# lidq92/LBDRN-MSIC

Hardware: AMD Instinct MI355X
Metric: Mpixels/s encode+decode (and bpp/PSNR parity) on D2/K5/bc64/nl2 (higher is better)
Workload: dtype f32; 1 GPU; synthetic 8-band 2048x2048 uint16 tile per step, K=5 D=2 bc=64 nl=2 bs=8192 e=10 (BASELINE.json configs[1] by default); encode fit + 16-bit weight truncation + decode; tiles_per_gpu=50, tiles_in_flight_per_gpu=4, tiles_per_launch=2, parallelism=image-sharded x1

## Files before the change

include/lbdrn_hip.h:

```cpp
#ifndef LBDRN_HIP_H
#define LBDRN_HIP_H

#include <stddef.h>
#include <stdint.h>

#ifdef __cplusplus
extern "C" {
#endif
#if defined(__GNUC__)
#pragma GCC visibility push(default)
#endif

#define LBDRN_ABI_VERSION 2

typedef enum lbdrn_status {
    LBDRN_OK = 0,
    LBDRN_E_ARG = -1,
    LBDRN_E_DEVICE = -2,
    LBDRN_E_UNSUPPORTED = -3,
    LBDRN_E_WORKSPACE = -4
} lbdrn_status;

typedef struct lbdrn_geom {
    int32_t C, H, W;
    int32_t K;
    int32_t D;
    int32_t msb_max;
    int32_t use_colors;
    int32_t relative;
    int32_t P;
    int32_t reserved;
    const float *rowtab;
    const float *coltab;
} lbdrn_geom;

typedef struct lbdrn_net {
    int32_t F, bc, C, nl;
    int32_t act;
} lbdrn_net;
enum { LBDRN_ACT_SINE = 0, LBDRN_ACT_RELU = 1 };

const char *lbdrn_last_error(void);
int lbdrn_abi_version(void);
int lbdrn_device_check(void);
int64_t lbdrn_param_count(const lbdrn_net *net);
int32_t lbdrn_feature_dim(const lbdrn_geom *g);

int lbdrn_split_bits(const uint16_t *img, int32_t C, int32_t H, int32_t W, int32_t K,
                     uint16_t *msb, int32_t *msb_max, void *stream);

int lbdrn_labels(const uint16_t *img, int32_t C, int32_t H, int32_t W, int32_t K,
                 const int64_t *idx, int64_t n, float *labels, void *stream);

int lbdrn_features(const lbdrn_geom *g, const uint16_t *msb, const int64_t *idx, int64_t n,
                   float *features, void *stream);

size_t lbdrn_forward_workspace(const lbdrn_net *net, int64_t B);
int lbdrn_forward(const lbdrn_net *net, const float *params, const float *x, int64_t B, float *y,
                  void *workspace, size_t workspace_bytes, void *stream);

size_t lbdrn_tape_bytes(const lbdrn_net *net, int64_t B);
int lbdrn_forward_tape(const lbdrn_net *net, const float *params, const float *x, int64_t B, float *y,
                       void *tape, size_t tape_bytes, void *stream);
size_t lbdrn_backward_workspace(const lbdrn_net *net, int64_t B);
int lbdrn_backward(const lbdrn_net *net, const float *params, const float *x, int64_t B, const void *tape,
                   size_t tape_bytes, const float *y, const float *dy, float *grads, float *dx, void *workspace,
                   size_t workspace_bytes, void *stream);

#define LBDRN_PATH_AUTO 0
#define LBDRN_PATH_GENERIC 1
#define LBDRN_PATH_MFMA 2
size_t lbdrn_apply_workspace(const lbdrn_geom *g, const lbdrn_net *net);
int lbdrn_decode_fused(const lbdrn_geom *g, const lbdrn_net *net, const uint16_t *msb,
                       const float *params, uint16_t *out, float *y_out, void *workspace,
                       size_t workspace_bytes, int32_t path, void *stream);

#define LBDRN_EVAL_BACKGROUND 0x200
#define LBDRN_EVAL_FAST 0x400
#define LBDRN_EVAL_X16 0x1000
#define LBDRN_EVAL_VALID 0x4000
#define LBDRN_EVAL_DECODED 0x8000
int lbdrn_eval_sse(const lbdrn_geom *g, const lbdrn_net *net, const uint16_t *img,
                   const uint16_t *msb, const float *params, double *sse, void *workspace,
                   size_t workspace_bytes, int32_t path, void *stream);

#define LBDRN_APPLY_DECODE 0x2000
int lbdrn_apply_instance(const lbdrn_geom *g, const lbdrn_net *net, int32_t path_word, int32_t *out);

size_t lbdrn_train_workspace(const lbdrn_geom *g, const lbdrn_net *net, int32_t batch_size);
#define LBDRN_TRAIN_ALONE 0x800
int lbdrn_train_prepare(const lbdrn_geom *g, const lbdrn_net *net, const uint16_t *img,
                        const uint16_t *msb, int32_t batch_size, void *workspace,
                        size_t workspace_bytes, int32_t path, void *stream);
int lbdrn_train_epoch(const lbdrn_geom *g, const lbdrn_net *net, const uint16_t *img,
                      const uint16_t *msb, const int64_t *perm, int64_t n, int32_t batch_size,
                      float *params, float *exp_avg, float *exp_avg_sq, int64_t adam_step0,
                      double lr, float *losses, void *workspace, size_t workspace_bytes,
                      int32_t path, void *stream);

int lbdrn_train_group_max(void);
int32_t lbdrn_train_group_size(const lbdrn_geom *g, const lbdrn_net *net);
int32_t lbdrn_train_step_features(const lbdrn_geom *g, const lbdrn_net *net);
int lbdrn_train_epoch_group(int32_t count, const lbdrn_geom *const *g, const lbdrn_net *net,
                            const uint16_t *const *img, const uint16_t *const *msb, const int64_t *const *perm,
                            int64_t n, int32_t batch_size, float *const *params, float *const *exp_avg,
                            float *const *exp_avg_sq, int64_t adam_step0, double lr, float *const *losses,
                            void *const *workspace, size_t workspace_bytes, int32_t path, void *stream);

int lbdrn_train_profile_mode(int32_t mode);

size_t lbdrn_randperm_workspace(int64_t n, int32_t count);
int lbdrn_randperm(const uint64_t *seeds, int32_t count, int64_t n, int64_t *perm, void *workspace,
                   size_t workspace_bytes, void *stream);
int64_t lbdrn_mt19937_jump_poly(int32_t segment, uint32_t *poly624);

size_t lbdrn_plane_bound(int32_t C, int32_t H, int32_t W);
size_t lbdrn_plane_workspace(int32_t C, int32_t H, int32_t W);
int lbdrn_plane_encode(const uint16_t *planes, int32_t C, int32_t H, int32_t W, void *body, size_t body_capacity,
                       uint64_t *body_bytes, void *workspace, size_t workspace_bytes, void *stream);
int lbdrn_plane_decode(const void *body, size_t body_bytes, int32_t C, int32_t H, int32_t W, uint16_t *planes,
                       int32_t *status, void *workspace, size_t workspace_bytes, void *stream);

int64_t lbdrn_jp2k_block_count(int32_t C, int32_t H, int32_t W);
size_t lbdrn_jp2k_bound(int32_t C, int32_t H, int32_t W);
size_t lbdrn_jp2k_workspace(int32_t C, int32_t H, int32_t W);
int lbdrn_jp2k_encode(const uint16_t *planes, int32_t C, int32_t H, int32_t W, int32_t bits, void *out, size_t capacity,
                      size_t *nbytes, void *workspace, size_t workspace_bytes, void *stream);

size_t lbdrn_weights_bound(int64_t n);
int lbdrn_weights_encode(const float *values, int64_t n, int32_t precision, void *out, size_t capacity,
                         size_t *nbytes);
int lbdrn_weights_info(const void *stream, size_t nbytes, int64_t *n, int32_t *precision);
int lbdrn_weights_decode(const void *stream, size_t nbytes, float *values, int64_t capacity);

int lbdrn_train_step(const lbdrn_net *net, const float *x, const float *t, int32_t B,
                     float *params, float *exp_avg, float *exp_avg_sq, int64_t adam_step,
                     double lr, int32_t apply_adam, float *loss, float *grads, void *workspace,
                     size_t workspace_bytes, void *stream);

#if defined(__GNUC__)
#pragma GCC visibility pop
#endif
#ifdef __cplusplus
}
#endif
#endif
```

lbdrn-msic_amd/csrc/apply_mfma.hip:

```cpp
#include <cstdlib>

#include "common.hpp"
#include "lbdrn_math.hpp"

namespace lbdrn {

typedef float f32x16 __attribute__((ext_vector_type(16)));
typedef float f32x4 __attribute__((ext_vector_type(4)));
typedef _Float16 f16x8 __attribute__((ext_vector_type(8)));
typedef _Float16 f16x2 __attribute__((ext_vector_type(2)));

constexpr int APPLY_CHUNK = 20;
constexpr int APPLY_WAVES = 8;
constexpr int APPLY_THREADS = APPLY_WAVES * 64;
constexpr int TILE_W = 64;

__host__ __device__ inline int tile_row_to_neuron(int i)
{
    return 2 * ((i & 3) + 4 * (i >> 3)) + ((i >> 2) & 1);
}
__host__ __device__ inline int acc_row(int r, int h) { return (r & 3) + 8 * (r >> 2) + 4 * h; }

enum ApplyMode { MODE_DECODE = 0, MODE_EVAL = 1, MODE_EVAL_FAST = 2,
                 MODE_EVAL_X16 = 3 };
__host__ __device__ constexpr bool mode_fast(int mode) { return mode == MODE_EVAL_FAST || mode == MODE_EVAL_X16; }

#define APPLY_INSTANCES(X) \
    X(1, MODE_DECODE)    X(2, MODE_DECODE)    X(4, MODE_DECODE) \
    X(1, MODE_EVAL)      X(2, MODE_EVAL)      X(4, MODE_EVAL)   \
    X(1, MODE_EVAL_FAST) X(2, MODE_EVAL_FAST)                   \
    X(1, MODE_EVAL_X16)  X(2, MODE_EVAL_X16)
#define WAPPLY_INSTANCES(X) X(8, 1) X(8, 2) X(16, 1) X(16, 2)

#define X(NT, MODE) if (nt == NT && (mode < 0 || mode == MODE)) return true;
constexpr bool apply_row(int nt, int mode = -1) { APPLY_INSTANCES(X) return false; }
#undef X
#define X(NT, NL) if (nt == NT && (nl < 0 || nl == NL)) return true;
constexpr bool wapply_row(int nt, int nl = -1) { WAPPLY_INSTANCES(X) return false; }
#undef X
constexpr int serving_mode(int mode, int nt, bool x16)
{
    if (mode == MODE_EVAL_X16 && !(x16 && apply_row(nt, MODE_EVAL_X16))) mode = MODE_EVAL_FAST;
    if (mode == MODE_EVAL_FAST && !(apply_row(nt, MODE_EVAL_FAST) || wapply_row(nt))) mode = MODE_EVAL;
    return mode;
}
#define SERVES(mode, x16, nt12, nt4, wide)                                                                                          \
    static_assert(serving_mode(mode, 1, x16) == nt12 && serving_mode(mode, 2, x16) == nt12 && serving_mode(mode, 4, x16) == nt4 && \
                  serving_mode(mode, 8, x16) == wide && serving_mode(mode, 16, x16) == wide, #mode);
SERVES(MODE_DECODE, false, MODE_DECODE, MODE_DECODE, MODE_DECODE)          SERVES(MODE_DECODE, true, MODE_DECODE, MODE_DECODE, MODE_DECODE)
SERVES(MODE_EVAL, false, MODE_EVAL, MODE_EVAL, MODE_EVAL)                  SERVES(MODE_EVAL, true, MODE_EVAL, MODE_EVAL, MODE_EVAL)
SERVES(MODE_EVAL_FAST, false, MODE_EVAL_FAST, MODE_EVAL, MODE_EVAL_FAST)   SERVES(MODE_EVAL_FAST, true, MODE_EVAL_FAST, MODE_EVAL, MODE_EVAL_FAST)
SERVES(MODE_EVAL_X16, false, MODE_EVAL_FAST, MODE_EVAL, MODE_EVAL_FAST)    SERVES(MODE_EVAL_X16, true, MODE_EVAL_X16, MODE_EVAL, MODE_EVAL_FAST)
#undef SERVES

struct ApplyPlan {
    int NT;
    int S0;
    int TH;
    int SH, SW;
    int ncolor;
    int pair;
    int RS;
    int x16;
    int M16;
    int off_scale;
    int off_w0, off_wh, off_wl, off_bh, off_bl, pack_floats;
    int off_ktab, off_rowt, off_colt, off_tile, lds_floats;
    int tiles_x, tiles_y;
};

constexpr int X16_PIECES = 3;

static bool make_plan(const lbdrn_geom& g, const lbdrn_net& net, ApplyPlan* p, bool fast = false, bool x16 = false)
{
    if (net.act != LBDRN_ACT_SINE && net.act != LBDRN_ACT_RELU) return false;
    if (net.bc % 32 != 0 || !apply_row(net.bc / 32)) return false;
    if (net.C > 32 || net.nl < 1 || net.nl > 15) return false;
    ApplyPlan q;
    q.NT = net.bc / 32;
    q.ncolor = net.F - 2 * g.P;
    if (q.ncolor < 0) return false;
    q.S0 = g.P + ((q.ncolor + 1) / 2 + 3) / 4 * 4;
    const int side = 2 * g.D + 1;
    q.pair = fast && q.NT <= 2 && g.use_colors && g.D >= 1 && g.D <= 3 && (g.C % 2) == 0 && q.ncolor == g.C * side * side;
    q.RS = side * side - ((g.relative && g.D > 0) ? 1 : 0);
    if (q.pair) q.S0 = g.P + (g.C / 2) * q.RS;
    q.x16 = x16 && q.pair && g.relative && g.P == 0 && g.msb_max >= 1 && g.msb_max <= 2047 && (q.RS % 8) == 0;
    q.M16 = q.RS / 8;
    const int half = net.bc / 2;
    int o = 0;
    q.off_w0 = o; o += q.x16 ? (g.C / 2) * q.M16 * X16_PIECES * 64 * q.NT * 4 : q.S0 * 64 * q.NT;
    q.off_wh = o; o += (net.nl - 1) * half * 64 * q.NT;
    q.off_wl = o; o += half * 64;
    q.off_bh = o; o += net.nl * q.NT * 32;
    q.off_bl = o; o += 32;
    q.off_scale = o; o += 4;
    q.pack_floats = o;
    q.off_ktab = o; o += 2 * 2 * (q.S0 - g.P) + 2;
    q.SW = TILE_W + 2 * g.D;
    const int fixed = o;
    int th = 16;
    for (;; th >>= 1) {
        if (th == 0) return false;
        q.TH = th;
        q.SH = th + 2 * g.D;
        o = fixed;
        q.off_rowt = o; o += th * g.P;
        q.off_colt = o; o += TILE_W * g.P;
        q.off_tile = o; o += (g.use_colors ? g.C * q.SH * q.SW : 0);
        q.lds_floats = std::max(o, q.off_rowt + 2 * APPLY_THREADS + 4);
        if ((size_t)q.lds_floats * 4 <= 160 * 1024) break;
    }
    q.tiles_x = (g.W + TILE_W - 1) / TILE_W;
    q.tiles_y = (g.H + q.TH - 1) / q.TH;
    *p = q;
    return true;
}

constexpr int MFMA_PARTIALS = 1024;


__global__ void __launch_bounds__(256) k_w0_absmax(const float* __restrict__ params, int n, float* __restrict__ out)
{
    __shared__ float red[256];
    float m = 0.0f;
    for (int e = threadIdx.x; e < n; e += 256) m = fmaxf(m, fabsf(params[e]));
    red[threadIdx.x] = m;
    __syncthreads();
    for (int o = 128; o > 0; o >>= 1) {
        if ((int)threadIdx.x < o) red[threadIdx.x] = fmaxf(red[threadIdx.x], red[threadIdx.x + o]);
        __syncthreads();
    }
    if (threadIdx.x == 0) *out = red[0];
}

__device__ __forceinline__ int x16_shift(float amax)
{
    if (!(amax > 0.0f) || !(amax < 3.0e38f)) return 0;
    int ex;
    (void)frexpf(amax, &ex);
    return 15 - ex;
}

__global__ void __launch_bounds__(256)
    k_pack_apply(const float* __restrict__ params, lbdrn_net net, ApplyPlan p, int P, int C, int msb_max, const float* __restrict__ amax,
                 float* __restrict__ out)
{
    int e = blockIdx.x * blockDim.x + threadIdx.x;
    if (e >= p.pack_floats) return;
    const int NT = p.NT, half = net.bc / 2;
    float v = 0.0f;
    if (p.x16 && e < p.off_wh) {
        const int j = e & 3, q4 = e >> 2;
        const int t = q4 % NT, lane = (q4 / NT) % 64, rest = q4 / (NT * 64);
        const int piece = rest % X16_PIECES, m = (rest / X16_PIECES) % p.M16, cp = rest / (X16_PIECES * p.M16);
        const int s2 = p.ncolor / C, cen = s2 / 2, sh = x16_shift(*amax);
        const int neuron = tile_row_to_neuron(lane & 31) + 32 * t, ch = cp + (lane >> 5) * (C / 2);
        _Float16 hv[2];
        for (int u = 0; u < 2; ++u) {
            const int pos = 8 * m + 2 * j + u, r = pos + (pos >= cen ? 1 : 0);
            const float w = ldexpf(params[(int64_t)neuron * net.F + ch * s2 + r], sh);
            const _Float16 hi = (_Float16)w;
            const float r1 = w - (float)hi;
            const _Float16 mid = (_Float16)r1;
            const float r2 = r1 - (float)mid;
            hv[u] = piece == 0 ? hi : piece == 1 ? mid : (_Float16)r2;
        }
        f16x2 pk = {hv[0], hv[1]};
        out[e] = __builtin_bit_cast(float, pk);
        return;
    }
    if (e >= p.off_scale) {
        out[e] = (p.x16 && e == p.off_scale) ? ldexpf(1.0f, -x16_shift(*amax)) / (float)msb_max : 0.0f;
        return;
    }
    if (e < p.off_wh) {
        int t = e % NT, lane = (e / NT) % 64, s = e / (NT * 64);
        int k = 2 * s + (lane >> 5);
        if (p.pair && s >= P) {
            const int s2 = (p.ncolor / C), sp = s - P, c = sp / p.RS, rr = sp - c * p.RS;
            const int r = rr + ((p.RS < s2 && rr >= s2 / 2) ? 1 : 0);
            k = 2 * P + (c + (lane >> 5) * (C / 2)) * s2 + r;
        }
        int neuron = tile_row_to_neuron(lane & 31) + 32 * t;
        if (k < net.F) v = params[(int64_t)neuron * net.F + k];
    } else if (e < p.off_wl) {
        int q = e - p.off_wh;
        int t = q % NT, lane = (q / NT) % 64, s = (q / (NT * 64)) % half, l = 1 + q / (NT * 64 * half);
        int k = 2 * s + (lane >> 5);
        int neuron = tile_row_to_neuron(lane & 31) + 32 * t;
        int64_t base = (int64_t)net.bc * net.F + net.bc + (int64_t)(l - 1) * ((int64_t)net.bc * net.bc + net.bc);
        v = params[base + (int64_t)neuron * net.bc + k];
    } else if (e < p.off_bh) {
        int q = e - p.off_wl;
        int lane = q % 64, s = q / 64;
        int k = 2 * s + (lane >> 5), ch = lane & 31;
        int64_t base = (int64_t)net.bc * net.F + net.bc + (int64_t)(net.nl - 1) * ((int64_t)net.bc * net.bc + net.bc);
        if (ch < net.C) v = params[base + (int64_t)ch * net.bc + k];
    } else if (e < p.off_bl) {
        int q = e - p.off_bh;
        int r = q % 16, h = (q / 16) % 2, t = (q / 32) % NT, l = q / (32 * NT);
        int neuron = 2 * r + h + 32 * t;
        int64_t wbase = l == 0 ? 0 : (int64_t)net.bc * net.F + net.bc + (int64_t)(l - 1) * ((int64_t)net.bc * net.bc + net.bc);
        int64_t nin = l == 0 ? net.F : net.bc;
        v = params[wbase + (int64_t)net.bc * nin + neuron];
    } else {
        int q = e - p.off_bl;
        int r = q % 16, h = q / 16;
        int ch = acc_row(r, h);
        int64_t base = (int64_t)net.bc * net.F + net.bc + (int64_t)(net.nl - 1) * ((int64_t)net.bc * net.bc + net.bc);
        if (ch < net.C) v = params[base + (int64_t)net.C * net.bc + ch];
    }
    out[e] = v;
}


struct ApplyArgs {
    lbdrn_geom g;
    lbdrn_net net;
    ApplyPlan p;
    const float* packed;
    const uint16_t* msb;
    const uint16_t* img;
    uint16_t* out;
    float* y_out;
    double* partial;
    int nvirt;
    int nodata;
    int decoded;
    unsigned long long* stamps;
};

#ifdef LBDRN_APPLY_STAMPS
#define ASTAMP(k)                                                                    \
    do {                                                                              \
        unsigned long long t_;                                                        \
        __builtin_amdgcn_sched_barrier(0);                                            \
        asm volatile("s_memtime %0\n\ts_waitcnt lgkmcnt(0)" : "=s"(t_)::"memory");   \
        __builtin_amdgcn_sched_barrier(0);                                            \
        acc_t[k] += t_ - last_t;                                                      \
        last_t = t_;                                                                  \
    } while (0)
#else
#define ASTAMP(k)
#endif

template <int NT>
__device__ __forceinline__ void load_a(const float* w, int idx, float (&a)[NT])
{
    if constexpr (NT == 1) {
        a[0] = w[idx];
    } else if constexpr (NT == 2) {
        float2 v = *reinterpret_cast<const float2*>(w + (size_t)idx * 2);
        a[0] = v.x; a[1] = v.y;
    } else {
        float4 v = *reinterpret_cast<const float4*>(w + (size_t)idx * 4);
        a[0] = v.x; a[1] = v.y; a[2] = v.z; a[3] = v.w;
    }
}

template <int NT, int D, bool REL>
__device__ __forceinline__ void layer0_pair(f32x16 (&acc)[NT], const float* wc, const float* tp)
{
    constexpr int side = 2 * D + 1, S2 = side * side, CEN = D * side + D, SW = TILE_W + 2 * D, RS = S2 - (REL ? 1 : 0);
    const float cen = tp[D * SW + D];
    float bq[RS];
#pragma unroll
    for (int r = 0; r < S2; ++r) {
        if (REL && r == CEN) continue;
        const float nb = tp[(r / side) * SW + (r % side)];
        bq[r - ((REL && r > CEN) ? 1 : 0)] = REL ? nb - cen : nb;
    }
    __builtin_amdgcn_sched_barrier(0);
#pragma unroll
    for (int k = 0; k < RS; ++k) {
        float a[NT];
        load_a<NT>(wc, k * 64, a);
#pragma unroll
        for (int tt = 0; tt < NT; ++tt) acc[tt] = __builtin_amdgcn_mfma_f32_32x32x2f32(a[tt], bq[k], acc[tt], 0, 0, 0);
    }
    __builtin_amdgcn_sched_barrier(0);
}

template <int NT, int D>
__device__ __forceinline__ void layer0_pair_x16(f32x16 (&acc)[NT], const float* wc, const float* tp)
{
    constexpr int side = 2 * D + 1, S2 = side * side, CEN = D * side + D, SW = TILE_W + 2 * D, RS = S2 - 1, M = RS / 8;
    static_assert(RS % 8 == 0, "(2D+1)^2 - 1 = 4 D (D+1)");
    const float cen = tp[D * SW + D];
    float bq[RS];
#pragma unroll
    for (int r = 0; r < S2; ++r) {
        if (r == CEN) continue;
        bq[r - (r > CEN ? 1 : 0)] = tp[(r / side) * SW + (r % side)] - cen;
    }
    f16x8 b[M];
#pragma unroll
    for (int m = 0; m < M; ++m)
#pragma unroll
        for (int j = 0; j < 4; ++j) {
            const f16x2 pk = __builtin_bit_cast(f16x2, __builtin_amdgcn_cvt_pkrtz(bq[8 * m + 2 * j], bq[8 * m + 2 * j + 1]));
            b[m][2 * j] = pk[0];
            b[m][2 * j + 1] = pk[1];
        }
    __builtin_amdgcn_sched_barrier(0);
#pragma unroll
    for (int m = 0; m < M; ++m)
#pragma unroll
        for (int pc = 0; pc < X16_PIECES; ++pc) {
            const float4* ap = reinterpret_cast<const float4*>(wc + (size_t)((m * X16_PIECES + pc) * 64) * NT * 4);
#pragma unroll
            for (int tt = 0; tt < NT; ++tt)
                acc[tt] = __builtin_amdgcn_mfma_f32_32x32x16_f16(__builtin_bit_cast(f16x8, ap[tt]), b[m], acc[tt], 0, 0, 0);
        }
    __builtin_amdgcn_sched_barrier(0);
}

template <int MODE, bool RELU>
__device__ __forceinline__ float apply_hidden_act(float z)
{
    if constexpr (RELU) return z > 0.0f ? z : 0.0f;
    else return mode_fast(MODE) ? fast_sin(30.0f * z) : siren_act(z);
}

template <int NT, int NG>
__device__ __forceinline__ void last_layer_4x4(f32x16& o, const f32x16 (&hid)[NT], const float* wl, const float* bl, int lane)
{
    const bool lo = lane < 32;
    f32x4 part[NG];
#pragma unroll
    for (int gq = 0; gq < NG; ++gq) {
        const float4 b4 = *reinterpret_cast<const float4*>(bl + gq * 16);
        part[gq][0] = lo ? b4.x : 0.0f; part[gq][1] = lo ? b4.y : 0.0f;
        part[gq][2] = lo ? b4.z : 0.0f; part[gq][3] = lo ? b4.w : 0.0f;
    }
    const float* wq = wl + (lane & 32) + (lane & 3);
    float a[NT * 16][NG];
#pragma unroll
    for (int s = 0; s < NT * 16; ++s)
#pragma unroll
        for (int gq = 0; gq < NG; ++gq) a[s][gq] = wq[s * 64 + 4 * gq];
    __builtin_amdgcn_sched_barrier(0);
#pragma unroll
    for (int s = 0; s < NT * 16; ++s) {
        const float b = hid[s / 16][s % 16];
#pragma unroll
        for (int gq = 0; gq < NG; ++gq) part[gq] = __builtin_amdgcn_mfma_f32_4x4x1f32(a[s][gq], b, part[gq], 0, 0, 0);
    }
#pragma unroll
    for (int i = 0; i < 4; ++i) {
        const float x = part[0][i], y = part[NG - 1][i];
        const auto sw = __builtin_amdgcn_permlane32_swap(__float_as_uint(x), __float_as_uint(y), false, false);
        const unsigned even = sw[0], odd = sw[1];
        o[i] = __uint_as_float(even) + __uint_as_float(odd);
    }
}

template <int NT, int MODE, bool RELU>
__global__ void __launch_bounds__(APPLY_THREADS) k_apply_mfma(ApplyArgs A)
{
    extern __shared__ __attribute__((aligned(16))) float lds[];
    const lbdrn_geom& g = A.g;
    const ApplyPlan& p = A.p;
    const int tid = threadIdx.x;
    const int lane = tid & 63, wave = tid >> 6;
    const int j = lane & 31, h = lane >> 5;
    const int half = A.net.bc / 2;
    const int P = g.P, D = g.D, C = g.C;

    for (int e = tid * 4; e < p.pack_floats; e += APPLY_THREADS * 4) {
        if (e + 3 < p.pack_floats) {
            *reinterpret_cast<float4*>(lds + e) = *reinterpret_cast<const float4*>(A.packed + e);
        } else {
            for (int q = e; q < p.pack_floats; ++q) lds[q] = A.packed[q];
        }
    }
    int* ktab = reinterpret_cast<int*>(lds + p.off_ktab);
    {
        const int side = 2 * D + 1, plane = p.SH * p.SW;
        for (int k = tid; k < 2 * (p.S0 - P) + 1; k += APPLY_THREADS) {
            int kk = min(k, p.ncolor - 1);
            kk = max(kk, 0);
            int c = kk / (side * side), r = kk - c * side * side;
            int dy = r / side, dx = r - dy * side;
            ktab[2 * k] = c * plane + (dy - D) * p.SW + (dx - D);
            ktab[2 * k + 1] = c * plane;
        }
    }
    const float* w0 = lds + p.off_w0;
    const float* wh = lds + p.off_wh;
    const float* wl = lds + p.off_wl;
    const float* bh = lds + p.off_bh;
    const float* bl = lds + p.off_bl;
    float* rowt = lds + p.off_rowt;
    float* colt = lds + p.off_colt;
    float* tile = lds + p.off_tile;
    const bool rel = g.relative && D > 0;
    const float maxf = (float)g.msb_max;
    const int64_t HW = (int64_t)g.H * g.W;
    const float scale = (float)((1 << g.K) - 1);
    const int lmask = (1 << g.K) - 1;
#ifdef LBDRN_APPLY_STAMPS
    unsigned long long acc_t[8] = {}, last_t;
    asm volatile("s_memtime %0\n\ts_waitcnt lgkmcnt(0)" : "=s"(last_t)::"memory");
#endif
    const int ntiles = p.tiles_x * p.tiles_y;
    for (int v = blockIdx.x; v < A.nvirt; v += gridDim.x) {
    double sse = 0.0;
    for (int t = v; t < ntiles; t += A.nvirt) {
        const int ty = t / p.tiles_x, tx = t - ty * p.tiles_x;
        const int y0 = ty * p.TH, x0 = tx * TILE_W;
        __syncthreads();
        if (g.use_colors) {
            const int plane = p.SH * p.SW, total = C * plane;
            const unsigned msw = 0xFFFFFFFFu / (unsigned)p.SW + 1u, msh = 0xFFFFFFFFu / (unsigned)p.SH + 1u;
            const bool simple = D < g.H && D < g.W && total < 65536 && p.SH > 1;
            constexpr int UB = 8;
            for (int base = 0; base < total; base += APPLY_THREADS * UB) {
                unsigned short raw[UB];
#pragma unroll
                for (int u = 0; u < UB; ++u) {
                    const int e = min(base + u * APPLY_THREADS + tid, total - 1);
                    int row, sx, c, sy, yy, xx;
                    if (simple) {
                        row = (int)__umulhi((unsigned)e, msw); sx = e - row * p.SW;
                        c = (int)__umulhi((unsigned)row, msh); sy = row - c * p.SH;
                        yy = y0 + sy - D; xx = x0 + sx - D;
                        yy = yy < 0 ? -yy : yy; yy = yy >= g.H ? 2 * (g.H - 1) - yy : yy;
                        xx = xx < 0 ? -xx : xx; xx = xx >= g.W ? 2 * (g.W - 1) - xx : xx;
                        yy = max(0, min(yy, g.H - 1));
                        xx = max(0, min(xx, g.W - 1));
                    } else {
                        row = e / p.SW; sx = e - row * p.SW; c = row / p.SH; sy = row - c * p.SH;
                        yy = reflect_idx(y0 + sy - D, g.H); xx = reflect_idx(x0 + sx - D, g.W);
                    }
                    raw[u] = mode_fast(MODE) ? (unsigned short)(A.img[(int64_t)c * HW + (int64_t)yy * g.W + xx] >> g.K)
                                             : A.msb[(int64_t)c * HW + (int64_t)yy * g.W + xx];
                }
#pragma unroll
                for (int u = 0; u < UB; ++u) {
                    const int e = base + u * APPLY_THREADS + tid;
                    if (e < total) tile[e] = MODE == MODE_EVAL_X16 ? (float)raw[u] : (float)raw[u] / maxf;
                }
            }
        }
        for (int e = tid; e < p.TH * P; e += APPLY_THREADS) {
            int yy = min(y0 + e / P, g.H - 1);
            rowt[e] = g.rowtab[(int64_t)yy * P + e % P];
        }
        for (int e = tid; e < TILE_W * P; e += APPLY_THREADS) {
            int xx = min(x0 + e / P, g.W - 1);
            colt[e] = g.coltab[(int64_t)xx * P + e % P];
        }
        __syncthreads();

        ASTAMP(0);
        const int nseg = p.TH * (TILE_W / 32);
        for (int seg = wave; seg < nseg; seg += APPLY_WAVES) {
            const int ly = seg / (TILE_W / 32), lx = (seg % (TILE_W / 32)) * 32;
            const int pixbase = (ly + D) * p.SW + (lx + j + D);
            const int yy = y0 + ly, xx = x0 + lx + j;
            const bool inside = yy < g.H && xx < g.W;
            const int64_t pix = (int64_t)min(yy, g.H - 1) * g.W + min(xx, g.W - 1);
            const int nreg = 4 * ((C + 7) / 8);
            unsigned short pre[16];
            {
                const uint16_t* src = (MODE == MODE_DECODE) ? A.msb : A.img;
#pragma unroll
                for (int r = 0; r < 16; ++r) {
                    pre[r] = 0;
                    if (r < nreg) pre[r] = src[(int64_t)min(acc_row(r, h), C - 1) * HW + pix];
                }
            }
            f32x16 acc[NT];
            f32x16 hid[NT];
#pragma unroll
            for (int tt = 0; tt < NT; ++tt)
#pragma unroll
                for (int q4 = 0; q4 < 4; ++q4) {
                    float4 b4 = *reinterpret_cast<const float4*>(bh + (tt * 2 + h) * 16 + q4 * 4);
                    acc[tt][q4 * 4 + 0] = b4.x; acc[tt][q4 * 4 + 1] = b4.y;
                    acc[tt][q4 * 4 + 2] = b4.z; acc[tt][q4 * 4 + 3] = b4.w;
                }
            if constexpr (MODE == MODE_EVAL_X16) {
                f32x16 bias0[NT];
#pragma unroll
                for (int tt = 0; tt < NT; ++tt) {
                    bias0[tt] = acc[tt];
#pragma unroll
                    for (int r = 0; r < 16; ++r) acc[tt][r] = 0.0f;
                }
                const int plane = p.SH * p.SW;
                const float* tp = tile + h * (C / 2) * plane + ly * p.SW + lx + j;
                const float* wc = w0 + (size_t)lane * NT * 4;
                const size_t wstep = (size_t)p.M16 * X16_PIECES * 64 * NT * 4;
                for (int c = 0; c < C / 2; ++c, tp += plane, wc += wstep) {
                    if (D == 1) layer0_pair_x16<NT, 1>(acc, wc, tp);
                    else if (D == 2) layer0_pair_x16<NT, 2>(acc, wc, tp);
                    else layer0_pair_x16<NT, 3>(acc, wc, tp);
                }
                const float cs = lds[p.off_scale];
#pragma unroll
                for (int tt = 0; tt < NT; ++tt)
#pragma unroll
                    for (int r = 0; r < 16; ++r) acc[tt][r] = fmaf(acc[tt][r], cs, bias0[tt][r]);
            }
            for (int s = 0; s < (MODE == MODE_EVAL_X16 ? 0 : P); ++s) {
                int k = 2 * s + h;
                float b = (k < P) ? rowt[ly * P + k] : colt[(lx + j) * P + (k - P)];
                float a[NT];
                load_a<NT>(w0, s * 64 + lane, a);
#pragma unroll
                for (int tt = 0; tt < NT; ++tt)
                    acc[tt] = __builtin_amdgcn_mfma_f32_32x32x2f32(a[tt], b, acc[tt], 0, 0, 0);
            }
            bool paired = MODE == MODE_EVAL_X16;
            if constexpr (MODE == MODE_EVAL_FAST) {
                if (p.pair) {
                    paired = true;
                    const int plane = p.SH * p.SW;
                    const float* tp = tile + h * (C / 2) * plane + ly * p.SW + lx + j;
                    const float* wc = w0 + ((size_t)P * 64 + lane) * NT;
                    for (int c = 0; c < C / 2; ++c, tp += plane, wc += (size_t)p.RS * 64 * NT) {
                        if (rel) {
                            if (D == 1) layer0_pair<NT, 1, true>(acc, wc, tp);
                            else if (D == 2) layer0_pair<NT, 2, true>(acc, wc, tp);
                            else layer0_pair<NT, 3, true>(acc, wc, tp);
                        } else {
                            if (D == 1) layer0_pair<NT, 1, false>(acc, wc, tp);
                            else if (D == 2) layer0_pair<NT, 2, false>(acc, wc, tp);
                            else layer0_pair<NT, 3, false>(acc, wc, tp);
                        }
                    }
                }
            }
            if (!paired) {
                constexpr int CH = APPLY_CHUNK;
                static_assert(CH % 4 == 0, "the steps left behind the chunks are taken four at a time");
                int s4 = P;
                for (; s4 + CH <= p.S0; s4 += CH) {
                    float bq[CH];
#pragma unroll
                    for (int u = 0; u < CH; ++u) {
                        const int kk = 2 * (s4 + u - P) + h;
                        const int2 e = *reinterpret_cast<const int2*>(ktab + 2 * kk);
                        const float nb = tile[pixbase + e.x];
                        const float ct = tile[pixbase + e.y];
                        bq[u] = rel ? nb - ct : nb;
                    }
                    __builtin_amdgcn_sched_barrier(0);
#pragma unroll
                    for (int u = 0; u < CH; ++u) {
                        float a[NT];
                        load_a<NT>(w0, (s4 + u) * 64 + lane, a);
#pragma unroll
                        for (int tt = 0; tt < NT; ++tt)
                            acc[tt] = __builtin_amdgcn_mfma_f32_32x32x2f32(a[tt], bq[u], acc[tt], 0, 0, 0);
                    }
                    __builtin_amdgcn_sched_barrier(0);
                }
                for (; s4 < p.S0; s4 += 4) {
                    float bq[4];
                    float aq[4][NT];
#pragma unroll
                    for (int u = 0; u < 4; ++u) {
                        int kk = 2 * (s4 + u - P) + h;
                        int2 e = *reinterpret_cast<const int2*>(ktab + 2 * kk);
                        float nb = tile[pixbase + e.x];
                        float ct = tile[pixbase + e.y];
                        bq[u] = rel ? nb - ct : nb;
                        load_a<NT>(w0, (s4 + u) * 64 + lane, aq[u]);
                    }
#pragma unroll
                    for (int u = 0; u < 4; ++u)
#pragma unroll
                        for (int tt = 0; tt < NT; ++tt)
                            acc[tt] = __builtin_amdgcn_mfma_f32_32x32x2f32(aq[u][tt], bq[u], acc[tt], 0, 0, 0);
                }
            }
            ASTAMP(1);
#pragma unroll
            for (int tt = 0; tt < NT; ++tt)
#pragma unroll
                for (int r = 0; r < 16; ++r) hid[tt][r] = apply_hidden_act<MODE, RELU>(acc[tt][r]);
            ASTAMP(2);
            for (int l = 1; l < A.net.nl; ++l) {
                const float* wlayer = wh + (size_t)(l - 1) * half * 64 * NT;
#pragma unroll
                for (int tt = 0; tt < NT; ++tt)
#pragma unroll
                    for (int q4 = 0; q4 < 4; ++q4) {
                        float4 b4 = *reinterpret_cast<const float4*>(bh + ((l * NT + tt) * 2 + h) * 16 + q4 * 4);
                        acc[tt][q4 * 4 + 0] = b4.x; acc[tt][q4 * 4 + 1] = b4.y;
                        acc[tt][q4 * 4 + 2] = b4.z; acc[tt][q4 * 4 + 3] = b4.w;
                    }
#pragma unroll
                for (int s = 0; s < NT * 16; ++s) {
                    float b = hid[s / 16][s % 16];
                    float a[NT];
                    load_a<NT>(wlayer, s * 64 + lane, a);
#pragma unroll
                    for (int tt = 0; tt < NT; ++tt)
                        acc[tt] = __builtin_amdgcn_mfma_f32_32x32x2f32(a[tt], b, acc[tt], 0, 0, 0);
                }
#pragma unroll
                for (int tt = 0; tt < NT; ++tt)
#pragma unroll
                    for (int r = 0; r < 16; ++r) hid[tt][r] = apply_hidden_act<MODE, RELU>(acc[tt][r]);
            }
            ASTAMP(3);
            f32x16 o;
            if (mode_fast(MODE)) {
                if (C > 4) last_layer_4x4<NT, 2>(o, hid, wl, bl, lane);
                else last_layer_4x4<NT, 1>(o, hid, wl, bl, lane);
            } else {
#pragma unroll
                for (int q4 = 0; q4 < 4; ++q4) {
                    float4 b4 = *reinterpret_cast<const float4*>(bl + h * 16 + q4 * 4);
                    o[q4 * 4 + 0] = b4.x; o[q4 * 4 + 1] = b4.y; o[q4 * 4 + 2] = b4.z; o[q4 * 4 + 3] = b4.w;
                }
#pragma unroll
                for (int s = 0; s < NT * 16; ++s) {
                    float b = hid[s / 16][s % 16];
                    float a = wl[s * 64 + lane];
                    o = __builtin_amdgcn_mfma_f32_32x32x2f32(a, b, o, 0, 0, 0);
                }
            }
            ASTAMP(4);
#pragma unroll
            for (int r = 0; r < 16; ++r) {
                const int ch = acc_row(r, h);
                if (r < nreg && ch < C && inside) {
                    float yv = mode_fast(MODE) ? fast_sigmoid(o[r]) : canon_sigmoid(o[r]);
                    if (MODE == MODE_DECODE) {
                        float rr = __builtin_rintf(yv * scale);
                        int base = (int)pre[r] << g.K;
                        A.out[(int64_t)ch * HW + pix] = (uint16_t)(base + (int)rr);
                        if (A.y_out) A.y_out[pix * C + ch] = yv;
                    } else if ((int)pre[r] != A.nodata) {
                        if (MODE == MODE_EVAL && A.decoded) {
                            int band = ch;
                            asm volatile("" : "+v"(band));
                            sse += decoded_term((int)pre[r], (int)A.msb[(int64_t)band * HW + pix], yv, scale, g.K);
                            continue;
                        }
                        float lab = (float)((int)pre[r] & lmask) / scale;
                        float d = yv - lab;
                        sse += (double)(d * d);
                    }
                }
            }
            ASTAMP(5);
        }
    }
    if (MODE != MODE_DECODE) {
        __syncthreads();
        double* red = reinterpret_cast<double*>(lds + ((p.off_rowt + 3) & ~3));
        red[tid] = sse;
        __syncthreads();
        for (int o2 = APPLY_THREADS / 2; o2 > 0; o2 >>= 1) {
            if (tid < o2) red[tid] += red[tid + o2];
            __syncthreads();
        }
        if (tid == 0) A.partial[v] = red[0];
    }
    }
#ifdef LBDRN_APPLY_STAMPS
    if (tid == 0 && A.stamps)
        for (int k = 0; k < 8; ++k) A.stamps[(size_t)blockIdx.x * 8 + k] = acc_t[k];
#endif
}

__global__ void k_sum_partials_mfma(const double* __restrict__ partial, int n, double* dst)
{
    const int lane = threadIdx.x;
    double s = 0.0;
    for (int i = lane; i < n; i += 64) s += partial[i];
    for (int o = 32; o > 0; o >>= 1) s += __shfl_down(s, o);
    if (lane == 0) *dst = s;
}

#include "apply_wide.inc"

static size_t wapply_workspace(const lbdrn_geom& g, const lbdrn_net& net)
{
    WApplyPlan p;
    if (!make_wapply_plan(g, net, &p)) return 0;
    return align_up((size_t)p.pack_floats * 4, 256) + align_up(MFMA_PARTIALS * sizeof(double), 256);
}

bool mfma_apply_supported(const lbdrn_geom& g, const lbdrn_net& net)
{
    ApplyPlan p;
    WApplyPlan w;
    return make_plan(g, net, &p) || make_wapply_plan(g, net, &w);
}

static size_t apply_pack_bytes(const lbdrn_geom& g, const lbdrn_net& net)
{
    ApplyPlan p{}, q{};
    if (!make_plan(g, net, &p)) return 0;
    lbdrn_geom gx = g;
    gx.msb_max = 1;
    const bool x = make_plan(gx, net, &q, true, true) && q.x16;
    return align_up((size_t)std::max(p.pack_floats, x ? q.pack_floats : 0) * 4, 256);
}

size_t mfma_apply_workspace(const lbdrn_geom& g, const lbdrn_net& net)
{
    ApplyPlan p;
    if (!make_plan(g, net, &p)) return wapply_workspace(g, net);
    return apply_pack_bytes(g, net) + align_up(MFMA_PARTIALS * sizeof(double), 256) + 256;
}

template <auto KERN, int THREADS, bool ALWAYS_160K, class Args>
static int launch_pass(const Args& A, int grid, hipStream_t s, bool whole_lds)
{
    const size_t lds_bytes = std::max((size_t)A.p.lds_floats * 4, whole_lds ? (size_t)125 * 1280 : (size_t)0);
    static std::atomic<unsigned long long> configured{0};
    if (ALWAYS_160K || whole_lds)
        if (int rc = configure_lds_once(KERN, 160 * 1024, configured)) return rc;
    KERN<<<grid, THREADS, lds_bytes, s>>>(A);
    LBDRN_LAUNCH_CHECK();
    return 0;
}

static int dispatch_apply(const ApplyArgs& A, int mode, int grid, hipStream_t s, bool whole_lds)
{
    const bool relu = A.net.act == LBDRN_ACT_RELU;
    if (mode_fast(mode) && A.net.C > 8) {
        set_error("the fast instances of the fused apply pass take at most 8 bands, not %d", A.net.C);
        return LBDRN_E_UNSUPPORTED;
    }
#define X(nt, m)                                                                                                       \
    if (A.p.NT == nt && mode == m)                                                                                     \
        return relu ? launch_pass<k_apply_mfma<nt, m, true>, APPLY_THREADS, true>(A, grid, s, whole_lds)               \
                    : launch_pass<k_apply_mfma<nt, m, false>, APPLY_THREADS, true>(A, grid, s, whole_lds);
    APPLY_INSTANCES(X)
#undef X
    set_error("no fused apply pass is built for NT = %d, mode %d", A.p.NT, mode);
    return LBDRN_E_UNSUPPORTED;
}

static int dispatch_wapply(const WApplyArgs& A, int mode, int grid, hipStream_t s, bool whole_lds)
{
#define LAUNCH(nt, n, m) if (mode == m) return launch_pass<k_apply_wide<nt, n, m>, WA_THREADS, false>(A, grid, s, whole_lds);
#define X(nt, n) if (A.p.NT == nt && A.net.nl == n) { LAUNCH(nt, n, MODE_DECODE) LAUNCH(nt, n, MODE_EVAL) LAUNCH(nt, n, MODE_EVAL_FAST) }
    WAPPLY_INSTANCES(X)
#undef X
#undef LAUNCH
    set_error("no streamed apply pass is built for NT = %d, nl = %d, mode %d", A.p.NT, A.net.nl, mode);
    return LBDRN_E_UNSUPPORTED;
}

struct ApplyCall {
    const lbdrn_geom& g;
    const lbdrn_net& net;
    const uint16_t *img, *msb;
    const float* params;
    uint16_t* out;
    float* y_out;
    double* sse;
    int nodata;
    bool decoded;
    void* ws;
    size_t ws_bytes;
    bool background;
    hipStream_t s;
};

static int workspace_holds(const ApplyCall& c, size_t need)
{
    if (c.ws && c.ws_bytes >= need) return 0;
    set_error("apply workspace too small: %zu < %zu", c.ws_bytes, need);
    return LBDRN_E_WORKSPACE;
}

template <class Args>
static int report_stamps(const Args& A, int grid, hipStream_t s)
{
#ifdef LBDRN_APPLY_STAMPS
    LBDRN_HIP_TRY(hipStreamSynchronize(s));
    unsigned long long h[1024 * 8];
    LBDRN_HIP_TRY(hipMemcpy(h, A.stamps, (size_t)grid * 8 * sizeof(unsigned long long), hipMemcpyDeviceToHost));
    double sum[8] = {};
    for (int b = 0; b < grid; ++b) for (int k = 0; k < 8; ++k) sum[k] += (double)h[b * 8 + k];
    if constexpr (std::is_same<Args, WApplyArgs>::value) {
        const double segs = (double)A.p.tiles_x * A.p.tiles_y * A.p.TH * (TILE_W / 16) / 4 / grid;
        double rtmin = 1e30, rtmax = 0;
        for (int b = 0; b < grid; ++b) { rtmin = std::min(rtmin, (double)h[b * 8 + 6]); rtmax = std::max(rtmax, (double)h[b * 8 + 6]); }
        fprintf(stderr, "[lbdrn wide apply stamps] wave lifetime %.2f .. %.2f ms (mean %.2f); per wave: tiles-staging %.0f total; per 16-px segment: L0 %.0f sin %.0f L1 %.0f last %.0f epilogue %.0f\n",
                rtmin / 1e5, rtmax / 1e5, sum[6] / grid / 1e5, sum[0] / grid, sum[1] / grid / segs, sum[2] / grid / segs, sum[3] / grid / segs, sum[4] / grid / segs, sum[5] / grid / segs);
    } else {
        const double blocks = (double)A.p.tiles_x * A.p.tiles_y * A.p.TH * (TILE_W / 32) / APPLY_WAVES / grid;
        fprintf(stderr, "[lbdrn apply stamps] per wave: tiles-staging %.0f total; per 32-px block: L0 %.0f sin %.0f hidden %.0f last %.0f epilogue %.0f\n",
                sum[0] / grid, sum[1] / grid / blocks, sum[2] / grid / blocks, sum[3] / grid / blocks, sum[4] / grid / blocks, sum[5] / grid / blocks);
    }
#endif
    return 0;
}

template <class Args>
static int run_pass(Args& A, const ApplyCall& c, int mode, const float* packed, double* partial,
                    int (*dispatch)(const Args&, int, int, hipStream_t, bool))
{
    A.g = c.g; A.net = c.net; A.packed = packed; A.msb = c.msb; A.img = c.img; A.out = c.out; A.y_out = c.y_out; A.partial = partial; A.nodata = c.nodata; A.decoded = c.decoded;
    int dev = 0, cus = 256;
    if (hipGetDevice(&dev) == hipSuccess)
        (void)hipDeviceGetAttribute(&cus, hipDeviceAttributeMultiprocessorCount, dev);
    A.nvirt = std::min(std::min(A.p.tiles_x * A.p.tiles_y, cus), MFMA_PARTIALS);
    const int grid = c.background ? std::max(1, A.nvirt / 2) : A.nvirt;
    A.stamps = nullptr;
#ifdef LBDRN_APPLY_STAMPS
    static unsigned long long* stamp_buf = nullptr;
    if (!stamp_buf) LBDRN_HIP_TRY(hipMalloc(&stamp_buf, 1024 * 8 * sizeof(unsigned long long)));
    A.stamps = stamp_buf;
#endif
    if (int rc = dispatch(A, mode, grid, c.s, c.background && mode != MODE_DECODE)) return rc;
    if (mode != MODE_DECODE) {
        k_sum_partials_mfma<<<1, 64, 0, c.s>>>(partial, A.nvirt, c.sse);
        LBDRN_LAUNCH_CHECK();
    }
    return report_stamps(A, grid, c.s);
}

static bool resolve_wapply(const lbdrn_geom& g, const lbdrn_net& net, int mode, WApplyPlan* plan, int* serving)
{
    if (!make_wapply_plan(g, net, plan, mode_fast(mode))) return false;
    *serving = serving_mode(mode, plan->NT, false);
    return true;
}

static int run_wapply(const ApplyCall& c, int mode)
{
    WApplyArgs A;
    int serving = mode;
    if (!resolve_wapply(c.g, c.net, mode, &A.p, &serving)) {
        set_error("shape not supported by the MFMA apply kernels");
        return LBDRN_E_UNSUPPORTED;
    }
    if (int rc = workspace_holds(c, wapply_workspace(c.g, c.net))) return rc;
    float* packed = (float*)c.ws;
    double* partial = (double*)((char*)c.ws + align_up((size_t)A.p.pack_floats * 4, 256));
    k_pack_apply_wide<<<(A.p.pack_floats + 255) / 256, 256, 0, c.s>>>(c.params, c.net, A.p, 2 * c.g.P, packed);
    LBDRN_LAUNCH_CHECK();
    return run_pass(A, c, serving, packed, partial, dispatch_wapply);
}

static int resolve_apply(const lbdrn_geom& g, const lbdrn_net& net, int mode, ApplyPlan* plan, int* wide_mode)
{
    if (mode == MODE_EVAL_X16) {
        ApplyPlan fp, xp;
        if (make_plan(g, net, &fp, true, false) && (!make_plan(g, net, &xp, true, true) || xp.TH < fp.TH)) mode = MODE_EVAL_FAST;
    }
    const int requested = mode;
    if (mode_fast(mode) && net.C > 8) mode = MODE_EVAL;
    *wide_mode = -1;
    if (!make_plan(g, net, plan, mode_fast(mode), mode == MODE_EVAL_X16)) {
        *wide_mode = requested;
        return requested;
    }
    return serving_mode(mode, plan->NT, plan->x16);
}

bool mfma_eval_reads_msb(const lbdrn_geom& g, const lbdrn_net& net, bool fast, bool x16)
{
    ApplyPlan plan;
    int wide_mode = -1;
    int mode = resolve_apply(g, net, fast ? (x16 ? MODE_EVAL_X16 : MODE_EVAL_FAST) : MODE_EVAL, &plan, &wide_mode);
    if (wide_mode >= 0) {
        WApplyPlan wp;
        if (!resolve_wapply(g, net, wide_mode, &wp, &mode)) return true;
    }
    return !mode_fast(mode);
}

bool mfma_apply_instance(const lbdrn_geom& g, const lbdrn_net& net, int request, int32_t out[8])
{
    ApplyPlan p;
    int wide_mode = -1;
    const int serving = resolve_apply(g, net, request, &p, &wide_mode);
    if (wide_mode < 0) {
        const int32_t v[8] = {1, p.NT, net.act == LBDRN_ACT_RELU, serving, p.TH, p.pair, p.x16, p.tiles_x * p.tiles_y};
        std::copy(v, v + 8, out);
        return true;
    }
    WApplyPlan w;
    int wserving = wide_mode;
    if (!resolve_wapply(g, net, wide_mode, &w, &wserving)) return false;
    const int32_t v[8] = {2, w.NT, net.nl, wserving, w.TH, w.skip, 0, w.tiles_x * w.tiles_y};
    std::copy(v, v + 8, out);
    return true;
}

static int run_apply(const ApplyCall& c, int mode)
{
    const lbdrn_geom& g = c.g;
    const lbdrn_net& net = c.net;
    ApplyArgs A;
    int wide_mode = -1;
    mode = resolve_apply(g, net, mode, &A.p, &wide_mode);
    if (wide_mode >= 0) return run_wapply(c, wide_mode);
    if (int rc = workspace_holds(c, mfma_apply_workspace(g, net))) return rc;
    float* packed = (float*)c.ws;
    const size_t pack_bytes = apply_pack_bytes(g, net);
    double* partial = (double*)((char*)c.ws + pack_bytes);
    float* amax = (float*)((char*)c.ws + pack_bytes + align_up(MFMA_PARTIALS * sizeof(double), 256));
    if (A.p.x16) {
        k_w0_absmax<<<1, 256, 0, c.s>>>(c.params, net.bc * net.F, amax);
        LBDRN_LAUNCH_CHECK();
    }
    k_pack_apply<<<(A.p.pack_floats + 255) / 256, 256, 0, c.s>>>(c.params, net, A.p, g.P, g.C, g.msb_max, amax, packed);
    LBDRN_LAUNCH_CHECK();
    return run_pass(A, c, mode, packed, partial, dispatch_apply);
}

int mfma_decode(const lbdrn_geom& g, const lbdrn_net& net, const uint16_t* msb, const float* params,
                uint16_t* out, float* y_out, void* ws, size_t ws_bytes, hipStream_t s)
{
    return run_apply({g, net, nullptr, msb, params, out, y_out, nullptr, -1, false, ws, ws_bytes, false, s}, MODE_DECODE);
}

int mfma_eval_sse(const lbdrn_geom& g, const lbdrn_net& net, const uint16_t* img,
                  const uint16_t* msb, const float* params, double* sse, void* ws, size_t ws_bytes,
                  bool background, bool fast, bool x16, int nodata, bool decoded, hipStream_t s)
{
    return run_apply({g, net, img, msb, params, nullptr, nullptr, sse, nodata, decoded, ws, ws_bytes, background, s},
                     fast ? (x16 ? MODE_EVAL_X16 : MODE_EVAL_FAST) : MODE_EVAL);
}

}
```

lbdrn-msic_amd/csrc/cabi.hip:

```cpp
#include <string>

#include "common.hpp"

namespace lbdrn {
bool mfma_train_supported(const lbdrn_geom& g, const lbdrn_net& net, int bs = 0);
int mfma_train_step_features(const lbdrn_geom& g, const lbdrn_net& net);
bool mfma_train_takes_groups(const lbdrn_geom& g, const lbdrn_net& net);
size_t mfma_train_workspace(const lbdrn_geom& g, const lbdrn_net& net, int bs);
int mfma_train_prepare(const lbdrn_geom& g, const lbdrn_net& net, const uint16_t* img,
                       const uint16_t* msb, int bs, void* ws, size_t ws_bytes, hipStream_t s);
int mfma_train_epoch(const lbdrn_geom& g, const lbdrn_net& net, const uint16_t* img,
                     const uint16_t* msb, const int64_t* perm, int64_t n, int bs, float* params,
                     float* m, float* v, int64_t step0, double lr, float* losses, void* ws,
                     size_t ws_bytes, hipStream_t s, bool alone);
int train_profile_mode(int mode);
size_t randperm_workspace(int64_t n, int count);
size_t plane_bound(int C, int H, int W);
size_t plane_workspace(int C, int H, int W);
int plane_encode(const uint16_t* planes, int C, int H, int W, void* body, size_t body_cap, uint64_t* body_bytes,
                 void* ws, size_t ws_bytes, hipStream_t s);
int plane_decode(const void* body, size_t body_bytes, int C, int H, int W, uint16_t* planes, int* status, void* ws,
                 size_t ws_bytes, hipStream_t s);
int plane_body_aligned(const void* body);
int64_t mt19937_jump_poly(int segment, uint32_t* out);
int randperm_batch(const uint64_t* seeds, int count, int64_t n, int64_t* out, void* ws, size_t ws_bytes,
                   hipStream_t s);
int64_t jp2k_block_count(int C, int H, int W);
size_t jp2k_bound(int C, int H, int W);
size_t jp2k_workspace(int C, int H, int W);
int jp2k_encode(const uint16_t* planes, int C, int H, int W, int bits, uint8_t* out, size_t cap, size_t* nbytes, void* ws,
                size_t ws_bytes, hipStream_t s);
size_t weights_bound(int64_t n);
int weights_encode(const float* values, int64_t n, int precision, uint8_t* out, size_t cap, size_t* nbytes);
int weights_info(const uint8_t* in, size_t nbytes, int64_t* n, int* precision);
int weights_decode(const uint8_t* in, size_t nbytes, float* values, int64_t cap);
}

using namespace lbdrn;

static int device_ok()
{
    static thread_local int cached = 1;
    static thread_local char why[384] = "";
    if (cached < 0) set_error("%s", why);
    if (cached != 1) return cached;
    int n = 0;
    hipError_t e = hipGetDeviceCount(&n);
    if (e != hipSuccess || n < 1) {
        snprintf(why, sizeof(why), "no HIP device available (%s); liblbdrn_hip has no CPU path",
                 e == hipSuccess ? "device count 0" : hipGetErrorString(e));
        set_error("%s", why);
        return cached = LBDRN_E_DEVICE;
    }
    int dev = 0;
    hipDeviceProp_t prop;
    if (hipGetDevice(&dev) != hipSuccess || hipGetDeviceProperties(&prop, dev) != hipSuccess) {
        snprintf(why, sizeof(why), "cannot query the current HIP device");
        set_error("%s", why);
        return cached = LBDRN_E_DEVICE;
    }
    if (std::string(prop.gcnArchName).rfind("gfx950", 0) != 0) {
        snprintf(why, sizeof(why), "device %d is %s; this library is built for gfx950 (MI355X) only", dev, prop.gcnArchName);
        set_error("%s", why);
        return cached = LBDRN_E_DEVICE;
    }
    return cached = 0;
}

#define NEED_DEVICE()                  \
    do {                               \
        if (int rc_ = device_ok()) return rc_; \
    } while (0)

static bool aligned_to(const void* p, size_t a) { return ((uintptr_t)p & (a - 1)) == 0; }
#define LBDRN_ALIGNED(ptr, a) LBDRN_REQUIRE(aligned_to(ptr, a), #ptr " must be %d-byte aligned (lbdrn_hip.h: Alignment)", (int)(a))
#define LBDRN_ALIGNED_FIT(arr, f, a) \
    LBDRN_REQUIRE(aligned_to((arr)[f], a), #arr " of fit %c must be %d-byte aligned (lbdrn_hip.h: Alignment)", (char)('A' + (f)), (int)(a))
enum { ALIGN_WORKSPACE = 256, ALIGN_TRAIN_PARAMS = 16 };

static int geom_tables_aligned(const lbdrn_geom* g)
{
    LBDRN_ALIGNED(g->rowtab, 4);
    LBDRN_ALIGNED(g->coltab, 4);
    return 0;
}

static int check_geom_call(const lbdrn_geom* g)
{
    if (int rc = check_geom(g)) return rc;
    return geom_tables_aligned(g);
}

static int net_matches(const lbdrn_geom* g, const lbdrn_net* net)
{
    LBDRN_REQUIRE(net->F == feature_dim(*g), "net.F=%d but the geometry yields %d features", net->F,
                  feature_dim(*g));
    LBDRN_REQUIRE(net->C == g->C, "net.C=%d but the image has %d bands", net->C, g->C);
    LBDRN_REQUIRE(g->msb_max >= 0 && g->msb_max <= 65535, "msb_max=%d out of range", g->msb_max);
    return 0;
}

static int workspace_fits(const char* what, const void* ws, size_t have, size_t need)
{
    if (!ws || have < need) {
        set_error("%s workspace too small: %zu < %zu", what, have, need);
        return LBDRN_E_WORKSPACE;
    }
    return 0;
}

extern "C" {

const char* lbdrn_last_error(void) { return last_error(); }
int lbdrn_abi_version(void) { return LBDRN_ABI_VERSION; }
int lbdrn_device_check(void) { return device_ok(); }

int64_t lbdrn_param_count(const lbdrn_net* net)
{
    if (check_net(net)) return LBDRN_E_ARG;
    return param_count(*net);
}

int32_t lbdrn_feature_dim(const lbdrn_geom* g)
{
    if (!g) return LBDRN_E_ARG;
    return feature_dim(*g);
}

int lbdrn_split_bits(const uint16_t* img, int32_t C, int32_t H, int32_t W, int32_t K, uint16_t* msb,
                     int32_t* msb_max, void* stream)
{
    LBDRN_REQUIRE(img && msb_max, "img and msb_max must not be null");
    LBDRN_REQUIRE(C >= 1 && H >= 1 && W >= 1 && K >= 1 && K <= 15, "bad arguments C=%d H=%d W=%d K=%d", C, H, W, K);
    LBDRN_ALIGNED(img, 2);
    LBDRN_ALIGNED(msb, 2);
    LBDRN_ALIGNED(msb_max, 4);
    NEED_DEVICE();
    return generic_split_bits(img, C, H, W, K, msb, msb_max, (hipStream_t)stream);
}

int lbdrn_labels(const uint16_t* img, int32_t C, int32_t H, int32_t W, int32_t K, const int64_t* idx,
                 int64_t n, float* labels, void* stream)
{
    LBDRN_REQUIRE(img && labels, "img and labels must not be null");
    LBDRN_REQUIRE(C >= 1 && H >= 1 && W >= 1 && K >= 1 && K <= 15 && n >= 0, "bad arguments");
    LBDRN_REQUIRE(idx || n <= (int64_t)H * W, "n exceeds the pixel count");
    LBDRN_ALIGNED(img, 2);
    LBDRN_ALIGNED(idx, 8);
    LBDRN_ALIGNED(labels, 4);
    NEED_DEVICE();
    return generic_labels(img, C, H, W, K, idx, n, labels, (hipStream_t)stream);
}

int lbdrn_features(const lbdrn_geom* g, const uint16_t* msb, const int64_t* idx, int64_t n,
                   float* features, void* stream)
{
    if (int rc = check_geom_call(g)) return rc;
    LBDRN_REQUIRE(msb && features && n >= 0, "msb/features null or n negative");
    LBDRN_REQUIRE(idx || n <= (int64_t)g->H * g->W, "n exceeds the pixel count");
    LBDRN_ALIGNED(msb, 2);
    LBDRN_ALIGNED(idx, 8);
    LBDRN_ALIGNED(features, 4);
    NEED_DEVICE();
    return generic_features(launch_geom(*g), msb, idx, n, 0, features, (hipStream_t)stream);
}

size_t lbdrn_forward_workspace(const lbdrn_net* net, int64_t B)
{
    if (check_net(net) || B < 0) return 0;
    return generic_forward_workspace(*net, B);
}

int lbdrn_forward(const lbdrn_net* net, const float* params, const float* x, int64_t B, float* y,
                  void* workspace, size_t workspace_bytes, void* stream)
{
    if (int rc = check_net(net)) return rc;
    LBDRN_REQUIRE(params && x && y && B >= 0, "null pointer or negative batch");
    LBDRN_ALIGNED(params, 4);
    LBDRN_ALIGNED(x, 4);
    LBDRN_ALIGNED(y, 4);
    LBDRN_ALIGNED(workspace, ALIGN_WORKSPACE);
    NEED_DEVICE();
    return generic_forward(*net, params, x, B, y, workspace, workspace_bytes, (hipStream_t)stream);
}

size_t lbdrn_tape_bytes(const lbdrn_net* net, int64_t B)
{
    if (check_net(net) || B < 0) return 0;
    return generic_tape_bytes(*net, B);
}

int lbdrn_forward_tape(const lbdrn_net* net, const float* params, const float* x, int64_t B, float* y, void* tape,
                       size_t tape_bytes, void* stream)
{
    if (int rc = check_net(net)) return rc;
    LBDRN_REQUIRE(params && x && y && B >= 0, "null pointer or negative batch");
    LBDRN_ALIGNED(params, 4);
    LBDRN_ALIGNED(x, 4);
    LBDRN_ALIGNED(y, 4);
    LBDRN_ALIGNED(tape, ALIGN_WORKSPACE);
    NEED_DEVICE();
    return generic_forward_tape(*net, params, x, B, y, tape, tape_bytes, (hipStream_t)stream);
}

size_t lbdrn_backward_workspace(const lbdrn_net* net, int64_t B)
{
    if (check_net(net) || B < 0) return 0;
    return generic_backward_workspace(*net, B);
}

int lbdrn_backward(const lbdrn_net* net, const float* params, const float* x, int64_t B, const void* tape,
                   size_t tape_bytes, const float* y, const float* dy, float* grads, float* dx, void* workspace,
                   size_t workspace_bytes, void* stream)
{
    if (int rc = check_net(net)) return rc;
    LBDRN_REQUIRE(params && x && y && dy && grads && B >= 0, "null pointer or negative batch");
    LBDRN_ALIGNED(params, 4);
    LBDRN_ALIGNED(x, 4);
    LBDRN_ALIGNED(y, 4);
    LBDRN_ALIGNED(dy, 4);
    LBDRN_ALIGNED(grads, 4);
    LBDRN_ALIGNED(dx, 4);
    LBDRN_ALIGNED(tape, ALIGN_WORKSPACE);
    LBDRN_ALIGNED(workspace, ALIGN_WORKSPACE);
    NEED_DEVICE();
    return generic_backward(*net, params, x, B, tape, tape_bytes, y, dy, grads, dx, workspace, workspace_bytes,
                            (hipStream_t)stream);
}

size_t lbdrn_apply_workspace(const lbdrn_geom* g, const lbdrn_net* net)
{
    if (check_geom(g) || check_net(net)) return 0;
    size_t a = generic_apply_workspace(*g, *net);
    size_t b = mfma_apply_supported(*g, *net) ? mfma_apply_workspace(*g, *net) : 0;
    return a > b ? a : b;
}

static int pick_apply(const lbdrn_geom* g, const lbdrn_net* net, int32_t path, bool* use_mfma)
{
    const bool ok = mfma_apply_supported(*g, *net);
    if (path == LBDRN_PATH_MFMA && !ok) {
        set_error("fused MFMA apply kernel does not support bc=%d nl=%d C=%d D=%d", net->bc, net->nl,
                  net->C, g->D);
        return LBDRN_E_UNSUPPORTED;
    }
    LBDRN_REQUIRE(path >= LBDRN_PATH_AUTO && path <= LBDRN_PATH_MFMA, "unknown path %d", path);
    *use_mfma = ok && path != LBDRN_PATH_GENERIC;
    return 0;
}

int lbdrn_decode_fused(const lbdrn_geom* g, const lbdrn_net* net, const uint16_t* msb,
                       const float* params, uint16_t* out, float* y_out, void* workspace,
                       size_t workspace_bytes, int32_t path, void* stream)
{
    if (int rc = check_geom_call(g)) return rc;
    if (int rc = check_net(net)) return rc;
    if (int rc = net_matches(g, net)) return rc;
    LBDRN_REQUIRE(msb && params && out, "msb, params and out must not be null");
    LBDRN_ALIGNED(msb, 2);
    LBDRN_ALIGNED(params, 4);
    LBDRN_ALIGNED(out, 2);
    LBDRN_ALIGNED(y_out, 4);
    LBDRN_ALIGNED(workspace, ALIGN_WORKSPACE);
    NEED_DEVICE();
    bool use_mfma = false;
    if (int rc = pick_apply(g, net, path, &use_mfma)) return rc;
    if (int rc = workspace_fits("apply", workspace, workspace_bytes, lbdrn_apply_workspace(g, net))) return rc;
    const lbdrn_geom gl = launch_geom(*g);
    if (use_mfma)
        return mfma_decode(gl, *net, msb, params, out, y_out, workspace, workspace_bytes, (hipStream_t)stream);
    return generic_decode(gl, *net, msb, params, out, y_out, workspace, workspace_bytes, (hipStream_t)stream);
}

int lbdrn_eval_sse(const lbdrn_geom* g, const lbdrn_net* net, const uint16_t* img, const uint16_t* msb,
                   const float* params, double* sse, void* workspace, size_t workspace_bytes,
                   int32_t path, void* stream)
{
    if (int rc = check_geom_call(g)) return rc;
    if (int rc = check_net(net)) return rc;
    if (int rc = net_matches(g, net)) return rc;
    LBDRN_REQUIRE(img && params && sse, "img, params and sse must not be null");
    LBDRN_ALIGNED(img, 2);
    LBDRN_ALIGNED(msb, 2);
    LBDRN_ALIGNED(params, 4);
    LBDRN_ALIGNED(sse, 8);
    LBDRN_ALIGNED(workspace, ALIGN_WORKSPACE);
    const bool background = (path & LBDRN_EVAL_BACKGROUND) != 0, fast = (path & LBDRN_EVAL_FAST) != 0;
    const bool x16 = fast && (path & LBDRN_EVAL_X16) != 0;
    const bool valid = (path & LBDRN_EVAL_VALID) != 0;
    LBDRN_REQUIRE(!valid || (g->reserved >= 0 && g->reserved <= 65535),
                  "LBDRN_EVAL_VALID: g->reserved holds the nodata value, 0..65535, not %d", g->reserved);
    const int nodata = valid ? g->reserved : -1;
    const bool decoded = (path & LBDRN_EVAL_DECODED) != 0;
    LBDRN_REQUIRE(!decoded || !(path & (LBDRN_EVAL_FAST | LBDRN_EVAL_X16)),
                  "LBDRN_EVAL_DECODED takes neither LBDRN_EVAL_FAST nor LBDRN_EVAL_X16: decode arithmetic is canonical");
    LBDRN_REQUIRE(!decoded || msb, "LBDRN_EVAL_DECODED: msb must not be null, it is the plane the reconstruction is built on");
    path &= ~(LBDRN_EVAL_BACKGROUND | LBDRN_EVAL_FAST | LBDRN_EVAL_X16 | LBDRN_EVAL_VALID | LBDRN_EVAL_DECODED);
    bool use_mfma = false;
    if (int rc = pick_apply(g, net, path, &use_mfma)) return rc;
    const lbdrn_geom gl = launch_geom(*g);
    LBDRN_REQUIRE(msb || (use_mfma && !mfma_eval_reads_msb(gl, *net, fast, x16)),
                  "msb must not be null: %s", !fast ? "only LBDRN_EVAL_FAST leaves it unread"
                  : !use_mfma ? "the generic path ignores LBDRN_EVAL_FAST and reads it"
                  : "a canonical instance serves this shape's LBDRN_EVAL_FAST request and reads it");
    NEED_DEVICE();
    if (int rc = workspace_fits("apply", workspace, workspace_bytes, lbdrn_apply_workspace(g, net))) return rc;
    if (use_mfma)
        return mfma_eval_sse(gl, *net, img, msb, params, sse, workspace, workspace_bytes, background, fast, x16,
                             nodata, decoded, (hipStream_t)stream);
    return generic_eval_sse(gl, *net, img, msb, params, sse, workspace, workspace_bytes, nodata, decoded, (hipStream_t)stream);
}

int lbdrn_apply_instance(const lbdrn_geom* g, const lbdrn_net* net, int32_t path_word, int32_t* out)
{
    if (int rc = check_geom(g)) return rc;
    if (int rc = check_net(net)) return rc;
    if (int rc = net_matches(g, net)) return rc;
    LBDRN_REQUIRE(out, "out must not be null");
    const bool decode = (path_word & LBDRN_APPLY_DECODE) != 0, fast = (path_word & LBDRN_EVAL_FAST) != 0;
    const bool x16 = fast && (path_word & LBDRN_EVAL_X16) != 0;
    LBDRN_REQUIRE(!(decode && fast), "LBDRN_APPLY_DECODE takes no evaluation flag");
    const int32_t path = path_word & ~(LBDRN_APPLY_DECODE | LBDRN_EVAL_BACKGROUND | LBDRN_EVAL_FAST | LBDRN_EVAL_X16 | LBDRN_EVAL_VALID | LBDRN_EVAL_DECODED);
    LBDRN_REQUIRE(path >= LBDRN_PATH_AUTO && path <= LBDRN_PATH_MFMA, "unknown path %d", path);
    if (!mfma_apply_supported(*g, *net) || !mfma_apply_instance(launch_geom(*g), *net, decode ? 0 : fast ? (x16 ? 3 : 2) : 1, out)) {
        set_error("fused MFMA apply kernel does not support bc=%d nl=%d C=%d D=%d", net->bc, net->nl, net->C, g->D);
        return LBDRN_E_UNSUPPORTED;
    }
    return 0;
}

size_t lbdrn_train_workspace(const lbdrn_geom* g, const lbdrn_net* net, int32_t batch_size)
{
    if (check_geom(g) || check_net(net) || batch_size < 1) return 0;
    size_t a = generic_train_workspace(*net, batch_size);
    size_t b = mfma_train_supported(*g, *net, batch_size) ? mfma_train_workspace(*g, *net, batch_size) : 0;
    return a > b ? a : b;
}

int lbdrn_train_prepare(const lbdrn_geom* g, const lbdrn_net* net, const uint16_t* img,
                        const uint16_t* msb, int32_t batch_size, void* workspace, size_t workspace_bytes,
                        int32_t path, void* stream)
{
    if (int rc = check_geom_call(g)) return rc;
    if (int rc = check_net(net)) return rc;
    if (int rc = net_matches(g, net)) return rc;
    LBDRN_REQUIRE(img && msb && batch_size >= 1, "null pointer or bad batch size");
    LBDRN_REQUIRE(path >= LBDRN_PATH_AUTO && path <= LBDRN_PATH_MFMA, "unknown path %d", path);
    LBDRN_ALIGNED(img, 2);
    LBDRN_ALIGNED(msb, 2);
    LBDRN_ALIGNED(workspace, ALIGN_WORKSPACE);
    NEED_DEVICE();
    const bool ok = mfma_train_supported(*g, *net, batch_size);
    if (path == LBDRN_PATH_MFMA && !ok) {
        set_error("fused MFMA train kernel does not support this shape or minibatch size");
        return LBDRN_E_UNSUPPORTED;
    }
    if (int rc = workspace_fits("train", workspace, workspace_bytes, lbdrn_train_workspace(g, net, batch_size))) return rc;
    if (ok && path != LBDRN_PATH_GENERIC)
        return mfma_train_prepare(launch_geom(*g), *net, img, msb, batch_size, workspace, workspace_bytes, (hipStream_t)stream);
    return 0;
}

int lbdrn_train_epoch(const lbdrn_geom* g, const lbdrn_net* net, const uint16_t* img,
                      const uint16_t* msb, const int64_t* perm, int64_t n, int32_t batch_size,
                      float* params, float* exp_avg, float* exp_avg_sq, int64_t adam_step0, double lr,
                      float* losses, void* workspace, size_t workspace_bytes, int32_t path,
                      void* stream)
{
    if (int rc = check_geom_call(g)) return rc;
    if (int rc = check_net(net)) return rc;
    if (int rc = net_matches(g, net)) return rc;
    LBDRN_REQUIRE(img && msb && perm && params && exp_avg && exp_avg_sq, "null pointer");
    LBDRN_REQUIRE(n >= 0 && batch_size >= 1 && adam_step0 >= 0, "bad n/batch_size/adam_step0");
    LBDRN_ALIGNED(img, 2);
    LBDRN_ALIGNED(msb, 2);
    LBDRN_ALIGNED(perm, 8);
    LBDRN_ALIGNED(params, ALIGN_TRAIN_PARAMS);
    LBDRN_ALIGNED(exp_avg, 4);
    LBDRN_ALIGNED(exp_avg_sq, 4);
    LBDRN_ALIGNED(losses, 4);
    LBDRN_ALIGNED(workspace, ALIGN_WORKSPACE);
    NEED_DEVICE();
    const bool alone = (path & LBDRN_TRAIN_ALONE) != 0;
    path &= ~LBDRN_TRAIN_ALONE;
    const bool ok = mfma_train_supported(*g, *net, batch_size);
    if (path == LBDRN_PATH_MFMA && !ok) {
        set_error("fused MFMA train kernel does not support this shape or minibatch size");
        return LBDRN_E_UNSUPPORTED;
    }
    LBDRN_REQUIRE(path >= LBDRN_PATH_AUTO && path <= LBDRN_PATH_MFMA, "unknown path %d", path);
    if (int rc = workspace_fits("train", workspace, workspace_bytes, lbdrn_train_workspace(g, net, batch_size))) return rc;
    const lbdrn_geom gl = launch_geom(*g);
    if (ok && path != LBDRN_PATH_GENERIC)
        return mfma_train_epoch(gl, *net, img, msb, perm, n, batch_size, params, exp_avg, exp_avg_sq,
                                adam_step0, lr, losses, workspace, workspace_bytes, (hipStream_t)stream, alone);
    return generic_train_epoch(gl, *net, img, msb, perm, n, batch_size, params, exp_avg, exp_avg_sq,
                               adam_step0, lr, losses, workspace, workspace_bytes, (hipStream_t)stream);
}

int lbdrn_train_group_max(void) { return 4; }

int32_t lbdrn_train_group_size(const lbdrn_geom* g, const lbdrn_net* net)
{
    if (!g || !net) return 1;
    return mfma_train_takes_groups(*g, *net) ? lbdrn_train_group_max() : 1;
}

int32_t lbdrn_train_step_features(const lbdrn_geom* g, const lbdrn_net* net)
{
    if (!g || !net) return 0;
    return mfma_train_step_features(*g, *net);
}

int lbdrn_train_epoch_group(int32_t count, const lbdrn_geom* const* g, const lbdrn_net* net, const uint16_t* const* img,
                            const uint16_t* const* msb, const int64_t* const* perm, int64_t n, int32_t batch_size,
                            float* const* params, float* const* exp_avg, float* const* exp_avg_sq, int64_t adam_step0,
                            double lr, float* const* losses, void* const* workspace, size_t workspace_bytes, int32_t path,
                            void* stream)
{
    LBDRN_REQUIRE(count >= 1 && count <= lbdrn_train_group_max(), "group of %d fits (1..%d)", count, lbdrn_train_group_max());
    LBDRN_REQUIRE(g && img && msb && perm && params && exp_avg && exp_avg_sq && workspace, "null pointer array");
    if (int rc = check_net(net)) return rc;
    for (int f = 0; f < count; ++f) {
        LBDRN_REQUIRE(g[f] && img[f] && msb[f] && perm[f] && params[f] && exp_avg[f] && exp_avg_sq[f], "null pointer (fit %d)", f);
        if (int rc = check_geom_call(g[f])) return rc;
        if (int rc = net_matches(g[f], net)) return rc;
        LBDRN_ALIGNED_FIT(img, f, 2);
        LBDRN_ALIGNED_FIT(msb, f, 2);
        LBDRN_ALIGNED_FIT(perm, f, 8);
        LBDRN_ALIGNED_FIT(params, f, ALIGN_TRAIN_PARAMS);
        LBDRN_ALIGNED_FIT(exp_avg, f, 4);
        LBDRN_ALIGNED_FIT(exp_avg_sq, f, 4);
        if (losses) LBDRN_ALIGNED_FIT(losses, f, 4);
        LBDRN_ALIGNED_FIT(workspace, f, ALIGN_WORKSPACE);
        LBDRN_REQUIRE(g[f]->C == g[0]->C && g[f]->H == g[0]->H && g[f]->W == g[0]->W &&
                      g[f]->D == g[0]->D && g[f]->P == g[0]->P && g[f]->use_colors == g[0]->use_colors &&
                      g[f]->relative == g[0]->relative, "the fits of a group must have one shape (fit %d differs)", f);
    }
    LBDRN_REQUIRE(n >= 0 && batch_size >= 1 && adam_step0 >= 0, "bad n/batch_size/adam_step0");
    const int32_t hint = count == 1 ? (path & LBDRN_TRAIN_ALONE) : 0;
    path &= ~LBDRN_TRAIN_ALONE;
    LBDRN_REQUIRE(path >= LBDRN_PATH_AUTO && path <= LBDRN_PATH_MFMA, "unknown path %d", path);
    NEED_DEVICE();
    for (int f = 0; f < count; ++f)
        if (int rc = workspace_fits("train", workspace[f], workspace_bytes, lbdrn_train_workspace(g[f], net, batch_size))) return rc;
    if (count > 1 && path != LBDRN_PATH_GENERIC && mfma_train_supported(*g[0], *net, batch_size)) {
        const int rc = mfma_train_epoch_group(count, launch_geom(*g[0]), *net, perm, n, batch_size, params, exp_avg, exp_avg_sq,
                                              adam_step0, lr, losses, workspace, workspace_bytes, (hipStream_t)stream, false);
        if (rc != LBDRN_E_UNSUPPORTED) return rc;
    }
    for (int f = 0; f < count; ++f)
        if (int rc = lbdrn_train_epoch(g[f], net, img[f], msb[f], perm[f], n, batch_size, params[f], exp_avg[f],
                                       exp_avg_sq[f], adam_step0, lr, losses ? losses[f] : nullptr, workspace[f],
                                       workspace_bytes, path | hint, stream))
            return rc;
    return 0;
}

int lbdrn_train_profile_mode(int32_t mode)
{
    LBDRN_REQUIRE(mode >= 0 && mode <= 5, "mode must be 0 .. 5");
    return train_profile_mode(mode);
}

size_t lbdrn_randperm_workspace(int64_t n, int32_t count)
{
    if (n < 0 || count < 1 || count > 32) return 0;
    return randperm_workspace(n, count);
}

int lbdrn_randperm(const uint64_t* seeds, int32_t count, int64_t n, int64_t* perm, void* workspace,
                   size_t workspace_bytes, void* stream)
{
    LBDRN_REQUIRE(n >= 0 && (perm || n == 0), "bad n or null output");
    LBDRN_ALIGNED(perm, 8);
    LBDRN_ALIGNED(workspace, ALIGN_WORKSPACE);
    NEED_DEVICE();
    return randperm_batch(seeds, count, n, perm, workspace, workspace_bytes, (hipStream_t)stream);
}

int64_t lbdrn_mt19937_jump_poly(int32_t segment, uint32_t* poly624)
{
    LBDRN_REQUIRE(poly624, "null output");
    return mt19937_jump_poly(segment, poly624);
}

size_t lbdrn_plane_bound(int32_t C, int32_t H, int32_t W) { return plane_bound(C, H, W); }
size_t lbdrn_plane_workspace(int32_t C, int32_t H, int32_t W) { return plane_workspace(C, H, W); }

int lbdrn_plane_encode(const uint16_t* planes, int32_t C, int32_t H, int32_t W, void* body, size_t body_capacity,
                       uint64_t* body_bytes, void* workspace, size_t workspace_bytes, void* stream)
{
    LBDRN_REQUIRE(C >= 1 && H >= 1 && W >= 1 && C <= 65535, "bad raster geometry");
    LBDRN_ALIGNED(planes, 2);
    if (int rc = plane_body_aligned(body)) return rc;
    LBDRN_ALIGNED(body_bytes, 8);
    LBDRN_ALIGNED(workspace, ALIGN_WORKSPACE);
    NEED_DEVICE();
    return plane_encode(planes, C, H, W, body, body_capacity, body_bytes, workspace, workspace_bytes,
                        (hipStream_t)stream);
}

int lbdrn_plane_decode(const void* body, size_t body_bytes, int32_t C, int32_t H, int32_t W, uint16_t* planes,
                       int32_t* status, void* workspace, size_t workspace_bytes, void* stream)
{
    LBDRN_REQUIRE(C >= 1 && H >= 1 && W >= 1 && C <= 65535, "bad raster geometry");
    if (int rc = plane_body_aligned(body)) return rc;
    LBDRN_ALIGNED(planes, 2);
    LBDRN_ALIGNED(status, 4);
    LBDRN_ALIGNED(workspace, ALIGN_WORKSPACE);
    NEED_DEVICE();
    return plane_decode(body, body_bytes, C, H, W, planes, status, workspace, workspace_bytes, (hipStream_t)stream);
}

int64_t lbdrn_jp2k_block_count(int32_t C, int32_t H, int32_t W) { return jp2k_block_count(C, H, W); }
size_t lbdrn_jp2k_bound(int32_t C, int32_t H, int32_t W) { return jp2k_bound(C, H, W); }
size_t lbdrn_jp2k_workspace(int32_t C, int32_t H, int32_t W) { return jp2k_workspace(C, H, W); }

int lbdrn_jp2k_encode(const uint16_t* planes, int32_t C, int32_t H, int32_t W, int32_t bits, void* out, size_t capacity,
                      size_t* nbytes, void* workspace, size_t workspace_bytes, void* stream)
{
    LBDRN_ALIGNED(planes, 2);
    LBDRN_ALIGNED(workspace, ALIGN_WORKSPACE);
    if (int rc = device_ok()) return rc;
    return jp2k_encode(planes, C, H, W, bits, (uint8_t*)out, capacity, nbytes, workspace, workspace_bytes, (hipStream_t)stream);
}

size_t lbdrn_weights_bound(int64_t n) { return n < 0 ? 0 : weights_bound(n); }

int lbdrn_weights_encode(const float* values, int64_t n, int32_t precision, void* out, size_t capacity, size_t* nbytes)
{
    LBDRN_REQUIRE((values || n == 0) && out && nbytes && n >= 0 && n < ((int64_t)1 << 32), "null pointer or bad count");
    LBDRN_REQUIRE(precision == 0 || (precision >= 2 && precision <= 32), "precision %d is not 0 or 2..32", precision);
    LBDRN_ALIGNED(values, 4);
    return weights_encode(values, n, precision, (uint8_t*)out, capacity, nbytes);
}

int lbdrn_weights_info(const void* stream, size_t nbytes, int64_t* n, int32_t* precision)
{
    LBDRN_REQUIRE(stream && n && precision, "null pointer");
    int prec = 0;
    const int rc = weights_info((const uint8_t*)stream, nbytes, n, &prec);
    *precision = prec;
    return rc;
}

int lbdrn_weights_decode(const void* stream, size_t nbytes, float* values, int64_t capacity)
{
    LBDRN_REQUIRE(stream && (values || capacity == 0) && capacity >= 0, "null pointer or bad capacity");
    LBDRN_ALIGNED(values, 4);
    return weights_decode((const uint8_t*)stream, nbytes, values, capacity);
}

int lbdrn_train_step(const lbdrn_net* net, const float* x, const float* t, int32_t B, float* params,
                     float* exp_avg, float* exp_avg_sq, int64_t adam_step, double lr,
                     int32_t apply_adam, float* loss, float* grads, void* workspace,
                     size_t workspace_bytes, void* stream)
{
    if (int rc = check_net(net)) return rc;
    LBDRN_REQUIRE(x && t && params, "x, t and params must not be null");
    LBDRN_REQUIRE(!apply_adam || (exp_avg && exp_avg_sq && adam_step >= 1), "Adam state missing or adam_step < 1");
    LBDRN_ALIGNED(x, 4);
    LBDRN_ALIGNED(t, 4);
    LBDRN_ALIGNED(params, 4);
    LBDRN_ALIGNED(exp_avg, 4);
    LBDRN_ALIGNED(exp_avg_sq, 4);
    LBDRN_ALIGNED(loss, 4);
    LBDRN_ALIGNED(grads, 4);
    LBDRN_ALIGNED(workspace, ALIGN_WORKSPACE);
    NEED_DEVICE();
    return generic_train_step(*net, x, t, B, params, exp_avg, exp_avg_sq, adam_step, lr, apply_adam,
                              loss, grads, workspace, workspace_bytes, (hipStream_t)stream);
}

}
```

lbdrn-msic_amd/csrc/common.hpp:

```cpp
#pragma once
#include <hip/hip_runtime.h>
#include <stdint.h>
#include <stdio.h>

#include <atomic>

#include "../../include/lbdrn_hip.h"

namespace lbdrn {

void set_error(const char* fmt, ...);
const char* last_error();

#define LBDRN_HIP_TRY(expr)                                                                  \
    do {                                                                                     \
        hipError_t e_ = (expr);                                                              \
        if (e_ != hipSuccess) {                                                              \
            ::lbdrn::set_error("%s failed: %s (%s:%d)", #expr, hipGetErrorString(e_), __FILE__, \
                               __LINE__);                                                    \
            return LBDRN_E_DEVICE;                                                           \
        }                                                                                    \
    } while (0)

#define LBDRN_REQUIRE(cond, ...)            \
    do {                                    \
        if (!(cond)) {                      \
            ::lbdrn::set_error(__VA_ARGS__); \
            return LBDRN_E_ARG;             \
        }                                   \
    } while (0)

#define LBDRN_LAUNCH_CHECK() LBDRN_HIP_TRY(hipGetLastError())

inline int64_t param_count(const lbdrn_net& n)
{
    int64_t c = 0;
    for (int l = 0; l < n.nl; ++l) c += (int64_t)n.bc * (l ? n.bc : n.F) + n.bc;
    return c + (int64_t)n.C * n.bc + n.C;
}
inline int64_t layer_offset(const lbdrn_net& n, int l)
{
    int64_t c = 0;
    for (int i = 0; i < l; ++i) c += (int64_t)n.bc * (i ? n.bc : n.F) + n.bc;
    return c;
}
inline int feature_dim(const lbdrn_geom& g)
{
    const int side = 2 * g.D + 1;
    return 2 * g.P + (g.use_colors ? g.C * side * side : 0);
}
inline size_t align_up(size_t x, size_t a) { return (x + a - 1) / a * a; }
inline lbdrn_geom launch_geom(const lbdrn_geom& g)
{
    lbdrn_geom r = g;
    if (r.msb_max < 1) r.msb_max = 1;
    return r;
}

template <class K>
static int configure_lds_once(K kern, int bytes, std::atomic<unsigned long long>& configured)
{
    int dev = 0;
    (void)hipGetDevice(&dev);
    const unsigned long long bit = 1ull << (dev & 63);
    if (!(configured.load(std::memory_order_relaxed) & bit)) {
        LBDRN_HIP_TRY(hipFuncSetAttribute(reinterpret_cast<const void*>(kern), hipFuncAttributeMaxDynamicSharedMemorySize, bytes));
        configured.fetch_or(bit, std::memory_order_relaxed);
    }
    return 0;
}

int check_geom(const lbdrn_geom* g);
int check_net(const lbdrn_net* n);

int generic_split_bits(const uint16_t* img, int C, int H, int W, int K, uint16_t* msb, int32_t* mx,
                       hipStream_t s);
int generic_labels(const uint16_t* img, int C, int H, int W, int K, const int64_t* idx, int64_t n,
                   float* labels, hipStream_t s);
int generic_features(const lbdrn_geom& g, const uint16_t* msb, const int64_t* idx, int64_t n,
                     int64_t first, float* out, hipStream_t s);
size_t generic_forward_workspace(const lbdrn_net& net, int64_t B);
int generic_forward(const lbdrn_net& net, const float* params, const float* x, int64_t B, float* y,
                    void* ws, size_t ws_bytes, hipStream_t s);
size_t generic_apply_workspace(const lbdrn_geom& g, const lbdrn_net& net);
int generic_decode(const lbdrn_geom& g, const lbdrn_net& net, const uint16_t* msb,
                   const float* params, uint16_t* out, float* y_out, void* ws, size_t ws_bytes,
                   hipStream_t s);
int generic_eval_sse(const lbdrn_geom& g, const lbdrn_net& net, const uint16_t* img,
                     const uint16_t* msb, const float* params, double* sse, void* ws,
                     size_t ws_bytes, int nodata, bool decoded, hipStream_t s);
size_t generic_train_workspace(const lbdrn_net& net, int B);
int generic_train_step(const lbdrn_net& net, const float* x, const float* t, int B, float* params,
                       float* m, float* v, int64_t adam_step, double lr, int apply_adam,
                       float* loss, float* grads, void* ws, size_t ws_bytes, hipStream_t s);
size_t generic_tape_bytes(const lbdrn_net& net, int64_t B);
size_t generic_backward_workspace(const lbdrn_net& net, int64_t B);
int generic_forward_tape(const lbdrn_net& net, const float* params, const float* x, int64_t B, float* y, void* tape,
                         size_t tape_bytes, hipStream_t s);
int generic_backward(const lbdrn_net& net, const float* params, const float* x, int64_t B, const void* tape,
                     size_t tape_bytes, const float* y, const float* dy, float* grads, float* dx, void* ws,
                     size_t ws_bytes, hipStream_t s);
int generic_train_epoch(const lbdrn_geom& g, const lbdrn_net& net, const uint16_t* img,
                        const uint16_t* msb, const int64_t* perm, int64_t n, int bs, float* params,
                        float* m, float* v, int64_t step0, double lr, float* losses, void* ws,
                        size_t ws_bytes, hipStream_t s);

bool mfma_apply_supported(const lbdrn_geom& g, const lbdrn_net& net);
size_t mfma_apply_workspace(const lbdrn_geom& g, const lbdrn_net& net);
int mfma_decode(const lbdrn_geom& g, const lbdrn_net& net, const uint16_t* msb, const float* params,
                uint16_t* out, float* y_out, void* ws, size_t ws_bytes, hipStream_t s);
int mfma_eval_sse(const lbdrn_geom& g, const lbdrn_net& net, const uint16_t* img,
                  const uint16_t* msb, const float* params, double* sse, void* ws, size_t ws_bytes,
                  bool background, bool fast, bool x16, int nodata, bool decoded, hipStream_t s);
bool mfma_eval_reads_msb(const lbdrn_geom& g, const lbdrn_net& net, bool fast, bool x16);
bool mfma_apply_instance(const lbdrn_geom& g, const lbdrn_net& net, int request, int32_t out[8]);

int mfma_train_epoch_group(int count, const lbdrn_geom& g, const lbdrn_net& net, const int64_t* const* perm, int64_t n,
                           int bs, float* const* params, float* const* m, float* const* v, int64_t step0, double lr,
                           float* const* losses, void* const* ws, size_t ws_bytes, hipStream_t s, bool alone);

}
```

lbdrn-msic_amd/lbdrn_hip/_lib.py:

```python
import ctypes

from ._native import E_ARG, E_DEVICE, E_UNSUPPORTED, E_WORKSPACE, Library

ABI_VERSION = 2
PATH_AUTO, PATH_GENERIC, PATH_MFMA = 0, 1, 2
EVAL_BACKGROUND = 0x200
EVAL_FAST = 0x400
EVAL_X16 = 0x1000
EVAL_VALID = 0x4000
EVAL_DECODED = 0x8000
APPLY_DECODE = 0x2000
TRAIN_ALONE = 0x800


class LbdrnError(RuntimeError):
    code = None


class Geom(ctypes.Structure):
    _fields_ = [("C", ctypes.c_int32), ("H", ctypes.c_int32), ("W", ctypes.c_int32),
                ("K", ctypes.c_int32), ("D", ctypes.c_int32), ("msb_max", ctypes.c_int32),
                ("use_colors", ctypes.c_int32), ("relative", ctypes.c_int32),
                ("P", ctypes.c_int32), ("reserved", ctypes.c_int32),
                ("rowtab", ctypes.c_void_p), ("coltab", ctypes.c_void_p)]


class Net(ctypes.Structure):
    _fields_ = [("F", ctypes.c_int32), ("bc", ctypes.c_int32), ("C", ctypes.c_int32),
                ("nl", ctypes.c_int32), ("act", ctypes.c_int32)]


_vp, _i32, _i64, _sz, _dbl = (ctypes.c_void_p, ctypes.c_int32, ctypes.c_int64, ctypes.c_size_t,
                              ctypes.c_double)
_GP, _NP = ctypes.POINTER(Geom), ctypes.POINTER(Net)
SIGNATURES = {
    "lbdrn_last_error": (ctypes.c_char_p, []),
    "lbdrn_abi_version": (ctypes.c_int, []),
    "lbdrn_device_check": (ctypes.c_int, []),
    "lbdrn_param_count": (_i64, [_NP]),
    "lbdrn_feature_dim": (_i32, [_GP]),
    "lbdrn_split_bits": (ctypes.c_int, [_vp, _i32, _i32, _i32, _i32, _vp, _vp, _vp]),
    "lbdrn_labels": (ctypes.c_int, [_vp, _i32, _i32, _i32, _i32, _vp, _i64, _vp, _vp]),
    "lbdrn_features": (ctypes.c_int, [_GP, _vp, _vp, _i64, _vp, _vp]),
    "lbdrn_forward_workspace": (_sz, [_NP, _i64]),
    "lbdrn_forward": (ctypes.c_int, [_NP, _vp, _vp, _i64, _vp, _vp, _sz, _vp]),
    "lbdrn_tape_bytes": (_sz, [_NP, _i64]),
    "lbdrn_forward_tape": (ctypes.c_int, [_NP, _vp, _vp, _i64, _vp, _vp, _sz, _vp]),
    "lbdrn_backward_workspace": (_sz, [_NP, _i64]),
    "lbdrn_backward": (ctypes.c_int, [_NP, _vp, _vp, _i64, _vp, _sz, _vp, _vp, _vp, _vp, _vp, _sz, _vp]),
    "lbdrn_apply_workspace": (_sz, [_GP, _NP]),
    "lbdrn_decode_fused": (ctypes.c_int, [_GP, _NP, _vp, _vp, _vp, _vp, _vp, _sz, _i32, _vp]),
    "lbdrn_eval_sse": (ctypes.c_int, [_GP, _NP, _vp, _vp, _vp, _vp, _vp, _sz, _i32, _vp]),
    "lbdrn_apply_instance": (ctypes.c_int, [_GP, _NP, _i32, ctypes.POINTER(_i32)]),
    "lbdrn_train_workspace": (_sz, [_GP, _NP, _i32]),
    "lbdrn_train_prepare": (ctypes.c_int, [_GP, _NP, _vp, _vp, _i32, _vp, _sz, _i32, _vp]),
    "lbdrn_train_epoch": (ctypes.c_int, [_GP, _NP, _vp, _vp, _vp, _i64, _i32, _vp, _vp, _vp, _i64,
                                         _dbl, _vp, _vp, _sz, _i32, _vp]),
    "lbdrn_train_group_max": (ctypes.c_int, []),
    "lbdrn_train_step_features": (_i32, [_GP, _NP]),
    "lbdrn_train_group_size": (_i32, [_GP, _NP]),
    "lbdrn_train_epoch_group": (ctypes.c_int, [_i32, _vp, _NP, _vp, _vp, _vp, _i64, _i32, _vp, _vp, _vp, _i64, _dbl, _vp,
                                               _vp, _sz, _i32, _vp]),
    "lbdrn_train_profile_mode": (ctypes.c_int, [_i32]),
    "lbdrn_randperm_workspace": (_sz, [_i64, _i32]),
    "lbdrn_randperm": (ctypes.c_int, [ctypes.POINTER(ctypes.c_uint64), _i32, _i64, _vp, _vp, _sz, _vp]),
    "lbdrn_mt19937_jump_poly": (_i64, [_i32, _vp]),
    "lbdrn_plane_bound": (_sz, [_i32, _i32, _i32]),
    "lbdrn_plane_workspace": (_sz, [_i32, _i32, _i32]),
    "lbdrn_plane_encode": (ctypes.c_int, [_vp, _i32, _i32, _i32, _vp, _sz, _vp, _vp, _sz, _vp]),
    "lbdrn_plane_decode": (ctypes.c_int, [_vp, _sz, _i32, _i32, _i32, _vp, _vp, _vp, _sz, _vp]),
    "lbdrn_jp2k_block_count": (_i64, [_i32, _i32, _i32]),
    "lbdrn_jp2k_bound": (_sz, [_i32, _i32, _i32]),
    "lbdrn_jp2k_workspace": (_sz, [_i32, _i32, _i32]),
    "lbdrn_jp2k_encode": (ctypes.c_int, [_vp, _i32, _i32, _i32, _i32, _vp, _sz, ctypes.POINTER(ctypes.c_size_t), _vp, _sz, _vp]),
    "lbdrn_weights_bound": (_sz, [_i64]),
    "lbdrn_weights_encode": (ctypes.c_int, [_vp, _i64, _i32, _vp, _sz, ctypes.POINTER(ctypes.c_size_t)]),
    "lbdrn_weights_info": (ctypes.c_int, [_vp, _sz, ctypes.POINTER(_i64), ctypes.POINTER(_i32)]),
    "lbdrn_weights_decode": (ctypes.c_int, [_vp, _sz, _vp, _i64]),
    "lbdrn_train_step": (ctypes.c_int, [_NP, _vp, _vp, _i32, _vp, _vp, _vp, _i64, _dbl, _i32, _vp,
                                        _vp, _vp, _sz, _vp]),
}

_NATIVE = Library("liblbdrn_hip.so", "LBDRN_HIP_LIB", "lbdrn_", ABI_VERSION, SIGNATURES, LbdrnError,
                  missing="{path} is missing: build it with `python lbdrn-msic_amd/csrc/build.py` "
                          "(hipcc, gfx950).  This package has no CPU fallback.",
                  mismatch="liblbdrn_hip ABI {got} != {want}")


def lib_path():
    return _NATIVE.path


def lib():
    if _NATIVE.loaded is None:
        import torch
        _NATIVE.lib()
    return _NATIVE.loaded


def check(rc):
    if rc != 0:
        err = LbdrnError(f"liblbdrn_hip error {rc}: {_NATIVE.last_error()}")
        err.code = rc
        raise err
```

lbdrn-msic_amd/lbdrn_hip/codec.py:

```python
import collections
import copy
import os
import threading
import time
from concurrent.futures import ThreadPoolExecutor

import numpy as np
import torch

from . import ops
from .features import FeatCfg
from .model import LBDRNModel
from .sampler import DevicePermutationStream, GPU_RANDPERM_MAX, as_valid_pixels, draw_pass_seeds, epoch_plan, steps_per_epoch as steps_of


def lr_schedule(lr, epochs):
    step = max(1, int(epochs / 3))
    out, cur = [], float(lr)
    for e in range(1, epochs + 1):
        out.append(cur)
        if e % step == 0:
            cur *= 0.1
    return out


def skip_fit_rng(n_feature, base_channel, channels, num_layers, epochs, val_duration=1):
    draw_fit(n_feature, base_channel, channels, num_layers, epochs, val_duration)


class FitDraws:

    def __init__(self, params, train_seeds):
        self.params, self.train_seeds = params, train_seeds


def draw_fit(n_feature, base_channel, channels, num_layers, epochs, val_duration=1):
    model = LBDRNModel(dim_in=n_feature, dim_hidden=base_channel, dim_out=channels, num_layers=num_layers)
    return FitDraws(model.flat_parameters(), draw_pass_seeds(epoch_plan(epochs, val_duration)))


class FitResult:
    def __init__(self):
        self.params = None
        self.best_epoch = -1
        self.best_mse = None
        self.epoch_mse = []
        self.losses = None
        self.msb = None
        self.msb_device = None
        self.msb_max = None
        self.n_feature = None
        self.channels = None
        self.n_subpixels = None
        self.n_valid = None
        self.seconds = {}


class DeviceFit:

    def __init__(self):
        self.best_params = None
        self.msb = None
        self.msb_max = None
        self.geom = None
        self.net = None
        self.mse_log = None
        self.evaluated = []
        self.losses = None
        self.epochs = 0
        self.n_valid = None


_RNG_LOCK = threading.Lock()
_POOL_LOCK = threading.Lock()
_FIT_STREAMS = {}


def _fit_stream_pool(dev, n):
    with _POOL_LOCK:
        pool_ = _FIT_STREAMS.setdefault(dev, [])
        while len(pool_) < n:
            pool_.append(torch.cuda.Stream(device=dev))
        return pool_


def fast_evaluation():
    return os.environ.get("LBDRN_EVAL_CANONICAL") != "1"


def exact16_evaluation():
    return os.environ.get("LBDRN_EVAL_X16") == "1"


def alone_streams_fit_queues():
    return 3 <= int(os.environ.get("GPU_MAX_HW_QUEUES", "4"))


def overlap_evaluation(dev, alone):
    env = os.environ.get("LBDRN_OVERLAP_EVAL")
    if env in ("0", "1"):
        return env == "1"
    if not alone or device_shared():
        return False
    return alone_streams_fit_queues()


def device_shared():
    return os.environ.get("LBDRN_DEVICE_SHARED", "0") not in ("", "0")


def k_per_fit(K, count):
    if isinstance(K, (int, np.integer)):
        return [int(K)] * count
    Ks = [int(k) for k in K]
    if len(Ks) != count:
        raise ValueError(f"{len(Ks)} values of K for {count} images: one K, or one per image")
    return Ks


def image_bytes(C, H, W):
    return C * H * W * 2


def fit_bytes(C, H, W, K, D, base_channel, num_layers, batch_size, epochs, cfg=None):
    if not isinstance(K, (int, np.integer)):
        return max(fit_bytes(C, H, W, int(k), D, base_channel, num_layers, batch_size, epochs, cfg) for k in K)
    cfg = cfg or FeatCfg.from_constants()
    N = H * W
    g = ops._lib.Geom(C, H, W, int(K), D, 1, int(cfg.use_colors), int(cfg.relative), int(cfg.P), 0, None, None)
    net = ops.make_net(cfg.feature_dim(C, D), base_channel, C, num_layers, cfg.act)
    L = ops.lib()
    import ctypes
    train = int(L.lbdrn_train_workspace(ctypes.byref(g), ctypes.byref(net), batch_size))
    apply_ws = int(L.lbdrn_apply_workspace(ctypes.byref(g), ctypes.byref(net)))
    perms = epochs * N * 8 + int(L.lbdrn_randperm_workspace(N, min(32, max(epochs - 1, 1))))
    planes = 3 * C * N * 2
    return train + apply_ws + perms + planes + (epochs + 4) * int(ops.param_count(net)) * 4 + (64 << 20)


def default_in_flight(C, H, W, K, D, base_channel, num_layers, cfg=None, path=None):
    cfg = cfg or FeatCfg.from_constants()
    if path == ops._lib.PATH_GENERIC:
        return 4
    if base_channel >= 128:
        return 3
    return 4


def memory_limited_in_flight(images, wanted, K, D, base_channel, num_layers, batch_size, epochs, cfg=None):
    if not images:
        return wanted
    dev = images[0].device
    Ks = k_per_fit(K, len(images))
    need = max(fit_bytes(*tuple(t.shape), k, D, base_channel, num_layers, batch_size, epochs, cfg) for t, k in zip(images, Ks))
    shared = max(image_bytes(*tuple(t.shape)) for t in images)
    free, total = torch.cuda.mem_get_info(dev)
    free += torch.cuda.memory_reserved(dev) - torch.cuda.memory_allocated(dev)
    if device_shared():
        free //= 2
    keys = [t.data_ptr() if hasattr(t, "data_ptr") else ("entry", k) for k, t in enumerate(images)]
    fits = in_flight_that_fit(keys, need, shared, 0.85 * free, wanted)
    if fits < 1:
        raise ops._lib.LbdrnError(f"one fit of this shape holds {need / 2**30:.1f} GiB on the device, {free / 2**30:.1f} GiB are free "
                                  f"(of {total / 2**30:.0f}): split the image (-sr)")
    return max(1, min(wanted, fits))


def in_flight_that_fit(image_keys, need, shared, budget, wanted):
    for m in range(max(int(wanted), 1), 0, -1):
        run = min(m, len(image_keys))
        distinct = max(len(set(image_keys[k:k + run])) for k in range(len(image_keys) - run + 1)) + m - run
        if m * (need - shared) + distinct * shared <= budget:
            return m
    return 0


EVAL_PASS_FRAC_OF_PEAK, HALF_CHIP_STEP_FRAC_OF_PEAK, HALF_CHIP_STEP_OVERHEAD_S, PEAK_FLOPS = 0.65, 0.26, 5.0e-6, 157.3e12
_HEAD_LOCK = threading.Lock()
_HEAD_MEASURED = {}
_HEAD_PENDING = {}


def _head_key(dev, net, n_pixels, batch_size):
    return (dev.index, int(net.F), int(net.bc), int(net.C), int(net.nl), int(net.act), int(n_pixels), int(batch_size))


def _calibrated_head(key, guess, steps_per_epoch):
    with _HEAD_LOCK:
        pend = _HEAD_PENDING.get(key)
        if pend is not None and pend[0][1].query() and pend[0][3].query():
            (p0, p1, h0, h1), head = pend
            del _HEAD_PENDING[key]
            t_pass, t_head = p0.elapsed_time(p1), h0.elapsed_time(h1)
            if t_pass > 0 and t_head > 0 and head > 0:
                _HEAD_MEASURED[key] = int(round(min(max(head * t_pass / t_head, 0.5 * guess), 2.0 * guess)))
        return max(0, min(steps_per_epoch, _HEAD_MEASURED.get(key, guess)))


def head_calibration():
    with _HEAD_LOCK:
        return dict(_HEAD_MEASURED)


def background_steps(steps_per_epoch, net=None, n_pixels=None, batch_size=None):
    env = os.environ.get("LBDRN_LONE_HEAD_FRAC")
    if env is not None:
        return int(round(float(env) * steps_per_epoch))
    if net is None:
        return int(round(0.27 * steps_per_epoch))
    F, bc, C, nl = int(net.F), int(net.bc), int(net.C), int(net.nl)
    fwd = 2 * (F * bc + (nl - 1) * bc * bc + bc * C)
    step = 2 * fwd + 2 * ((nl - 1) * bc * bc + bc * C)
    t_pass = 2.0 * n_pixels * fwd / (EVAL_PASS_FRAC_OF_PEAK * PEAK_FLOPS)
    t_step = min(batch_size, n_pixels) * step / (HALF_CHIP_STEP_FRAC_OF_PEAK * PEAK_FLOPS) + HALF_CHIP_STEP_OVERHEAD_S
    return max(0, min(steps_per_epoch, int(round(t_pass / t_step))))


def _eval_stream(dev, main):
    for s in _fit_stream_pool(dev, 2):
        if s.cuda_stream != main.cuda_stream:
            return s


def fit_device(img_d, K, D, base_channel, num_layers, lr, batch_size, epochs, val_duration=1,
               cfg=None, path=ops.PATH_AUTO, keep_losses=False, seed=None, draws=None, alone=True, nodata=None):
    cfg = cfg or FeatCfg.from_constants()
    out = DeviceFit()
    dev = img_d.device
    C, H, W = img_d.shape
    N = H * W
    alone = alone and not device_shared()
    msb_d, msb_max = ops.split_bits(img_d, K)
    geom = ops.FeatureGeometry(C, H, W, K, D, msb_max, cfg, dev)
    if N >= GPU_RANDPERM_MAX:
        raise ops._lib.LbdrnError(
            f"{N} pixels in one fit: torch.randperm switches algorithm at 2^32/20 elements and lbdrn_randperm "
            "implements the Fisher-Yates branch only; split the image (-sr) -- there is no host fallback")
    if draws is None:
        with _RNG_LOCK:
            if seed is not None:
                torch.manual_seed(seed)
            draws = draw_fit(geom.F, base_channel, C, num_layers, epochs, val_duration)
    vp = as_valid_pixels(img_d, nodata)
    n_fit = N if vp is None else vp.n
    out.n_valid = None if vp is None else vp.n
    net = ops.make_net(geom.F, base_channel, C, num_layers, cfg.act)
    params = draws.params.to(dev, copy=True).contiguous()
    if params.numel() != ops.param_count(net):
        raise ValueError("draws were made for another network shape")
    steps_per_epoch = steps_of(n_fit, batch_size)
    if n_fit == 0:
        out.best_params, out.msb, out.msb_max, out.geom, out.net = params, msb_d, msb_max, geom, net
        out.mse_log, out.epochs = torch.zeros((epochs, 2), dtype=torch.float32, device=dev), epochs
        out.losses = torch.zeros((epochs, 0), dtype=torch.float32, device=dev) if keep_losses else None
        return out
    stream = DevicePermutationStream(n_fit, epochs, val_duration, dev, train_seeds=draws.train_seeds)
    draws_params0 = params.clone()
    exp_avg = torch.zeros_like(params)
    exp_avg_sq = torch.zeros_like(params)
    lrs = lr_schedule(lr, epochs)
    mean_over = float(N * C) if vp is None else vp.samples.to(torch.float64)
    losses = torch.zeros((epochs, steps_per_epoch), dtype=torch.float32, device=dev) if keep_losses else None
    train_ws = ops.TrainWorkspace(geom, net, batch_size, dev).prepare(img_d, msb_d, path)
    apply_ws = ops.ApplyWorkspace(geom, net, dev)
    mse_log = torch.zeros((epochs, 2), dtype=torch.float32, device=dev)
    eval_epochs = [] if epochs == 1 else [e for e in range(1, epochs + 1) if e % min(val_duration, epochs) == 0]
    main = torch.cuda.current_stream(dev)
    side = _eval_stream(dev, main) if len(eval_epochs) > 1 and overlap_evaluation(dev, alone) else None
    snaps = torch.empty((max(len(eval_epochs), 1), params.numel()), dtype=torch.float32, device=dev)
    mses = torch.zeros((max(len(eval_epochs), 1),), dtype=torch.float32, device=dev)
    if side is not None:
        side.wait_stream(main)
    adam_steps = 0
    hkey = _head_key(dev, net, n_fit, batch_size)
    cal_epoch = eval_epochs[0] if eval_epochs else 0
    cal_events = [torch.cuda.Event(enable_timing=True) for _ in range(4)] if (side is not None and alone and cal_epoch + 1 <= epochs) else None
    try:
        for e in range(1, epochs + 1):
            perm = stream.get(e).to(dev, non_blocking=True)
            if vp is not None:
                perm = vp.gather(perm)
            head = 0
            if side is not None and alone and e - 1 in eval_epochs:
                head = background_steps(steps_per_epoch, net, n_fit, batch_size)
                if "LBDRN_LONE_HEAD_FRAC" not in os.environ:
                    head = _calibrated_head(hkey, head, steps_per_epoch)
            for lo, hi, hint in ((0, head, False), (head, steps_per_epoch, alone)):
                if hi > lo:
                    timed = cal_events is not None and lo == 0 and head > 0 and e == cal_epoch + 1
                    if timed:
                        cal_events[2].record(main)
                    ops.train_epoch(geom, net, img_d, msb_d, perm[lo * batch_size:hi * batch_size], batch_size, params, exp_avg,
                                    exp_avg_sq, adam_steps + lo, lrs[e - 1], losses[e - 1][lo:hi] if keep_losses else None, path,
                                    train_ws, alone=hint)
                    if timed:
                        cal_events[3].record(main)
                        with _HEAD_LOCK:
                            _HEAD_PENDING[hkey] = (cal_events, head)
            adam_steps += steps_per_epoch
            if e in eval_epochs:
                k = eval_epochs.index(e)
                snaps[k].copy_(params)
                if side is not None:
                    side.wait_stream(main)
                with torch.cuda.stream(side if side is not None else main):
                    background = side is not None and e != epochs
                    if cal_events is not None and e == cal_epoch:
                        cal_events[0].record()
                    sse = ops.eval_sse(geom, net, img_d, msb_d, snaps[k], path, apply_ws, background=background,
                                       fast=fast_evaluation(), x16=exact16_evaluation(),
                                       nodata=None if vp is None else vp.value)
                    if cal_events is not None and e == cal_epoch:
                        cal_events[1].record()
                    mses[k:k + 1].copy_((sse / mean_over).float())
                out.evaluated.append(e)
    finally:
        if side is not None:
            main.wait_stream(side)
    best_params = params.clone() if epochs == 1 else draws_params0
    best_mse = torch.full((1,), 1e6, dtype=torch.float32, device=dev)
    for k, e in enumerate(eval_epochs):
        mse = mses[k:k + 1]
        improved = mse < best_mse
        best_params = torch.where(improved, snaps[k], best_params)
        best_mse = torch.where(improved, mse, best_mse)
        mse_log[e - 1, 0] = mse[0]
        mse_log[e - 1, 1] = improved[0].float()
    stream.close()
    out.best_params, out.msb, out.msb_max, out.geom, out.net = best_params, msb_d, msb_max, geom, net
    out.mse_log, out.losses, out.epochs = mse_log, losses, epochs
    return out


def fit_group(imgs_d, K, D, base_channel, num_layers, lr, batch_size, epochs, val_duration=1, cfg=None,
              path=ops.PATH_AUTO, keep_losses=False, seed=None, draws=None, nodata=None):
    cfg = cfg or FeatCfg.from_constants()
    G = len(imgs_d)
    Ks = k_per_fit(K, G)
    vps = valid_pixels_per_fit(imgs_d, nodata)
    dev = imgs_d[0].device
    C, H, W = imgs_d[0].shape
    if any(tuple(t.shape) != (C, H, W) for t in imgs_d):
        raise ValueError("the fits of a group must have one raster shape")
    N = H * W
    if N >= GPU_RANDPERM_MAX:
        raise ops._lib.LbdrnError(f"{N} pixels in one fit: split the image (-sr)")
    if len({None if vp is None else vp.n for vp in vps}) > 1:
        raise ValueError("the fits of a group must have one n_valid: " + ", ".join(str(None if vp is None else vp.n) for vp in vps))
    n_fit = N if vps[0] is None else vps[0].n
    if n_fit == 0:
        return [fit_device(img_d, K_, D, base_channel, num_layers, lr, batch_size, epochs, val_duration, cfg, path, keep_losses,
                           seed, draws[k] if draws is not None else None, alone=False, nodata=vp)
                for k, (img_d, K_, vp) in enumerate(zip(imgs_d, Ks, vps))]
    outs = [DeviceFit() for _ in range(G)]
    st = []
    net = None
    streams = {}
    for k, (img_d, K) in enumerate(zip(imgs_d, Ks)):
        msb_d, msb_max = ops.split_bits(img_d, K)
        geom = ops.FeatureGeometry(C, H, W, K, D, msb_max, cfg, dev)
        dr = draws[k] if draws is not None else None
        if dr is None:
            with _RNG_LOCK:
                if seed is not None:
                    torch.manual_seed(seed)
                dr = draw_fit(geom.F, base_channel, C, num_layers, epochs, val_duration)
        net = ops.make_net(geom.F, base_channel, C, num_layers, cfg.act)
        params = dr.params.to(dev, copy=True).contiguous()
        if params.numel() != ops.param_count(net):
            raise ValueError("draws were made for another network shape")
        steps = steps_of(n_fit, batch_size)
        seeds = tuple(int(s_) for s_ in dr.train_seeds)
        if seeds not in streams:
            streams[seeds] = DevicePermutationStream(n_fit, epochs, val_duration, dev, train_seeds=seeds)
        vp = vps[k]
        st.append(dict(
            vp=vp, mean_over=float(N * C) if vp is None else vp.samples.to(torch.float64),
            img=img_d, msb=msb_d, msb_max=msb_max, geom=geom, params=params, params0=params.clone(),
            m=torch.zeros_like(params), v=torch.zeros_like(params),
            perms=streams[seeds],
            losses=torch.zeros((epochs, steps), dtype=torch.float32, device=dev) if keep_losses else None,
            tws=ops.TrainWorkspace(geom, net, batch_size, dev).prepare(img_d, msb_d, path),
            aws=ops.ApplyWorkspace(geom, net, dev)))
    lrs = lr_schedule(lr, epochs)
    steps_per_epoch = steps_of(n_fit, batch_size)
    eval_epochs = [] if epochs == 1 else [e for e in range(1, epochs + 1) if e % min(val_duration, epochs) == 0]
    for f in st:
        f["snaps"] = torch.empty((max(len(eval_epochs), 1), f["params"].numel()), dtype=torch.float32, device=dev)
        f["mses"] = torch.zeros((max(len(eval_epochs), 1),), dtype=torch.float32, device=dev)
    adam_steps = 0
    for e in range(1, epochs + 1):
        of_stream = {id(ps): ps.get(e).to(dev, non_blocking=True) for ps in streams.values()}
        gathered = {}
        perms = []
        for f in st:
            key = (id(f["perms"]), id(f["vp"]))
            if key not in gathered:
                perm = of_stream[id(f["perms"])]
                gathered[key] = perm if f["vp"] is None else f["vp"].gather(perm)
            perms.append(gathered[key])
        ops.train_epoch_group([f["geom"] for f in st], net, [f["img"] for f in st], [f["msb"] for f in st], perms,
                              batch_size, [f["params"] for f in st], [f["m"] for f in st], [f["v"] for f in st],
                              adam_steps, lrs[e - 1], [f["losses"][e - 1] for f in st] if keep_losses else None,
                              path, [f["tws"] for f in st])
        adam_steps += steps_per_epoch
        if e in eval_epochs:
            k = eval_epochs.index(e)
            for f, out in zip(st, outs):
                f["snaps"][k].copy_(f["params"])
                sse = ops.eval_sse(f["geom"], net, f["img"], f["msb"], f["snaps"][k], path, f["aws"], fast=fast_evaluation(), x16=exact16_evaluation(),
                                   nodata=None if f["vp"] is None else f["vp"].value)
                f["mses"][k:k + 1].copy_((sse / f["mean_over"]).float())
                out.evaluated.append(e)
    for f, out in zip(st, outs):
        best_params = f["params"].clone() if epochs == 1 else f["params0"]
        best_mse = torch.full((1,), 1e6, dtype=torch.float32, device=dev)
        mse_log = torch.zeros((epochs, 2), dtype=torch.float32, device=dev)
        for k, e in enumerate(eval_epochs):
            mse = f["mses"][k:k + 1]
            improved = mse < best_mse
            best_params = torch.where(improved, f["snaps"][k], best_params)
            best_mse = torch.where(improved, mse, best_mse)
            mse_log[e - 1, 0] = mse[0]
            mse_log[e - 1, 1] = improved[0].float()
        out.best_params, out.msb, out.msb_max, out.geom, out.net = best_params, f["msb"], f["msb_max"], f["geom"], net
        out.mse_log, out.losses, out.epochs = mse_log, f["losses"], epochs
        out.n_valid = None if f["vp"] is None else f["vp"].n
    for ps in streams.values():
        ps.close()
    return outs


def fit_many(images, K, D, base_channel, num_layers, lr, batch_size, epochs, val_duration=1, cfg=None,
             path=ops.PATH_AUTO, seed=19920517, in_flight=None, then=None, draws=None, group=None, nodata=None):
    Ks = k_per_fit(K, len(images))
    vps = valid_pixels_per_fit(images, nodata)
    K = Ks[0] if Ks else K
    if in_flight is None:
        in_flight = default_in_flight(*tuple(images[0].shape), K, D, base_channel, num_layers, cfg, path) if images else 4
    in_flight = memory_limited_in_flight(images, in_flight, Ks, D, base_channel, num_layers, batch_size, epochs, cfg)
    if group is None:
        group = int(os.environ.get("LBDRN_FIT_GROUP", "0"))
        if group == 0:
            group = 1
            if in_flight >= 4 and images:
                C, H, W = images[0].shape
                fcfg = cfg or FeatCfg.from_constants()
                if ops.train_group_size(C, H, W, K, D, fcfg, base_channel, num_layers) >= 2 and path != ops._lib.PATH_GENERIC:
                    group = 2
    group = max(1, min(group, in_flight, ops.train_group_max()))
    if draws is not None:
        seed = None
        if len(draws) != len(images):
            raise ValueError("one FitDraws per image expected")
    elif seed is None and in_flight > 1 and len(images) > 1:
        raise ValueError("fits in flight together must seed themselves (seed=...) or bring their draws: "
                         "they share one generator")
    caller = torch.cuda.current_stream(images[0].device) if images else None
    local = threading.local()
    taken = []

    def work(job):
        idx, imgs, drs, ks = job
        if not hasattr(local, "stream"):
            with _POOL_LOCK:
                k = len(taken)
                taken.append(None)
            local.stream = _fit_stream_pool(imgs[0].device, k + 1)[k]
            local.stream.wait_stream(caller)
        with torch.cuda.stream(local.stream):
            if len(imgs) == 1:
                fits = [fit_device(imgs[0], ks[0], D, base_channel, num_layers, lr, batch_size, epochs, val_duration, cfg,
                                   path, seed=seed, draws=drs[0], alone=False, nodata=vps[idx[0]])]
            else:
                fits = fit_group(imgs, ks, D, base_channel, num_layers, lr, batch_size, epochs, val_duration, cfg, path,
                                 seed=seed, draws=drs if draws is not None else None, nodata=[vps[i] for i in idx])
            outs = [then(fit) if then is not None else fit for fit in fits]
            done = torch.cuda.Event()
            done.record(local.stream)
        return idx, outs, done

    drs_all = draws if draws is not None else [None] * len(images)
    if in_flight <= 1 or len(images) <= 1:
        results = []
        for img_d, dr, k_, vp in zip(images, drs_all, Ks, vps):
            fit = fit_device(img_d, k_, D, base_channel, num_layers, lr, batch_size, epochs, val_duration, cfg, path,
                             seed=seed, draws=dr, nodata=vp)
            results.append(then(fit) if then is not None else fit)
        return results
    n_valid = [None if vp is None else vp.n for vp in vps]
    jobs = form_jobs(images, drs_all, Ks, group, n_valid)
    if group > 1 and 2 * sum(len(j[0]) for j in jobs if len(j[0]) > 1) < len(images):
        group = 1
        jobs = form_jobs(images, drs_all, Ks, 1, n_valid)
    with ThreadPoolExecutor(max_workers=max(1, in_flight // group)) as pool:
        done_jobs = list(pool.map(work, jobs))
    results = [None] * len(images)
    for idx, outs, done in done_jobs:
        caller.wait_event(done)
        for i, o in zip(idx, outs):
            results[i] = o
    return results


def valid_pixels_per_fit(images, nodata):
    if not isinstance(nodata, (list, tuple)):
        nodata = [nodata] * len(images)
    if len(nodata) != len(images):
        raise ValueError(f"{len(nodata)} nodata entries for {len(images)} images: one, or one per image")
    formed, out = {}, []
    for img, nd in zip(images, nodata):
        if nd is not None and not hasattr(nd, "idx"):
            key = (id(img), int(nd))
            if key not in formed:
                formed[key] = as_valid_pixels(img, int(nd))
            nd = formed[key]
        out.append(nd)
    return out


def form_jobs(images, draws, Ks, group, n_valid=None):
    if n_valid is None:
        n_valid = [None] * len(images)
    jobs, k = [], 0
    while k < len(images):
        n = 1
        while (n < group and k + n < len(images) and tuple(images[k + n].shape) == tuple(images[k].shape)
               and n_valid[k + n] == n_valid[k]):
            n += 1
        jobs.append((list(range(k, k + n)), list(images[k:k + n]), list(draws[k:k + n]), list(Ks[k:k + n])))
        k += n
    return jobs


def truncate_device(params, precision):
    if precision in (0, 32):
        return params.clone()
    mask = -(1 << (32 - precision))
    return (params.view(torch.int32) & mask).view(torch.float32)


def apply_device(geom, net, msb_d, params_d, path=ops.PATH_AUTO, ws=None, want_y=False):
    return ops.decode_fused(geom, net, msb_d, params_d, want_y=want_y, path=path, ws=ws)


def _host_result(fit, epochs, seconds, host_msb):
    res = FitResult()
    res.seconds = dict(seconds)
    mse_host = fit.mse_log.cpu().numpy()
    if epochs == 1:
        res.best_epoch = 1
    for e in fit.evaluated:
        res.epoch_mse.append((e, float(mse_host[e - 1, 0]), bool(mse_host[e - 1, 1] > 0)))
        if mse_host[e - 1, 1] > 0:
            res.best_epoch, res.best_mse = e, float(mse_host[e - 1, 0])
    if epochs > 1 and fit.evaluated and res.best_epoch < 0:
        worst = [m for _, m, _ in res.epoch_mse]
        raise ops._lib.LbdrnError(
            f"no evaluation pass improved on the initial best MSE of 1e6 (per-epoch MSE {worst}): the fit diverged or "
            "the input is degenerate (e.g. an all-zero MSB plane gives 0/0 features); no bitstream is written")
    res.params = fit.best_params.cpu().numpy()
    res.msb_device = fit.msb
    if host_msb:
        msb = ops.from_device_u16(fit.msb)
        res.msb = msb.astype(np.uint16) if fit.msb_max > 255 else msb.astype(np.uint8)
    res.msb_max = fit.msb_max
    C, H, W = fit.msb.shape
    res.n_feature, res.channels, res.n_subpixels = fit.geom.F, C, H * W * C
    res.losses = fit.losses
    res.n_valid = fit.n_valid
    return res


def _as_planes(img):
    img = np.ascontiguousarray(img, dtype=np.uint16)
    return img[None] if img.ndim == 2 else img


def fit_image(img, K, D, base_channel, num_layers, lr, batch_size, epochs, val_duration=1, cfg=None,
              device="cuda:0", path=ops.PATH_AUTO, keep_losses=False, host_msb=True, draws=None, nodata=None):
    t0 = time.time()
    img_d = ops.to_device_u16(_as_planes(img), torch.device(device))
    t1 = time.time()
    fit = fit_device(img_d, K, D, base_channel, num_layers, lr, batch_size, epochs, val_duration, cfg,
                     path, keep_losses, draws=draws, nodata=nodata)
    res = _host_result(fit, epochs, {"upload": t1 - t0}, host_msb)
    res.seconds["fit"] = time.time() - t1
    return res


def fit_images(imgs, K, D, base_channel, num_layers, lr, batch_size, epochs, val_duration=1, cfg=None,
               device="cuda:0", path=ops.PATH_AUTO, host_msb=True, draws=None, seed=None, in_flight=None, errors="raise",
               nodata=None):
    t0 = time.time()
    dev = torch.device(device)
    uploaded = {}
    for img in imgs:
        if id(img) not in uploaded:
            uploaded[id(img)] = ops.to_device_u16(_as_planes(img), dev)
    tiles = [uploaded[id(img)] for img in imgs]
    t1 = time.time()
    fits = fit_many(tiles, K, D, base_channel, num_layers, lr, batch_size, epochs, val_duration, cfg, path,
                    seed=seed, in_flight=in_flight, draws=draws, nodata=nodata)
    results = []
    for fit in fits:
        try:
            results.append(_host_result(fit, epochs, {"upload": (t1 - t0) / max(len(imgs), 1)}, host_msb))
        except Exception as e:
            if errors != "return":
                raise
            results.append(e)
    per_tile = (time.time() - t1) / max(len(imgs), 1)
    for res in results:
        if not isinstance(res, Exception):
            res.seconds["fit"] = per_tile
    return results


def apply_image(base, params, K, D, base_channel, num_layers, cfg=None, device="cuda:0",
                path=ops.PATH_AUTO, want_y=False, keep_on_device=False):
    cfg = cfg or FeatCfg.from_constants()
    dev = torch.device(device)
    if isinstance(base, torch.Tensor):
        msb_d = base if base.dim() == 3 else base[None]
        msb_max = int((msb_d.to(torch.int32) & 0xFFFF).max().item())
    else:
        base = np.ascontiguousarray(base).astype(np.uint16)
        if base.ndim == 2:
            base = base[None]
        msb_d = ops.to_device_u16(base, dev)
        msb_max = int(base.max())
    C, H, W = msb_d.shape
    geom = ops.FeatureGeometry(C, H, W, K, D, msb_max, cfg, dev)
    net = ops.make_net(geom.F, base_channel, C, num_layers, cfg.act)
    p = torch.from_numpy(np.ascontiguousarray(params, dtype=np.float32)).to(dev)
    if p.numel() != ops.param_count(net):
        raise ValueError(f"weight payload has {p.numel()} values, the network needs {ops.param_count(net)}")
    out = ops.decode_fused(geom, net, msb_d, p, want_y=want_y, path=path)
    if keep_on_device:
        return out
    if want_y:
        return ops.from_device_u16(out[0]), out[1].cpu().numpy()
    return ops.from_device_u16(out)



def _closed_loop_recon(fit_result, img, nn_payload, K, D, base_channel, num_layers, cfg, device, path):
    from . import container
    cfg = cfg or FeatCfg.from_constants()
    dev = torch.device(device)
    msb_d = fit_result.msb_device
    C, H, W = msb_d.shape
    orig_d = ops.to_device_u16(_as_planes(img), dev)
    if tuple(orig_d.shape) != (C, H, W):
        raise ValueError(f"the original is {tuple(orig_d.shape)}, the fit's planes are {(C, H, W)}")
    geom = ops.FeatureGeometry(C, H, W, K, D, fit_result.msb_max, cfg, dev)
    net = ops.make_net(geom.F, base_channel, C, num_layers, cfg.act)
    params = container.decode_weights(nn_payload, expected=ops.param_count(net))
    p = torch.from_numpy(np.ascontiguousarray(params, dtype=np.float32)).to(dev)
    return orig_d, ops.decode_fused(geom, net, msb_d, p, path=path).contiguous()


def closed_loop_sse(fit_result, img, nn_payload, K, D, base_channel, num_layers, cfg=None, device="cuda:0",
                    path=ops.PATH_AUTO):
    from . import container
    cfg = cfg or FeatCfg.from_constants()
    dev = torch.device(device)
    msb_d = fit_result.msb_device
    C, H, W = msb_d.shape
    orig_d = ops.to_device_u16(_as_planes(img), dev)
    if tuple(orig_d.shape) != (C, H, W):
        raise ValueError(f"the original is {tuple(orig_d.shape)}, the fit's planes are {(C, H, W)}")
    geom = ops.FeatureGeometry(C, H, W, K, D, fit_result.msb_max, cfg, dev)
    net = ops.make_net(geom.F, base_channel, C, num_layers, cfg.act)
    params = container.decode_weights(nn_payload, expected=ops.param_count(net))
    p = torch.from_numpy(np.ascontiguousarray(params, dtype=np.float32)).to(dev)
    sse = float(ops.eval_sse(geom, net, orig_d, msb_d, p, path=path, decoded=True).item())
    if not (sse < 2.0 ** 53 and sse == int(sse)):
        raise ops._lib.LbdrnError(f"closed-loop SSE {sse!r} is not an exact integer below 2^53")
    return int(sse)


def residual_encode(fit_result, tau, img, nn_payload, K, D, base_channel, num_layers, cfg=None, device="cuda:0",
                    path=ops.PATH_AUTO, nodata=None):
    from . import resid
    orig_d, recon = _closed_loop_recon(fit_result, img, nn_payload, K, D, base_channel, num_layers, cfg, device, path)
    if nodata is not None:
        from . import nodata as nd
        V, kind, mask_body = nodata
        body = resid.encode(nd.merge_original(orig_d, recon, V), recon, nd.tau_for(tau, V))
        check = nd.apply(resid.apply(body, recon.clone()), kind, mask_body, V)
        try:
            return body, nd.check(orig_d, check, V, tau)
        except ValueError as e:
            raise ops._lib.LbdrnError(str(e)) from None
    body = resid.encode(orig_d, recon, tau)
    check = resid.apply(body, recon.clone())
    err = int((orig_d.to(torch.int32) & 0xFFFF).sub_(check.to(torch.int32) & 0xFFFF).abs_().max().item())
    if err > tau:
        raise ops._lib.LbdrnError(f"residual layer: max error {err} after decoding the body, {tau} was asked for; no bitstream is written")
    return body, err


def nodata_verify(fit_result, nodata, img, nn_payload, K, D, base_channel, num_layers, cfg=None, device="cuda:0", path=ops.PATH_AUTO):
    from . import nodata as nd
    orig_d, recon = _closed_loop_recon(fit_result, img, nn_payload, K, D, base_channel, num_layers, cfg, device, path)
    V, kind, mask_body = nodata
    try:
        return nd.check(orig_d, nd.apply(recon, kind, mask_body, V), V)
    except ValueError as e:
        raise ops._lib.LbdrnError(str(e)) from None


def residual_apply(body, recon_d, rect=None):
    from . import resid
    return resid.apply(body, recon_d, rect)



WindowPiece = collections.namedtuple(
    "WindowPiece", "tile tx ty tw th xa xb ya yb left right top bottom ox oy")
WindowPiece.__doc__ = """The part of a window that lies in one tile.  tile: index in tile_windows order; (tx, ty, tw, th): the
tile in scene pixels; [xa,xb) x [ya,yb): the window clipped to the tile, in TILE pixels; left / right / top / bottom: the
margin of MSB samples taken around it (D, clipped to the tile's own edges); (ox, oy): where the piece goes in the window."""


def check_window(window, width, height):
    try:
        x0, y0, w, h = (int(v) for v in window)
    except (TypeError, ValueError):
        raise ValueError(f"window {window!r}: four integers (x0, y0, w, h) expected") from None
    if w < 1 or h < 1:
        raise ValueError(f"window x0={x0} y0={y0} w={w} h={h} is empty (the scene is {width} x {height})")
    if x0 < 0 or y0 < 0 or x0 + w > width or y0 + h > height:
        raise ValueError(f"window x0={x0} y0={y0} w={w} h={h} is not inside the {width} x {height} scene")
    return x0, y0, w, h


def window_pieces(width, height, split_ratio, window, D):
    from LBDRNdataset import tile_windows
    x0, y0, w, h = check_window(window, width, height)
    pieces = []
    for t, (_, _, tx, ty, tw, th) in enumerate(tile_windows(width, height, split_ratio)):
        xa, xb = max(x0, tx) - tx, min(x0 + w, tx + tw) - tx
        ya, yb = max(y0, ty) - ty, min(y0 + h, ty + th) - ty
        if xa >= xb or ya >= yb:
            continue
        pieces.append(WindowPiece(t, tx, ty, tw, th, xa, xb, ya, yb, min(D, xa), min(D, tw - xb), min(D, ya),
                                  min(D, th - yb), tx + xa - x0, ty + ya - y0))
    return pieces


def decode_window_pieces(bitstream, window, device="cuda:0", path=ops.PATH_AUTO, cfg=None, take=None, enhance=True, mask=True):
    from . import container
    from .features import window_tables
    bitstream = bytes(bitstream) if not isinstance(bitstream, (bytes, memoryview)) else bitstream
    n_hdr, split_ratio, width, height, K, bc, nl, D, nn_list, base_list = container.unpack_header(bitstream)
    pieces = window_pieces(width, height, split_ratio, window, D)
    cfg = copy.copy(cfg) if cfg is not None else FeatCfg.from_constants()
    activation = container.header_activation(bitstream)
    if activation is not None:
        cfg.activation = activation
    dev = torch.device(device)
    layer = container.unpack_residual_trailer(bitstream) if enhance else None
    nodata = container.unpack_nodata_trailer(bitstream) if mask else None
    offsets = [n_hdr]
    for t in range(split_ratio * split_ratio):
        offsets.append(offsets[-1] + nn_list[t] + base_list[t])
    out = []
    for k, pc in enumerate(pieces):
        if take is not None and not take(k, pc):
            continue
        off = offsets[pc.tile]
        nn_payload = bitstream[off:off + nn_list[pc.tile]]
        base_payload = bitstream[off + nn_list[pc.tile]:offsets[pc.tile + 1]]
        base = container.decode_base(bytes(base_payload), device=device, keep_on_device=True)
        if not isinstance(base, torch.Tensor):
            base = np.ascontiguousarray(base).astype(np.uint16)
            base = ops.to_device_u16(base[None] if base.ndim == 2 else base, dev)
        msb_d = base if base.dim() == 3 else base[None]
        C, H, W = msb_d.shape
        if (H, W) != (pc.th, pc.tw):
            raise ValueError(f"tile {pc.tile}: the MSB payload is {W} x {H}, the header's tile is {pc.tw} x {pc.th}")
        msb_max = int((msb_d.to(torch.int32) & 0xFFFF).max().item())
        need = ops.param_count(ops.make_net(cfg.feature_dim(C, D), bc, C, nl))
        params = container.decode_weights(bytes(nn_payload), expected=need)
        rows, cols = (pc.ya - pc.top, pc.yb + pc.bottom), (pc.xa - pc.left, pc.xb + pc.right)
        crop = msb_d[:, rows[0]:rows[1], cols[0]:cols[1]].contiguous()
        geom = ops.FeatureGeometry(C, rows[1] - rows[0], cols[1] - cols[0], K, D, msb_max, cfg, dev,
                                   tables=window_tables(H, W, cfg, rows, cols))
        net = ops.make_net(geom.F, bc, C, nl, cfg.act)
        p = torch.from_numpy(np.ascontiguousarray(params, dtype=np.float32)).to(dev)
        rec = ops.decode_fused(geom, net, crop, p, path=path)
        rec = rec[:, pc.top:pc.top + pc.yb - pc.ya, pc.left:pc.left + pc.xb - pc.xa]
        if layer is not None:
            rec = residual_apply(layer[1][pc.tile], rec.contiguous(), (pc.xa, pc.ya, pc.xb - pc.xa, pc.yb - pc.ya))
        if nodata is not None:
            from . import nodata as nd
            rec = nd.apply(rec.contiguous(), *nodata[1][pc.tile], nodata[0], (pc.xa, pc.ya, pc.xb - pc.xa, pc.yb - pc.ya))
        out.append((pc, rec))
    return (width, height), out


def decode_window(bitstream, window, device="cuda:0", path=ops.PATH_AUTO, cfg=None, keep_on_device=True, enhance=True, mask=True):
    _, parts = decode_window_pieces(bitstream, window, device, path, cfg, enhance=enhance, mask=mask)
    x0, y0, w, h = (int(v) for v in window)
    out = None
    for pc, rec in parts:
        if out is None:
            out = torch.empty((rec.shape[0], h, w), dtype=rec.dtype, device=rec.device)
        out[:, pc.oy:pc.oy + rec.shape[1], pc.ox:pc.ox + rec.shape[2]] = rec
    return out if keep_on_device else ops.from_device_u16(out)
```

lbdrn-msic_amd/lbdrn_hip/ops.py:

```python
import ctypes

import numpy as np
import torch

from . import _lib
from ._lib import EVAL_BACKGROUND, EVAL_DECODED, EVAL_FAST, EVAL_VALID, EVAL_X16, TRAIN_ALONE, Geom, Net, PATH_AUTO, check, lib


def _call(fn, ref, *args):
    dev = ref.device if isinstance(ref, torch.Tensor) else torch.device(ref)
    if dev.type != "cuda":
        raise _lib.LbdrnError("liblbdrn_hip works on device (HBM) tensors only; there is no CPU path in this package")
    with torch.cuda.device(dev):
        check(fn(*args, ctypes.c_void_p(torch.cuda.current_stream(dev).cuda_stream)))


def _ptr(t):
    return ctypes.c_void_p(t.data_ptr()) if t is not None else None


def _need_cuda(*ts):
    for t in ts:
        if t is not None and not t.is_cuda:
            raise _lib.LbdrnError("liblbdrn_hip works on device (HBM) tensors only; there is no "
                                  "CPU path in this package")


def _u16(t):
    if t.dtype == torch.uint16:
        return t.view(torch.int16)
    assert t.dtype == torch.int16, t.dtype
    return t


class FeatureGeometry:

    def __init__(self, C, H, W, K, D, msb_max, cfg, device, tables=None):
        from .features import pos_tables
        self.C, self.H, self.W, self.K, self.D, self.msb_max = C, H, W, K, D, int(msb_max)
        self.cfg = cfg
        rowtab, coltab = tables if tables is not None else pos_tables(H, W, cfg)
        if rowtab.shape != (H, cfg.P) or coltab.shape != (W, cfg.P):
            raise ValueError(f"positional tables {rowtab.shape}, {coltab.shape} for a {H} x {W} raster with P = {cfg.P}")
        self.P = rowtab.shape[1]
        self.rowtab = torch.from_numpy(rowtab).to(device) if self.P else None
        self.coltab = torch.from_numpy(coltab).to(device) if self.P else None
        self.F = cfg.feature_dim(C, D)
        self.c = Geom(C, H, W, K, D, int(msb_max), int(cfg.use_colors), int(cfg.relative), self.P,
                      0, self.rowtab.data_ptr() if self.P else None,
                      self.coltab.data_ptr() if self.P else None)

    def with_max(self, msb_max):
        self.msb_max = int(msb_max)
        self.c.msb_max = int(msb_max)
        return self


ACT_SINE, ACT_RELU = 0, 1


def make_net(F, bc, C, nl, act=ACT_SINE):
    return Net(F, bc, C, nl, act)


def param_count(net):
    return int(lib().lbdrn_param_count(ctypes.byref(net)))


def split_bits(img, K):
    _need_cuda(img)
    img = _u16(img.contiguous())
    C, H, W = img.shape
    msb = torch.empty_like(img)
    mx = torch.zeros(1, dtype=torch.int32, device=img.device)
    _call(lib().lbdrn_split_bits, img, _ptr(img), C, H, W, K, _ptr(msb), _ptr(mx))
    return msb, int(mx.item())


def labels(img, K, idx=None):
    _need_cuda(img, idx)
    img = _u16(img.contiguous())
    C, H, W = img.shape
    n = H * W if idx is None else idx.numel()
    out = torch.empty((n, C), dtype=torch.float32, device=img.device)
    if idx is not None:
        idx = idx.to(torch.int64).contiguous()
    _call(lib().lbdrn_labels, img, _ptr(img), C, H, W, K, _ptr(idx), n, _ptr(out))
    return out


def features(geom, msb, idx=None):
    _need_cuda(msb, idx)
    msb = _u16(msb.contiguous())
    n = geom.H * geom.W if idx is None else idx.numel()
    out = torch.empty((n, geom.F), dtype=torch.float32, device=msb.device)
    if idx is not None:
        idx = idx.to(torch.int64).contiguous()
    _call(lib().lbdrn_features, msb, ctypes.byref(geom.c), _ptr(msb), _ptr(idx), n, _ptr(out))
    return out


def forward(net, params, x):
    _need_cuda(params, x)
    x = x.contiguous().float()
    params = params.contiguous().float()
    B = x.shape[0]
    assert x.shape[1] == net.F and params.numel() == param_count(net)
    y = torch.empty((B, net.C), dtype=torch.float32, device=x.device)
    nbytes = lib().lbdrn_forward_workspace(ctypes.byref(net), B)
    ws = torch.empty(max(nbytes, 1), dtype=torch.uint8, device=x.device)
    _call(lib().lbdrn_forward, x, ctypes.byref(net), _ptr(params), _ptr(x), B, _ptr(y), _ptr(ws), nbytes)
    return y


def forward_tape(net, params, x):
    _need_cuda(params, x)
    x = x.contiguous().float()
    params = params.contiguous().float()
    B = x.shape[0]
    assert x.shape[1] == net.F and params.numel() == param_count(net)
    y = torch.empty((B, net.C), dtype=torch.float32, device=x.device)
    nbytes = lib().lbdrn_tape_bytes(ctypes.byref(net), B)
    tape = torch.empty(max(nbytes, 1), dtype=torch.uint8, device=x.device)
    _call(lib().lbdrn_forward_tape, x, ctypes.byref(net), _ptr(params), _ptr(x), B, _ptr(y), _ptr(tape), nbytes)
    return y, tape


def backward(net, params, x, tape, y, dy, want_dx=False):
    _need_cuda(params, x, tape, y, dy)
    x = x.contiguous().float()
    params = params.contiguous().float()
    dy = dy.contiguous().float()
    B = x.shape[0]
    assert x.shape[1] == net.F and params.numel() == param_count(net)
    assert y.shape == (B, net.C) and dy.shape == (B, net.C) and y.is_contiguous()
    grads = torch.empty(param_count(net), dtype=torch.float32, device=x.device)
    dx = torch.empty((B, net.F), dtype=torch.float32, device=x.device) if want_dx else None
    nbytes = lib().lbdrn_backward_workspace(ctypes.byref(net), B)
    ws = torch.empty(max(nbytes, 1), dtype=torch.uint8, device=x.device)
    _call(lib().lbdrn_backward, x, ctypes.byref(net), _ptr(params), _ptr(x), B, _ptr(tape), tape.numel(), _ptr(y),
          _ptr(dy), _ptr(grads), _ptr(dx), _ptr(ws), nbytes)
    return grads, dx


class ApplyWorkspace:
    def __init__(self, geom, net, device):
        self.nbytes = lib().lbdrn_apply_workspace(ctypes.byref(geom.c), ctypes.byref(net))
        self.buf = torch.empty(max(self.nbytes, 1), dtype=torch.uint8, device=device)


def decode_fused(geom, net, msb, params, want_y=False, path=PATH_AUTO, ws=None):
    _need_cuda(msb, params)
    msb = _u16(msb.contiguous())
    params = params.contiguous().float()
    out = torch.empty_like(msb)
    y = torch.empty((geom.H * geom.W, geom.C), dtype=torch.float32, device=msb.device) if want_y else None
    ws = ws or ApplyWorkspace(geom, net, msb.device)
    _call(lib().lbdrn_decode_fused, msb, ctypes.byref(geom.c), ctypes.byref(net), _ptr(msb), _ptr(params),
                                   _ptr(out), _ptr(y), _ptr(ws.buf), ws.nbytes, path)
    return (out, y) if want_y else out


def eval_sse(geom, net, img, msb, params, path=PATH_AUTO, ws=None, out=None, background=False, fast=False, x16=False,
             nodata=None, decoded=False):
    _need_cuda(img, msb, params)
    img = _u16(img.contiguous())
    msb = _u16(msb.contiguous())
    params = params.contiguous().float()
    sse = out if out is not None else torch.zeros(1, dtype=torch.float64, device=msb.device)
    ws = ws or ApplyWorkspace(geom, net, msb.device)
    gc = geom.c
    if nodata is not None:
        gc = Geom.from_buffer_copy(geom.c)
        gc.reserved = int(nodata)
    _call(lib().lbdrn_eval_sse, msb, ctypes.byref(gc), ctypes.byref(net), _ptr(img), _ptr(msb),
                               _ptr(params), _ptr(sse), _ptr(ws.buf), ws.nbytes,
                               path | (EVAL_BACKGROUND if background else 0) | (EVAL_FAST if fast else 0) |
                               (EVAL_X16 if (fast and x16) else 0) | (EVAL_VALID if nodata is not None else 0) |
                               (EVAL_DECODED if decoded else 0))
    return sse


class TrainWorkspace:

    def __init__(self, geom, net, batch_size, device):
        self.geom, self.net, self.batch_size = geom, net, batch_size
        self.nbytes = lib().lbdrn_train_workspace(ctypes.byref(geom.c), ctypes.byref(net), batch_size)
        self.buf = torch.empty(max(self.nbytes, 1), dtype=torch.uint8, device=device)
        self.prepared_for = None

    def prepare(self, img, msb, path=PATH_AUTO):
        img, msb = _u16(img.contiguous()), _u16(msb.contiguous())
        _call(lib().lbdrn_train_prepare, img, ctypes.byref(self.geom.c), ctypes.byref(self.net), _ptr(img),
                                        _ptr(msb), self.batch_size, _ptr(self.buf), self.nbytes, path)
        self.prepared_for = self.key(img, path, self.geom)
        return self

    @staticmethod
    def key(img, path, geom):
        return (img.data_ptr(), path, int(geom.c.K), int(geom.c.D), int(geom.c.msb_max))


def train_epoch(geom, net, img, msb, perm, batch_size, params, exp_avg, exp_avg_sq, adam_step0, lr,
                losses=None, path=PATH_AUTO, ws=None, alone=False):
    _need_cuda(img, msb, perm, params, exp_avg, exp_avg_sq, losses)
    img = _u16(img.contiguous())
    msb = _u16(msb.contiguous())
    assert perm.dtype == torch.int64 and perm.is_contiguous()
    for t in (params, exp_avg, exp_avg_sq):
        assert t.dtype == torch.float32 and t.is_contiguous()
    if ws is None:
        ws = TrainWorkspace(geom, net, batch_size, img.device).prepare(img, msb, path)
    if ws.prepared_for != TrainWorkspace.key(img, path, geom):
        raise _lib.LbdrnError("TrainWorkspace.prepare(img, msb, path) must run once for this image first")
    _call(lib().lbdrn_train_epoch, img, ctypes.byref(geom.c), ctypes.byref(net), _ptr(img), _ptr(msb),
                                  _ptr(perm), perm.numel(), batch_size, _ptr(params), _ptr(exp_avg),
                                  _ptr(exp_avg_sq), adam_step0, float(lr), _ptr(losses), _ptr(ws.buf),
                                  ws.nbytes, path | (TRAIN_ALONE if alone else 0))


def train_group_max():
    return int(lib().lbdrn_train_group_max())


def train_group_size(C, H, W, K, D, cfg, base_channel, num_layers):
    g = Geom(C, H, W, K, D, 1, int(cfg.use_colors), int(cfg.relative), int(cfg.P), 0, None, None)
    net = Net(cfg.feature_dim(C, D), base_channel, C, num_layers, cfg.act)
    return int(lib().lbdrn_train_group_size(ctypes.byref(g), ctypes.byref(net)))


def train_step_features(geom, net):
    return int(lib().lbdrn_train_step_features(ctypes.byref(geom.c), ctypes.byref(net)))


def train_epoch_group(geoms, net, imgs, msbs, perms, batch_size, params, exp_avgs, exp_avg_sqs, adam_step0, lr,
                      losses=None, path=PATH_AUTO, wss=None):
    n = len(imgs)
    _need_cuda(*imgs, *msbs, *perms, *params, *exp_avgs, *exp_avg_sqs)
    imgs = [_u16(t.contiguous()) for t in imgs]
    msbs = [_u16(t.contiguous()) for t in msbs]
    for t in perms:
        assert t.dtype == torch.int64 and t.is_contiguous() and t.numel() == perms[0].numel()
    for t in list(params) + list(exp_avgs) + list(exp_avg_sqs):
        assert t.dtype == torch.float32 and t.is_contiguous()
    for ws, img, geom in zip(wss, imgs, geoms):
        if ws.prepared_for != TrainWorkspace.key(img, path, geom) or ws.nbytes != wss[0].nbytes:
            raise _lib.LbdrnError("every fit of a group needs its own TrainWorkspace, prepared for its image")
    arr = lambda ptrs: (ctypes.c_void_p * n)(*ptrs)
    garr = (ctypes.POINTER(Geom) * n)(*[ctypes.pointer(g.c) for g in geoms])
    larr = arr([_ptr(t) for t in losses]) if losses is not None else None
    _call(lib().lbdrn_train_epoch_group, imgs[0], n, ctypes.cast(garr, ctypes.c_void_p), ctypes.byref(net),
          arr([_ptr(t) for t in imgs]), arr([_ptr(t) for t in msbs]), arr([_ptr(t) for t in perms]),
          perms[0].numel(), batch_size, arr([_ptr(t) for t in params]), arr([_ptr(t) for t in exp_avgs]),
          arr([_ptr(t) for t in exp_avg_sqs]), adam_step0, float(lr), larr, arr([_ptr(w.buf) for w in wss]),
          wss[0].nbytes, path)


def train_profile_mode(mode):
    check(lib().lbdrn_train_profile_mode(int(mode)))


def train_step(net, x, t, params, exp_avg, exp_avg_sq, adam_step, lr, apply_adam=True):
    _need_cuda(x, t, params)
    x = x.contiguous().float()
    t = t.contiguous().float()
    B = x.shape[0]
    loss = torch.zeros(1, dtype=torch.float32, device=x.device)
    grads = torch.empty_like(params)
    g = Geom(net.C, 1, 1, 1, 0, 1, 1, 1, 0, 0, None, None)
    nbytes = lib().lbdrn_train_workspace(ctypes.byref(g), ctypes.byref(net), B)
    ws = torch.empty(max(nbytes, 1), dtype=torch.uint8, device=x.device)
    _call(lib().lbdrn_train_step, x, ctypes.byref(net), _ptr(x), _ptr(t), B, _ptr(params), _ptr(exp_avg),
                                 _ptr(exp_avg_sq), adam_step, float(lr), int(apply_adam), _ptr(loss),
                                 _ptr(grads), _ptr(ws), nbytes)
    return loss, grads


def randperm(seeds, n, device):
    scalar = isinstance(seeds, int)
    seeds = [seeds] if scalar else list(seeds)
    out = torch.empty((len(seeds), n), dtype=torch.int64, device=device)
    for c0 in range(0, len(seeds), 32):
        chunk = seeds[c0:c0 + 32]
        arr = (ctypes.c_uint64 * len(chunk))(*[s & 0xFFFFFFFFFFFFFFFF for s in chunk])
        nbytes = lib().lbdrn_randperm_workspace(n, len(chunk))
        ws = torch.empty(max(nbytes, 1), dtype=torch.uint8, device=device)
        _call(lib().lbdrn_randperm, out, arr, len(chunk), n, _ptr(out[c0:]), _ptr(ws), nbytes)
    return out[0] if scalar else out


def plane_encode(planes):
    _need_cuda(planes)
    planes = _u16(planes.contiguous())
    C, H, W = planes.shape
    dev = planes.device
    body = torch.empty(lib().lbdrn_plane_bound(C, H, W), dtype=torch.uint8, device=dev)
    nbytes = torch.zeros(1, dtype=torch.int64, device=dev)
    ws = torch.empty(max(lib().lbdrn_plane_workspace(C, H, W), 1), dtype=torch.uint8, device=dev)
    _call(lib().lbdrn_plane_encode, planes, _ptr(planes), C, H, W, _ptr(body), body.numel(), _ptr(nbytes), _ptr(ws),
                                   ws.numel())
    return body[:int(nbytes.item())].cpu().numpy().tobytes()


def jp2k_encode(planes, bits, out=None):
    _need_cuda(planes)
    planes = _u16(planes.contiguous())
    C, H, W = planes.shape
    dev = planes.device
    cap = lib().lbdrn_jp2k_bound(C, H, W)
    if not cap:
        raise _lib.LbdrnError(f"lbdrn_jp2k_encode: geometry {C} x {H} x {W} is not supported")
    if out is None:
        out = np.empty(cap, np.uint8)
    n = ctypes.c_size_t()
    ws = torch.empty(max(lib().lbdrn_jp2k_workspace(C, H, W), 1), dtype=torch.uint8, device=dev)
    _call(lib().lbdrn_jp2k_encode, planes, _ptr(planes), C, H, W, int(bits), out.ctypes.data_as(ctypes.c_void_p), out.size,
                                  ctypes.byref(n), _ptr(ws), ws.numel())
    return out[:n.value].tobytes()


def plane_decode(body, C, H, W, device):
    raw = torch.frombuffer(bytearray(body), dtype=torch.uint8).to(device)
    planes = torch.empty((C, H, W), dtype=torch.int16, device=device)
    status = torch.zeros(1, dtype=torch.int32, device=device)
    ws = torch.empty(max(lib().lbdrn_plane_workspace(C, H, W), 1), dtype=torch.uint8, device=device)
    _call(lib().lbdrn_plane_decode, planes, _ptr(raw), raw.numel(), C, H, W, _ptr(planes), _ptr(status), _ptr(ws),
                                   ws.numel())
    if int(status.item()):
        raise _lib.LbdrnError("LBB2 payload is inconsistent with its geometry (corrupt or truncated stream)")
    return planes


def to_device_u16(arr, device):
    a = np.ascontiguousarray(arr, dtype=np.uint16)
    return torch.from_numpy(a.view(np.int16)).to(device)


def from_device_u16(t):
    return t.cpu().numpy().view(np.uint16)
```

Before: 71.63 Mpixels/s.

## Prebuild reflect-padded float planes for evaluation passes and stage tiles from them

Adds a one-time kernel that builds reflect-padded, normalized float planes of the MSB image per tile. A new evaluation kernel variant stages its LDS tiles from these planes instead of gathering uint16 pixels with reflection arithmetic and conversion on every eval pass. The planes are cached per image/version in the apply workspace and are used for the EVAL and EVAL_FAST modes, since evaluation runs several times per fit. The cost is extra device memory for the planes and a build pass per tile, plus more code paths to keep in sync.

```diff
diff --git a/include/lbdrn_hip.h b/include/lbdrn_hip.h
--- a/include/lbdrn_hip.h
+++ b/include/lbdrn_hip.h
@@ -84,6 +84,14 @@
                    const uint16_t *msb, const float *params, double *sse, void *workspace,
                    size_t workspace_bytes, int32_t path, void *stream);
 
+size_t lbdrn_eval_planes_bytes(const lbdrn_geom *g);
+int lbdrn_eval_planes_build(const lbdrn_geom *g, const uint16_t *img, const uint16_t *msb, void *planes,
+                            size_t planes_bytes, void *stream);
+int lbdrn_eval_sse_planes(const lbdrn_geom *g, const lbdrn_net *net, const uint16_t *img,
+                          const uint16_t *msb, const float *params, double *sse, void *workspace,
+                          size_t workspace_bytes, int32_t path, void *stream, const void *planes,
+                          size_t planes_bytes);
+
 #define LBDRN_APPLY_DECODE 0x2000
 int lbdrn_apply_instance(const lbdrn_geom *g, const lbdrn_net *net, int32_t path_word, int32_t *out);
 
diff --git a/lbdrn-msic_amd/csrc/apply_mfma.hip b/lbdrn-msic_amd/csrc/apply_mfma.hip
--- a/lbdrn-msic_amd/csrc/apply_mfma.hip
+++ b/lbdrn-msic_amd/csrc/apply_mfma.hip
@@ -229,6 +229,8 @@
     int nodata;
     int decoded;
     unsigned long long* stamps;
+    const float* pw;
+    int pw_rows, pw_pitch;
 };
 
 #ifdef LBDRN_APPLY_STAMPS
@@ -359,317 +361,19 @@
 template <int NT, int MODE, bool RELU>
 __global__ void __launch_bounds__(APPLY_THREADS) k_apply_mfma(ApplyArgs A)
 {
-    extern __shared__ __attribute__((aligned(16))) float lds[];
-    const lbdrn_geom& g = A.g;
-    const ApplyPlan& p = A.p;
-    const int tid = threadIdx.x;
-    const int lane = tid & 63, wave = tid >> 6;
-    const int j = lane & 31, h = lane >> 5;
-    const int half = A.net.bc / 2;
-    const int P = g.P, D = g.D, C = g.C;
-
-    for (int e = tid * 4; e < p.pack_floats; e += APPLY_THREADS * 4) {
-        if (e + 3 < p.pack_floats) {
-            *reinterpret_cast<float4*>(lds + e) = *reinterpret_cast<const float4*>(A.packed + e);
-        } else {
-            for (int q = e; q < p.pack_floats; ++q) lds[q] = A.packed[q];
-        }
-    }
-    int* ktab = reinterpret_cast<int*>(lds + p.off_ktab);
-    {
-        const int side = 2 * D + 1, plane = p.SH * p.SW;
-        for (int k = tid; k < 2 * (p.S0 - P) + 1; k += APPLY_THREADS) {
-            int kk = min(k, p.ncolor - 1);
-            kk = max(kk, 0);
-            int c = kk / (side * side), r = kk - c * side * side;
-            int dy = r / side, dx = r - dy * side;
-            ktab[2 * k] = c * plane + (dy - D) * p.SW + (dx - D);
-            ktab[2 * k + 1] = c * plane;
-        }
-    }
-    const float* w0 = lds + p.off_w0;
-    const float* wh = lds + p.off_wh;
-    const float* wl = lds + p.off_wl;
-    const float* bh = lds + p.off_bh;
-    const float* bl = lds + p.off_bl;
-    float* rowt = lds + p.off_rowt;
-    float* colt = lds + p.off_colt;
-    float* tile = lds + p.off_tile;
-    const bool rel = g.relative && D > 0;
-    const float maxf = (float)g.msb_max;
-    const int64_t HW = (int64_t)g.H * g.W;
-    const float scale = (float)((1 << g.K) - 1);
-    const int lmask = (1 << g.K) - 1;
-#ifdef LBDRN_APPLY_STAMPS
-    unsigned long long acc_t[8] = {}, last_t;
-    asm volatile("s_memtime %0\n\ts_waitcnt lgkmcnt(0)" : "=s"(last_t)::"memory");
-#endif
-    const int ntiles = p.tiles_x * p.tiles_y;
-    for (int v = blockIdx.x; v < A.nvirt; v += gridDim.x) {
-    double sse = 0.0;
-    for (int t = v; t < ntiles; t += A.nvirt) {
-        const int ty = t / p.tiles_x, tx = t - ty * p.tiles_x;
-        const int y0 = ty * p.TH, x0 = tx * TILE_W;
-        __syncthreads();
-        if (g.use_colors) {
-            const int plane = p.SH * p.SW, total = C * plane;
-            const unsigned msw = 0xFFFFFFFFu / (unsigned)p.SW + 1u, msh = 0xFFFFFFFFu / (unsigned)p.SH + 1u;
-            const bool simple = D < g.H && D < g.W && total < 65536 && p.SH > 1;
-            constexpr int UB = 8;
-            for (int base = 0; base < total; base += APPLY_THREADS * UB) {
-                unsigned short raw[UB];
-#pragma unroll
-                for (int u = 0; u < UB; ++u) {
-                    const int e = min(base + u * APPLY_THREADS + tid, total - 1);
-                    int row, sx, c, sy, yy, xx;
-                    if (simple) {
-                        row = (int)__umulhi((unsigned)e, msw); sx = e - row * p.SW;
-                        c = (int)__umulhi((unsigned)row, msh); sy = row - c * p.SH;
-                        yy = y0 + sy - D; xx = x0 + sx - D;
-                        yy = yy < 0 ? -yy : yy; yy = yy >= g.H ? 2 * (g.H - 1) - yy : yy;
-                        xx = xx < 0 ? -xx : xx; xx = xx >= g.W ? 2 * (g.W - 1) - xx : xx;
-                        yy = max(0, min(yy, g.H - 1));
-                        xx = max(0, min(xx, g.W - 1));
-                    } else {
-                        row = e / p.SW; sx = e - row * p.SW; c = row / p.SH; sy = row - c * p.SH;
-                        yy = reflect_idx(y0 + sy - D, g.H); xx = reflect_idx(x0 + sx - D, g.W);
-                    }
-                    raw[u] = mode_fast(MODE) ? (unsigned short)(A.img[(int64_t)c * HW + (int64_t)yy * g.W + xx] >> g.K)
-                                             : A.msb[(int64_t)c * HW + (int64_t)yy * g.W + xx];
-                }
-#pragma unroll
-                for (int u = 0; u < UB; ++u) {
-                    const int e = base + u * APPLY_THREADS + tid;
-                    if (e < total) tile[e] = MODE == MODE_EVAL_X16 ? (float)raw[u] : (float)raw[u] / maxf;
-                }
-            }
-        }
-        for (int e = tid; e < p.TH * P; e += APPLY_THREADS) {
-            int yy = min(y0 + e / P, g.H - 1);
-            rowt[e] = g.rowtab[(int64_t)yy * P + e % P];
-        }
-        for (int e = tid; e < TILE_W * P; e += APPLY_THREADS) {
-            int xx = min(x0 + e / P, g.W - 1);
-            colt[e] = g.coltab[(int64_t)xx * P + e % P];
-        }
-        __syncthreads();
-
-        ASTAMP(0);
-        const int nseg = p.TH * (TILE_W / 32);
-        for (int seg = wave; seg < nseg; seg += APPLY_WAVES) {
-            const int ly = seg / (TILE_W / 32), lx = (seg % (TILE_W / 32)) * 32;
-            const int pixbase = (ly + D) * p.SW + (lx + j + D);
-            const int yy = y0 + ly, xx = x0 + lx + j;
-            const bool inside = yy < g.H && xx < g.W;
-            const int64_t pix = (int64_t)min(yy, g.H - 1) * g.W + min(xx, g.W - 1);
-            const int nreg = 4 * ((C + 7) / 8);
-            unsigned short pre[16];
-            {
-                const uint16_t* src = (MODE == MODE_DECODE) ? A.msb : A.img;
-#pragma unroll
-                for (int r = 0; r < 16; ++r) {
-                    pre[r] = 0;
-                    if (r < nreg) pre[r] = src[(int64_t)min(acc_row(r, h), C - 1) * HW + pix];
-                }
-            }
-            f32x16 acc[NT];
-            f32x16 hid[NT];
-#pragma unroll
-            for (int tt = 0; tt < NT; ++tt)
-#pragma unroll
-                for (int q4 = 0; q4 < 4; ++q4) {
-                    float4 b4 = *reinterpret_cast<const float4*>(bh + (tt * 2 + h) * 16 + q4 * 4);
-                    acc[tt][q4 * 4 + 0] = b4.x; acc[tt][q4 * 4 + 1] = b4.y;
-                    acc[tt][q4 * 4 + 2] = b4.z; acc[tt][q4 * 4 + 3] = b4.w;
-                }
-            if constexpr (MODE == MODE_EVAL_X16) {
-                f32x16 bias0[NT];
-#pragma unroll
-                for (int tt = 0; tt < NT; ++tt) {
-                    bias0[tt] = acc[tt];
-#pragma unroll
-                    for (int r = 0; r < 16; ++r) acc[tt][r] = 0.0f;
-                }
-                const int plane = p.SH * p.SW;
-                const float* tp = tile + h * (C / 2) * plane + ly * p.SW + lx + j;
-                const float* wc = w0 + (size_t)lane * NT * 4;
-                const size_t wstep = (size_t)p.M16 * X16_PIECES * 64 * NT * 4;
-                for (int c = 0; c < C / 2; ++c, tp += plane, wc += wstep) {
-                    if (D == 1) layer0_pair_x16<NT, 1>(acc, wc, tp);
-                    else if (D == 2) layer0_pair_x16<NT, 2>(acc, wc, tp);
-                    else layer0_pair_x16<NT, 3>(acc, wc, tp);
-                }
-                const float cs = lds[p.off_scale];
-#pragma unroll
-                for (int tt = 0; tt < NT; ++tt)
-#pragma unroll
-                    for (int r = 0; r < 16; ++r) acc[tt][r] = fmaf(acc[tt][r], cs, bias0[tt][r]);
-            }
-            for (int s = 0; s < (MODE == MODE_EVAL_X16 ? 0 : P); ++s) {
-                int k = 2 * s + h;
-                float b = (k < P) ? rowt[ly * P + k] : colt[(lx + j) * P + (k - P)];
-                float a[NT];
-                load_a<NT>(w0, s * 64 + lane, a);
-#pragma unroll
-                for (int tt = 0; tt < NT; ++tt)
-                    acc[tt] = __builtin_amdgcn_mfma_f32_32x32x2f32(a[tt], b, acc[tt], 0, 0, 0);
-            }
-            bool paired = MODE == MODE_EVAL_X16;
-            if constexpr (MODE == MODE_EVAL_FAST) {
-                if (p.pair) {
-                    paired = true;
-                    const int plane = p.SH * p.SW;
-                    const float* tp = tile + h * (C / 2) * plane + ly * p.SW + lx + j;
-                    const float* wc = w0 + ((size_t)P * 64 + lane) * NT;
-                    for (int c = 0; c < C / 2; ++c, tp += plane, wc += (size_t)p.RS * 64 * NT) {
-                        if (rel) {
-                            if (D == 1) layer0_pair<NT, 1, true>(acc, wc, tp);
-                            else if (D == 2) layer0_pair<NT, 2, true>(acc, wc, tp);
-                            else layer0_pair<NT, 3, true>(acc, wc, tp);
-                        } else {
-                            if (D == 1) layer0_pair<NT, 1, false>(acc, wc, tp);
-                            else if (D == 2) layer0_pair<NT, 2, false>(acc, wc, tp);
-                            else layer0_pair<NT, 3, false>(acc, wc, tp);
-                        }
-                    }
-                }
-            }
-            if (!paired) {
-                constexpr int CH = APPLY_CHUNK;
-                static_assert(CH % 4 == 0, "the steps left behind the chunks are taken four at a time");
-                int s4 = P;
-                for (; s4 + CH <= p.S0; s4 += CH) {
-                    float bq[CH];
-#pragma unroll
-                    for (int u = 0; u < CH; ++u) {
-                        const int kk = 2 * (s4 + u - P) + h;
-                        const int2 e = *reinterpret_cast<const int2*>(ktab + 2 * kk);
-                        const float nb = tile[pixbase + e.x];
-                        const float ct = tile[pixbase + e.y];
-                        bq[u] = rel ? nb - ct : nb;
-                    }
-                    __builtin_amdgcn_sched_barrier(0);
-#pragma unroll
-                    for (int u = 0; u < CH; ++u) {
-                        float a[NT];
-                        load_a<NT>(w0, (s4 + u) * 64 + lane, a);
-#pragma unroll
-                        for (int tt = 0; tt < NT; ++tt)
-                            acc[tt] = __builtin_amdgcn_mfma_f32_32x32x2f32(a[tt], bq[u], acc[tt], 0, 0, 0);
-                    }
-                    __builtin_amdgcn_sched_barrier(0);
-                }
-                for (; s4 < p.S0; s4 += 4) {
-                    float bq[4];
-                    float aq[4][NT];
-#pragma unroll
-                    for (int u = 0; u < 4; ++u) {
-                        int kk = 2 * (s4 + u - P) + h;
-                        int2 e = *reinterpret_cast<const int2*>(ktab + 2 * kk);
-                        float nb = tile[pixbase + e.x];
-                        float ct = tile[pixbase + e.y];
-                        bq[u] = rel ? nb - ct : nb;
-                        load_a<NT>(w0, (s4 + u) * 64 + lane, aq[u]);
-                    }
-#pragma unroll
-                    for (int u = 0; u < 4; ++u)
-#pragma unroll
-                        for (int tt = 0; tt < NT; ++tt)
-                            acc[tt] = __builtin_amdgcn_mfma_f32_32x32x2f32(aq[u][tt], bq[u], acc[tt], 0, 0, 0);
-                }
-            }
-            ASTAMP(1);
-#pragma unroll
-            for (int tt = 0; tt < NT; ++tt)
-#pragma unroll
-                for (int r = 0; r < 16; ++r) hid[tt][r] = apply_hidden_act<MODE, RELU>(acc[tt][r]);
-            ASTAMP(2);
-            for (int l = 1; l < A.net.nl; ++l) {
-                const float* wlayer = wh + (size_t)(l - 1) * half * 64 * NT;
-#pragma unroll
-                for (int tt = 0; tt < NT; ++tt)
-#pragma unroll
-                    for (int q4 = 0; q4 < 4; ++q4) {
-                        float4 b4 = *reinterpret_cast<const float4*>(bh + ((l * NT + tt) * 2 + h) * 16 + q4 * 4);
-                        acc[tt][q4 * 4 + 0] = b4.x; acc[tt][q4 * 4 + 1] = b4.y;
-                        acc[tt][q4 * 4 + 2] = b4.z; acc[tt][q4 * 4 + 3] = b4.w;
-                    }
-#pragma unroll
-                for (int s = 0; s < NT * 16; ++s) {
-                    float b = hid[s / 16][s % 16];
-                    float a[NT];
-                    load_a<NT>(wlayer, s * 64 + lane, a);
-#pragma unroll
-                    for (int tt = 0; tt < NT; ++tt)
-                        acc[tt] = __builtin_amdgcn_mfma_f32_32x32x2f32(a[tt], b, acc[tt], 0, 0, 0);
-                }
-#pragma unroll
-                for (int tt = 0; tt < NT; ++tt)
-#pragma unroll
-                    for (int r = 0; r < 16; ++r) hid[tt][r] = apply_hidden_act<MODE, RELU>(acc[tt][r]);
-            }
-            ASTAMP(3);
-            f32x16 o;
-            if (mode_fast(MODE)) {
-                if (C > 4) last_layer_4x4<NT, 2>(o, hid, wl, bl, lane);
-                else last_layer_4x4<NT, 1>(o, hid, wl, bl, lane);
-            } else {
-#pragma unroll
-                for (int q4 = 0; q4 < 4; ++q4) {
-                    float4 b4 = *reinterpret_cast<const float4*>(bl + h * 16 + q4 * 4);
-                    o[q4 * 4 + 0] = b4.x; o[q4 * 4 + 1] = b4.y; o[q4 * 4 + 2] = b4.z; o[q4 * 4 + 3] = b4.w;
-                }
-#pragma unroll
-                for (int s = 0; s < NT * 16; ++s) {
-                    float b = hid[s / 16][s % 16];
-                    float a = wl[s * 64 + lane];
-                    o = __builtin_amdgcn_mfma_f32_32x32x2f32(a, b, o, 0, 0, 0);
-                }
-            }
-            ASTAMP(4);
-#pragma unroll
-            for (int r = 0; r < 16; ++r) {
-                const int ch = acc_row(r, h);
-                if (r < nreg && ch < C && inside) {
-                    float yv = mode_fast(MODE) ? fast_sigmoid(o[r]) : canon_sigmoid(o[r]);
-                    if (MODE == MODE_DECODE) {
-                        float rr = __builtin_rintf(yv * scale);
-                        int base = (int)pre[r] << g.K;
-                        A.out[(int64_t)ch * HW + pix] = (uint16_t)(base + (int)rr);
-                        if (A.y_out) A.y_out[pix * C + ch] = yv;
-                    } else if ((int)pre[r] != A.nodata) {
-                        if (MODE == MODE_EVAL && A.decoded) {
-                            int band = ch;
-                            asm volatile("" : "+v"(band));
-                            sse += decoded_term((int)pre[r], (int)A.msb[(int64_t)band * HW + pix], yv, scale, g.K);
-                            continue;
-                        }
-                        float lab = (float)((int)pre[r] & lmask) / scale;
-                        float d = yv - lab;
-                        sse += (double)(d * d);
-                    }
-                }
-            }
-            ASTAMP(5);
-        }
-    }
-    if (MODE != MODE_DECODE) {
-        __syncthreads();
-        double* red = reinterpret_cast<double*>(lds + ((p.off_rowt + 3) & ~3));
-        red[tid] = sse;
-        __syncthreads();
-        for (int o2 = APPLY_THREADS / 2; o2 > 0; o2 >>= 1) {
-            if (tid < o2) red[tid] += red[tid + o2];
-            __syncthreads();
-        }
-        if (tid == 0) A.partial[v] = red[0];
-    }
-    }
-#ifdef LBDRN_APPLY_STAMPS
-    if (tid == 0 && A.stamps)
-        for (int k = 0; k < 8; ++k) A.stamps[(size_t)blockIdx.x * 8 + k] = acc_t[k];
-#endif
-}
+    constexpr bool PLANES = false;
+#include "apply_pass.inc"
+}
+
+template <int NT, int MODE, bool RELU>
+__global__ void __launch_bounds__(APPLY_THREADS) k_apply_planes(ApplyArgs A)
+{
+    static_assert(MODE == MODE_EVAL || MODE == MODE_EVAL_FAST, "the planes serve the two float-staging evaluation modes");
+    constexpr bool PLANES = true;
+#include "apply_pass.inc"
+}
+
+#include "eval_planes.inc"
 
 __global__ void k_sum_partials_mfma(const double* __restrict__ partial, int n, double* dst)
 {
@@ -725,6 +429,17 @@
     return 0;
 }
 
+template <int NT, int MODE>
+static int launch_apply_row(const ApplyArgs& A, bool relu, int grid, hipStream_t s, bool whole_lds)
+{
+    if constexpr (MODE == MODE_EVAL || MODE == MODE_EVAL_FAST)
+        if (A.pw)
+            return relu ? launch_pass<k_apply_planes<NT, MODE, true>, APPLY_THREADS, true>(A, grid, s, whole_lds)
+                        : launch_pass<k_apply_planes<NT, MODE, false>, APPLY_THREADS, true>(A, grid, s, whole_lds);
+    return relu ? launch_pass<k_apply_mfma<NT, MODE, true>, APPLY_THREADS, true>(A, grid, s, whole_lds)
+                : launch_pass<k_apply_mfma<NT, MODE, false>, APPLY_THREADS, true>(A, grid, s, whole_lds);
+}
+
 static int dispatch_apply(const ApplyArgs& A, int mode, int grid, hipStream_t s, bool whole_lds)
 {
     const bool relu = A.net.act == LBDRN_ACT_RELU;
@@ -732,10 +447,7 @@
         set_error("the fast instances of the fused apply pass take at most 8 bands, not %d", A.net.C);
         return LBDRN_E_UNSUPPORTED;
     }
-#define X(nt, m)                                                                                                       \
-    if (A.p.NT == nt && mode == m)                                                                                     \
-        return relu ? launch_pass<k_apply_mfma<nt, m, true>, APPLY_THREADS, true>(A, grid, s, whole_lds)               \
-                    : launch_pass<k_apply_mfma<nt, m, false>, APPLY_THREADS, true>(A, grid, s, whole_lds);
+#define X(nt, m) if (A.p.NT == nt && mode == m) return launch_apply_row<nt, m>(A, relu, grid, s, whole_lds);
     APPLY_INSTANCES(X)
 #undef X
     set_error("no fused apply pass is built for NT = %d, mode %d", A.p.NT, mode);
@@ -767,6 +479,7 @@
     size_t ws_bytes;
     bool background;
     hipStream_t s;
+    const void* planes = nullptr;
 };
 
 static int workspace_holds(const ApplyCall& c, size_t need)
@@ -912,6 +625,14 @@
     }
     k_pack_apply<<<(A.p.pack_floats + 255) / 256, 256, 0, c.s>>>(c.params, net, A.p, g.P, g.C, g.msb_max, amax, packed);
     LBDRN_LAUNCH_CHECK();
+    A.pw = nullptr;
+    A.pw_rows = A.pw_pitch = 0;
+    if (c.planes && (mode == MODE_EVAL || mode == MODE_EVAL_FAST)) {
+        const EvalPlanes L = eval_planes_layout(g);
+        A.pw = (const float*)c.planes;
+        A.pw_rows = L.Hp;
+        A.pw_pitch = L.pitch;
+    }
     return run_pass(A, c, mode, packed, partial, dispatch_apply);
 }
 
@@ -923,9 +644,9 @@
 
 int mfma_eval_sse(const lbdrn_geom& g, const lbdrn_net& net, const uint16_t* img,
                   const uint16_t* msb, const float* params, double* sse, void* ws, size_t ws_bytes,
-                  bool background, bool fast, bool x16, int nodata, bool decoded, hipStream_t s)
-{
-    return run_apply({g, net, img, msb, params, nullptr, nullptr, sse, nodata, decoded, ws, ws_bytes, background, s},
+                  bool background, bool fast, bool x16, int nodata, bool decoded, hipStream_t s, const void* planes)
+{
+    return run_apply({g, net, img, msb, params, nullptr, nullptr, sse, nodata, decoded, ws, ws_bytes, background, s, planes},
                      fast ? (x16 ? MODE_EVAL_X16 : MODE_EVAL_FAST) : MODE_EVAL);
 }
 
diff --git a/lbdrn-msic_amd/csrc/apply_pass.inc b/lbdrn-msic_amd/csrc/apply_pass.inc
--- /dev/null
+++ b/lbdrn-msic_amd/csrc/apply_pass.inc
@@ -0,0 +1,348 @@
+    extern __shared__ __attribute__((aligned(16))) float lds[];
+    const lbdrn_geom& g = A.g;
+    const ApplyPlan& p = A.p;
+    const int tid = threadIdx.x;
+    const int lane = tid & 63, wave = tid >> 6;
+    const int j = lane & 31, h = lane >> 5;
+    const int half = A.net.bc / 2;
+    const int P = g.P, D = g.D, C = g.C;
+
+    for (int e = tid * 4; e < p.pack_floats; e += APPLY_THREADS * 4) {
+        if (e + 3 < p.pack_floats) {
+            *reinterpret_cast<float4*>(lds + e) = *reinterpret_cast<const float4*>(A.packed + e);
+        } else {
+            for (int q = e; q < p.pack_floats; ++q) lds[q] = A.packed[q];
+        }
+    }
+    int* ktab = reinterpret_cast<int*>(lds + p.off_ktab);
+    {
+        const int side = 2 * D + 1, plane = p.SH * p.SW;
+        for (int k = tid; k < 2 * (p.S0 - P) + 1; k += APPLY_THREADS) {
+            int kk = min(k, p.ncolor - 1);
+            kk = max(kk, 0);
+            int c = kk / (side * side), r = kk - c * side * side;
+            int dy = r / side, dx = r - dy * side;
+            ktab[2 * k] = c * plane + (dy - D) * p.SW + (dx - D);
+            ktab[2 * k + 1] = c * plane;
+        }
+    }
+    const float* w0 = lds + p.off_w0;
+    const float* wh = lds + p.off_wh;
+    const float* wl = lds + p.off_wl;
+    const float* bh = lds + p.off_bh;
+    const float* bl = lds + p.off_bl;
+    float* rowt = lds + p.off_rowt;
+    float* colt = lds + p.off_colt;
+    float* tile = lds + p.off_tile;
+    const bool rel = g.relative && D > 0;
+    const float maxf = (float)g.msb_max;
+    const int64_t HW = (int64_t)g.H * g.W;
+    const float scale = (float)((1 << g.K) - 1);
+    const int lmask = (1 << g.K) - 1;
+#ifdef LBDRN_APPLY_STAMPS
+    unsigned long long acc_t[8] = {}, last_t;
+    asm volatile("s_memtime %0\n\ts_waitcnt lgkmcnt(0)" : "=s"(last_t)::"memory");
+#endif
+    const int ntiles = p.tiles_x * p.tiles_y;
+    for (int v = blockIdx.x; v < A.nvirt; v += gridDim.x) {
+    double sse = 0.0;
+    for (int t = v; t < ntiles; t += A.nvirt) {
+        const int ty = t / p.tiles_x, tx = t - ty * p.tiles_x;
+        const int y0 = ty * p.TH, x0 = tx * TILE_W;
+        __syncthreads();
+        if constexpr (PLANES) {
+            if (g.use_colors) {
+                const int V = (p.SW & 3) ? 2 : 4, PR = p.SW / V, total = C * p.SH * PR;
+                const unsigned mpr = 0xFFFFFFFFu / (unsigned)PR + 1u, msh = 0xFFFFFFFFu / (unsigned)p.SH + 1u;
+                const float* ring = A.pw + (int64_t)y0 * A.pw_pitch + x0;
+                const bool pairs = (p.off_tile & 1) == 0;
+                constexpr int UB = 8;
+                for (int base = 0; base < total; base += APPLY_THREADS * UB) {
+                    float4 v[UB];
+                    int o[UB];
+#pragma unroll
+                    for (int u = 0; u < UB; ++u) {
+                        const int q = min(base + u * APPLY_THREADS + tid, total - 1);
+                        const int row = (int)__umulhi((unsigned)q, mpr), col = (q - row * PR) * V;
+                        const int c = p.SH > 1 ? (int)__umulhi((unsigned)row, msh) : row, sy = row - c * p.SH;
+                        const float* sp = ring + ((int64_t)c * A.pw_rows + sy) * A.pw_pitch + col;
+                        o[u] = row * p.SW + col;
+                        if (V == 4) {
+                            v[u] = *reinterpret_cast<const float4*>(sp);
+                        } else {
+                            const float2 t2 = *reinterpret_cast<const float2*>(sp);
+                            v[u] = make_float4(t2.x, t2.y, 0.0f, 0.0f);
+                        }
+                    }
+#pragma unroll
+                    for (int u = 0; u < UB; ++u) {
+                        if (base + u * APPLY_THREADS + tid >= total) continue;
+                        float* d = tile + o[u];
+                        if (pairs) {
+                            *reinterpret_cast<float2*>(d) = make_float2(v[u].x, v[u].y);
+                            if (V == 4) *reinterpret_cast<float2*>(d + 2) = make_float2(v[u].z, v[u].w);
+                        } else {
+                            d[0] = v[u].x; d[1] = v[u].y;
+                            if (V == 4) { d[2] = v[u].z; d[3] = v[u].w; }
+                        }
+                    }
+                }
+            }
+        } else if (g.use_colors) {
+            const int plane = p.SH * p.SW, total = C * plane;
+            const unsigned msw = 0xFFFFFFFFu / (unsigned)p.SW + 1u, msh = 0xFFFFFFFFu / (unsigned)p.SH + 1u;
+            const bool simple = D < g.H && D < g.W && total < 65536 && p.SH > 1;
+            constexpr int UB = 8;
+            for (int base = 0; base < total; base += APPLY_THREADS * UB) {
+                unsigned short raw[UB];
+#pragma unroll
+                for (int u = 0; u < UB; ++u) {
+                    const int e = min(base + u * APPLY_THREADS + tid, total - 1);
+                    int row, sx, c, sy, yy, xx;
+                    if (simple) {
+                        row = (int)__umulhi((unsigned)e, msw); sx = e - row * p.SW;
+                        c = (int)__umulhi((unsigned)row, msh); sy = row - c * p.SH;
+                        yy = y0 + sy - D; xx = x0 + sx - D;
+                        yy = yy < 0 ? -yy : yy; yy = yy >= g.H ? 2 * (g.H - 1) - yy : yy;
+                        xx = xx < 0 ? -xx : xx; xx = xx >= g.W ? 2 * (g.W - 1) - xx : xx;
+                        yy = max(0, min(yy, g.H - 1));
+                        xx = max(0, min(xx, g.W - 1));
+                    } else {
+                        row = e / p.SW; sx = e - row * p.SW; c = row / p.SH; sy = row - c * p.SH;
+                        yy = reflect_idx(y0 + sy - D, g.H); xx = reflect_idx(x0 + sx - D, g.W);
+                    }
+                    raw[u] = mode_fast(MODE) ? (unsigned short)(A.img[(int64_t)c * HW + (int64_t)yy * g.W + xx] >> g.K)
+                                             : A.msb[(int64_t)c * HW + (int64_t)yy * g.W + xx];
+                }
+#pragma unroll
+                for (int u = 0; u < UB; ++u) {
+                    const int e = base + u * APPLY_THREADS + tid;
+                    if (e < total) tile[e] = MODE == MODE_EVAL_X16 ? (float)raw[u] : (float)raw[u] / maxf;
+                }
+            }
+        }
+        for (int e = tid; e < p.TH * P; e += APPLY_THREADS) {
+            int yy = min(y0 + e / P, g.H - 1);
+            rowt[e] = g.rowtab[(int64_t)yy * P + e % P];
+        }
+        for (int e = tid; e < TILE_W * P; e += APPLY_THREADS) {
+            int xx = min(x0 + e / P, g.W - 1);
+            colt[e] = g.coltab[(int64_t)xx * P + e % P];
+        }
+        __syncthreads();
+
+        ASTAMP(0);
+        const int nseg = p.TH * (TILE_W / 32);
+        for (int seg = wave; seg < nseg; seg += APPLY_WAVES) {
+            const int ly = seg / (TILE_W / 32), lx = (seg % (TILE_W / 32)) * 32;
+            const int pixbase = (ly + D) * p.SW + (lx + j + D);
+            const int yy = y0 + ly, xx = x0 + lx + j;
+            const bool inside = yy < g.H && xx < g.W;
+            const int64_t pix = (int64_t)min(yy, g.H - 1) * g.W + min(xx, g.W - 1);
+            const int nreg = 4 * ((C + 7) / 8);
+            unsigned short pre[16];
+            {
+                const uint16_t* src = (MODE == MODE_DECODE) ? A.msb : A.img;
+#pragma unroll
+                for (int r = 0; r < 16; ++r) {
+                    pre[r] = 0;
+                    if (r < nreg) pre[r] = src[(int64_t)min(acc_row(r, h), C - 1) * HW + pix];
+                }
+            }
+            f32x16 acc[NT];
+            f32x16 hid[NT];
+#pragma unroll
+            for (int tt = 0; tt < NT; ++tt)
+#pragma unroll
+                for (int q4 = 0; q4 < 4; ++q4) {
+                    float4 b4 = *reinterpret_cast<const float4*>(bh + (tt * 2 + h) * 16 + q4 * 4);
+                    acc[tt][q4 * 4 + 0] = b4.x; acc[tt][q4 * 4 + 1] = b4.y;
+                    acc[tt][q4 * 4 + 2] = b4.z; acc[tt][q4 * 4 + 3] = b4.w;
+                }
+            if constexpr (MODE == MODE_EVAL_X16) {
+                f32x16 bias0[NT];
+#pragma unroll
+                for (int tt = 0; tt < NT; ++tt) {
+                    bias0[tt] = acc[tt];
+#pragma unroll
+                    for (int r = 0; r < 16; ++r) acc[tt][r] = 0.0f;
+                }
+                const int plane = p.SH * p.SW;
+                const float* tp = tile + h * (C / 2) * plane + ly * p.SW + lx + j;
+                const float* wc = w0 + (size_t)lane * NT * 4;
+                const size_t wstep = (size_t)p.M16 * X16_PIECES * 64 * NT * 4;
+                for (int c = 0; c < C / 2; ++c, tp += plane, wc += wstep) {
+                    if (D == 1) layer0_pair_x16<NT, 1>(acc, wc, tp);
+                    else if (D == 2) layer0_pair_x16<NT, 2>(acc, wc, tp);
+                    else layer0_pair_x16<NT, 3>(acc, wc, tp);
+                }
+                const float cs = lds[p.off_scale];
+#pragma unroll
+                for (int tt = 0; tt < NT; ++tt)
+#pragma unroll
+                    for (int r = 0; r < 16; ++r) acc[tt][r] = fmaf(acc[tt][r], cs, bias0[tt][r]);
+            }
+            for (int s = 0; s < (MODE == MODE_EVAL_X16 ? 0 : P); ++s) {
+                int k = 2 * s + h;
+                float b = (k < P) ? rowt[ly * P + k] : colt[(lx + j) * P + (k - P)];
+                float a[NT];
+                load_a<NT>(w0, s * 64 + lane, a);
+#pragma unroll
+                for (int tt = 0; tt < NT; ++tt)
+                    acc[tt] = __builtin_amdgcn_mfma_f32_32x32x2f32(a[tt], b, acc[tt], 0, 0, 0);
+            }
+            bool paired = MODE == MODE_EVAL_X16;
+            if constexpr (MODE == MODE_EVAL_FAST) {
+                if (p.pair) {
+                    paired = true;
+                    const int plane = p.SH * p.SW;
+                    const float* tp = tile + h * (C / 2) * plane + ly * p.SW + lx + j;
+                    const float* wc = w0 + ((size_t)P * 64 + lane) * NT;
+                    for (int c = 0; c < C / 2; ++c, tp += plane, wc += (size_t)p.RS * 64 * NT) {
+                        if (rel) {
+                            if (D == 1) layer0_pair<NT, 1, true>(acc, wc, tp);
+                            else if (D == 2) layer0_pair<NT, 2, true>(acc, wc, tp);
+                            else layer0_pair<NT, 3, true>(acc, wc, tp);
+                        } else {
+                            if (D == 1) layer0_pair<NT, 1, false>(acc, wc, tp);
+                            else if (D == 2) layer0_pair<NT, 2, false>(acc, wc, tp);
+                            else layer0_pair<NT, 3, false>(acc, wc, tp);
+                        }
+                    }
+                }
+            }
+            if (!paired) {
+                constexpr int CH = APPLY_CHUNK;
+                static_assert(CH % 4 == 0, "the steps left behind the chunks are taken four at a time");
+                int s4 = P;
+                for (; s4 + CH <= p.S0; s4 += CH) {
+                    float bq[CH];
+#pragma unroll
+                    for (int u = 0; u < CH; ++u) {
+                        const int kk = 2 * (s4 + u - P) + h;
+                        const int2 e = *reinterpret_cast<const int2*>(ktab + 2 * kk);
+                        const float nb = tile[pixbase + e.x];
+                        const float ct = tile[pixbase + e.y];
+                        bq[u] = rel ? nb - ct : nb;
+                    }
+                    __builtin_amdgcn_sched_barrier(0);
+#pragma unroll
+                    for (int u = 0; u < CH; ++u) {
+                        float a[NT];
+                        load_a<NT>(w0, (s4 + u) * 64 + lane, a);
+#pragma unroll
+                        for (int tt = 0; tt < NT; ++tt)
+                            acc[tt] = __builtin_amdgcn_mfma_f32_32x32x2f32(a[tt], bq[u], acc[tt], 0, 0, 0);
+                    }
+                    __builtin_amdgcn_sched_barrier(0);
+                }
+                for (; s4 < p.S0; s4 += 4) {
+                    float bq[4];
+                    float aq[4][NT];
+#pragma unroll
+                    for (int u = 0; u < 4; ++u) {
+                        int kk = 2 * (s4 + u - P) + h;
+                        int2 e = *reinterpret_cast<const int2*>(ktab + 2 * kk);
+                        float nb = tile[pixbase + e.x];
+                        float ct = tile[pixbase + e.y];
+                        bq[u] = rel ? nb - ct : nb;
+                        load_a<NT>(w0, (s4 + u) * 64 + lane, aq[u]);
+                    }
+#pragma unroll
+                    for (int u = 0; u < 4; ++u)
+#pragma unroll
+                        for (int tt = 0; tt < NT; ++tt)
+                            acc[tt] = __builtin_amdgcn_mfma_f32_32x32x2f32(aq[u][tt], bq[u], acc[tt], 0, 0, 0);
+                }
+            }
+            ASTAMP(1);
+#pragma unroll
+            for (int tt = 0; tt < NT; ++tt)
+#pragma unroll
+                for (int r = 0; r < 16; ++r) hid[tt][r] = apply_hidden_act<MODE, RELU>(acc[tt][r]);
+            ASTAMP(2);
+            for (int l = 1; l < A.net.nl; ++l) {
+                const float* wlayer = wh + (size_t)(l - 1) * half * 64 * NT;
+#pragma unroll
+                for (int tt = 0; tt < NT; ++tt)
+#pragma unroll
+                    for (int q4 = 0; q4 < 4; ++q4) {
+                        float4 b4 = *reinterpret_cast<const float4*>(bh + ((l * NT + tt) * 2 + h) * 16 + q4 * 4);
+                        acc[tt][q4 * 4 + 0] = b4.x; acc[tt][q4 * 4 + 1] = b4.y;
+                        acc[tt][q4 * 4 + 2] = b4.z; acc[tt][q4 * 4 + 3] = b4.w;
+                    }
+#pragma unroll
+                for (int s = 0; s < NT * 16; ++s) {
+                    float b = hid[s / 16][s % 16];
+                    float a[NT];
+                    load_a<NT>(wlayer, s * 64 + lane, a);
+#pragma unroll
+                    for (int tt = 0; tt < NT; ++tt)
+                        acc[tt] = __builtin_amdgcn_mfma_f32_32x32x2f32(a[tt], b, acc[tt], 0, 0, 0);
+                }
+#pragma unroll
+                for (int tt = 0; tt < NT; ++tt)
+#pragma unroll
+                    for (int r = 0; r < 16; ++r) hid[tt][r] = apply_hidden_act<MODE, RELU>(acc[tt][r]);
+            }
+            ASTAMP(3);
+            f32x16 o;
+            if (mode_fast(MODE)) {
+                if (C > 4) last_layer_4x4<NT, 2>(o, hid, wl, bl, lane);
+                else last_layer_4x4<NT, 1>(o, hid, wl, bl, lane);
+            } else {
+#pragma unroll
+                for (int q4 = 0; q4 < 4; ++q4) {
+                    float4 b4 = *reinterpret_cast<const float4*>(bl + h * 16 + q4 * 4);
+                    o[q4 * 4 + 0] = b4.x; o[q4 * 4 + 1] = b4.y; o[q4 * 4 + 2] = b4.z; o[q4 * 4 + 3] = b4.w;
+                }
+#pragma unroll
+                for (int s = 0; s < NT * 16; ++s) {
+                    float b = hid[s / 16][s % 16];
+                    float a = wl[s * 64 + lane];
+                    o = __builtin_amdgcn_mfma_f32_32x32x2f32(a, b, o, 0, 0, 0);
+                }
+            }
+            ASTAMP(4);
+#pragma unroll
+            for (int r = 0; r < 16; ++r) {
+                const int ch = acc_row(r, h);
+                if (r < nreg && ch < C && inside) {
+                    float yv = mode_fast(MODE) ? fast_sigmoid(o[r]) : canon_sigmoid(o[r]);
+                    if (MODE == MODE_DECODE) {
+                        float rr = __builtin_rintf(yv * scale);
+                        int base = (int)pre[r] << g.K;
+                        A.out[(int64_t)ch * HW + pix] = (uint16_t)(base + (int)rr);
+                        if (A.y_out) A.y_out[pix * C + ch] = yv;
+                    } else if ((int)pre[r] != A.nodata) {
+                        if (MODE == MODE_EVAL && A.decoded) {
+                            int band = ch;
+                            asm volatile("" : "+v"(band));
+                            sse += decoded_term((int)pre[r], (int)A.msb[(int64_t)band * HW + pix], yv, scale, g.K);
+                            continue;
+                        }
+                        float lab = (float)((int)pre[r] & lmask) / scale;
+                        float d = yv - lab;
+                        sse += (double)(d * d);
+                    }
+                }
+            }
+            ASTAMP(5);
+        }
+    }
+    if (MODE != MODE_DECODE) {
+        __syncthreads();
+        double* red = reinterpret_cast<double*>(lds + ((p.off_rowt + 3) & ~3));
+        red[tid] = sse;
+        __syncthreads();
+        for (int o2 = APPLY_THREADS / 2; o2 > 0; o2 >>= 1) {
+            if (tid < o2) red[tid] += red[tid + o2];
+            __syncthreads();
+        }
+        if (tid == 0) A.partial[v] = red[0];
+    }
+    }
+#ifdef LBDRN_APPLY_STAMPS
+    if (tid == 0 && A.stamps)
+        for (int k = 0; k < 8; ++k) A.stamps[(size_t)blockIdx.x * 8 + k] = acc_t[k];
+#endif
diff --git a/lbdrn-msic_amd/csrc/cabi.hip b/lbdrn-msic_amd/csrc/cabi.hip
--- a/lbdrn-msic_amd/csrc/cabi.hip
+++ b/lbdrn-msic_amd/csrc/cabi.hip
@@ -100,6 +100,7 @@
     return 0;
 }
 
+static int planes_fit(const lbdrn_geom* g, const void* planes, size_t have);
 static int workspace_fits(const char* what, const void* ws, size_t have, size_t need)
 {
     if (!ws || have < need) {
@@ -272,9 +273,60 @@
     return generic_decode(gl, *net, msb, params, out, y_out, workspace, workspace_bytes, (hipStream_t)stream);
 }
 
+size_t lbdrn_eval_planes_bytes(const lbdrn_geom* g)
+{
+    if (check_geom(g)) return 0;
+    return mfma_eval_planes_bytes(*g);
+}
+
+int lbdrn_eval_planes_build(const lbdrn_geom* g, const uint16_t* img, const uint16_t* msb, void* planes, size_t planes_bytes,
+                            void* stream)
+{
+    if (int rc = check_geom_call(g)) return rc;
+    LBDRN_REQUIRE(g->msb_max >= 0 && g->msb_max <= 65535, "msb_max=%d out of range", g->msb_max);
+    LBDRN_REQUIRE(img, "img must not be null");
+    LBDRN_ALIGNED(img, 2);
+    LBDRN_ALIGNED(msb, 2);
+    LBDRN_ALIGNED(planes, ALIGN_WORKSPACE);
+    if (int rc = planes_fit(g, planes, planes_bytes)) return rc;
+    NEED_DEVICE();
+    return mfma_eval_planes_build(launch_geom(*g), img, msb, planes, (hipStream_t)stream);
+}
+
+static int planes_fit(const lbdrn_geom* g, const void* planes, size_t have)
+{
+    const size_t need = mfma_eval_planes_bytes(*g);
+    if (!need) {
+        set_error("no evaluation planes for a %d x %d x %d raster (lbdrn_eval_planes_bytes is 0)", g->C, g->H, g->W);
+        return LBDRN_E_UNSUPPORTED;
+    }
+    return workspace_fits("planes", planes, have, need);
+}
+
+static int eval_sse_call(const lbdrn_geom* g, const lbdrn_net* net, const uint16_t* img, const uint16_t* msb,
+                         const float* params, double* sse, void* workspace, size_t workspace_bytes,
+                         int32_t path, void* stream, const void* planes);
+
 int lbdrn_eval_sse(const lbdrn_geom* g, const lbdrn_net* net, const uint16_t* img, const uint16_t* msb,
                    const float* params, double* sse, void* workspace, size_t workspace_bytes,
                    int32_t path, void* stream)
+{
+    return eval_sse_call(g, net, img, msb, params, sse, workspace, workspace_bytes, path, stream, nullptr);
+}
+
+int lbdrn_eval_sse_planes(const lbdrn_geom* g, const lbdrn_net* net, const uint16_t* img, const uint16_t* msb,
+                          const float* params, double* sse, void* workspace, size_t workspace_bytes,
+                          int32_t path, void* stream, const void* planes, size_t planes_bytes)
+{
+    if (int rc = check_geom_call(g)) return rc;
+    LBDRN_ALIGNED(planes, ALIGN_WORKSPACE);
+    if (int rc = planes_fit(g, planes, planes_bytes)) return rc;
+    return eval_sse_call(g, net, img, msb, params, sse, workspace, workspace_bytes, path, stream, planes);
+}
+
+static int eval_sse_call(const lbdrn_geom* g, const lbdrn_net* net, const uint16_t* img, const uint16_t* msb,
+                         const float* params, double* sse, void* workspace, size_t workspace_bytes,
+                         int32_t path, void* stream, const void* planes)
 {
     if (int rc = check_geom_call(g)) return rc;
     if (int rc = check_net(net)) return rc;
@@ -307,7 +359,7 @@
     if (int rc = workspace_fits("apply", workspace, workspace_bytes, lbdrn_apply_workspace(g, net))) return rc;
     if (use_mfma)
         return mfma_eval_sse(gl, *net, img, msb, params, sse, workspace, workspace_bytes, background, fast, x16,
-                             nodata, decoded, (hipStream_t)stream);
+                             nodata, decoded, (hipStream_t)stream, planes);
     return generic_eval_sse(gl, *net, img, msb, params, sse, workspace, workspace_bytes, nodata, decoded, (hipStream_t)stream);
 }
 
diff --git a/lbdrn-msic_amd/csrc/common.hpp b/lbdrn-msic_amd/csrc/common.hpp
--- a/lbdrn-msic_amd/csrc/common.hpp
+++ b/lbdrn-msic_amd/csrc/common.hpp
@@ -111,7 +111,10 @@
                 uint16_t* out, float* y_out, void* ws, size_t ws_bytes, hipStream_t s);
 int mfma_eval_sse(const lbdrn_geom& g, const lbdrn_net& net, const uint16_t* img,
                   const uint16_t* msb, const float* params, double* sse, void* ws, size_t ws_bytes,
-                  bool background, bool fast, bool x16, int nodata, bool decoded, hipStream_t s);
+                  bool background, bool fast, bool x16, int nodata, bool decoded, hipStream_t s,
+                  const void* planes = nullptr);
+size_t mfma_eval_planes_bytes(const lbdrn_geom& g);
+int mfma_eval_planes_build(const lbdrn_geom& g, const uint16_t* img, const uint16_t* msb, void* planes, hipStream_t s);
 bool mfma_eval_reads_msb(const lbdrn_geom& g, const lbdrn_net& net, bool fast, bool x16);
 bool mfma_apply_instance(const lbdrn_geom& g, const lbdrn_net& net, int request, int32_t out[8]);
 
diff --git a/lbdrn-msic_amd/csrc/eval_planes.inc b/lbdrn-msic_amd/csrc/eval_planes.inc
--- /dev/null
+++ b/lbdrn-msic_amd/csrc/eval_planes.inc
@@ -0,0 +1,48 @@
+struct EvalPlanes {
+    int Hp, Wp, pitch;
+    size_t bytes;
+};
+
+static EvalPlanes eval_planes_layout(const lbdrn_geom& g)
+{
+    EvalPlanes L;
+    L.Hp = 16 * ((g.H + 15) / 16) + 2 * g.D;
+    L.Wp = TILE_W * ((g.W + TILE_W - 1) / TILE_W) + 2 * g.D;
+    L.pitch = (L.Wp + 3) & ~3;
+    L.bytes = align_up((size_t)g.C * L.Hp * L.pitch * 4, 256);
+    return L;
+}
+
+__global__ void __launch_bounds__(256) k_build_eval_planes(lbdrn_geom g, const uint16_t* __restrict__ img, const uint16_t* __restrict__ msb,
+                                                          float* __restrict__ planes, EvalPlanes L)
+{
+    const int b = blockIdx.x, tid = threadIdx.x;
+    const int64_t HW = (int64_t)g.H * g.W;
+    if (b == 0)
+        for (size_t e = (size_t)g.C * L.Hp * L.pitch + tid; e < L.bytes / 4; e += 256) planes[e] = 0.0f;
+    const int c = b / L.Hp, py = b - c * L.Hp, y = py - g.D;
+    const int iy = y < g.H + g.D ? reflect_idx(y, g.H) : g.H - 1;
+    const uint16_t* src = (msb ? msb : img) + (int64_t)c * HW + (int64_t)iy * g.W;
+    const int shift = msb ? 0 : g.K;
+    const float maxf = (float)g.msb_max;
+    float* dst = planes + (size_t)b * L.pitch;
+    for (int px = tid; px < L.pitch; px += 256) {
+        const int x = px - g.D;
+        const int ix = x < g.W + g.D ? reflect_idx(x, g.W) : g.W - 1;
+        dst[px] = (float)(unsigned short)(src[ix] >> shift) / maxf;
+    }
+}
+
+size_t mfma_eval_planes_bytes(const lbdrn_geom& g)
+{
+    if (g.H > (1 << 24) || g.W > (1 << 24) || (int64_t)g.C * ((int64_t)g.H + 2 * g.D + 16) > 0x7fffffff) return 0;
+    return eval_planes_layout(g).bytes;
+}
+
+int mfma_eval_planes_build(const lbdrn_geom& g, const uint16_t* img, const uint16_t* msb, void* planes, hipStream_t s)
+{
+    const EvalPlanes L = eval_planes_layout(g);
+    k_build_eval_planes<<<g.C * L.Hp, 256, 0, s>>>(g, img, msb, (float*)planes, L);
+    LBDRN_LAUNCH_CHECK();
+    return 0;
+}
diff --git a/lbdrn-msic_amd/lbdrn_hip/_lib.py b/lbdrn-msic_amd/lbdrn_hip/_lib.py
--- a/lbdrn-msic_amd/lbdrn_hip/_lib.py
+++ b/lbdrn-msic_amd/lbdrn_hip/_lib.py
@@ -51,6 +51,9 @@
     "lbdrn_apply_workspace": (_sz, [_GP, _NP]),
     "lbdrn_decode_fused": (ctypes.c_int, [_GP, _NP, _vp, _vp, _vp, _vp, _vp, _sz, _i32, _vp]),
     "lbdrn_eval_sse": (ctypes.c_int, [_GP, _NP, _vp, _vp, _vp, _vp, _vp, _sz, _i32, _vp]),
+    "lbdrn_eval_planes_bytes": (_sz, [_GP]),
+    "lbdrn_eval_planes_build": (ctypes.c_int, [_GP, _vp, _vp, _vp, _sz, _vp]),
+    "lbdrn_eval_sse_planes": (ctypes.c_int, [_GP, _NP, _vp, _vp, _vp, _vp, _vp, _sz, _i32, _vp, _vp, _sz]),
     "lbdrn_apply_instance": (ctypes.c_int, [_GP, _NP, _i32, ctypes.POINTER(_i32)]),
     "lbdrn_train_workspace": (_sz, [_GP, _NP, _i32]),
     "lbdrn_train_prepare": (ctypes.c_int, [_GP, _NP, _vp, _vp, _i32, _vp, _sz, _i32, _vp]),
diff --git a/lbdrn-msic_amd/lbdrn_hip/codec.py b/lbdrn-msic_amd/lbdrn_hip/codec.py
--- a/lbdrn-msic_amd/lbdrn_hip/codec.py
+++ b/lbdrn-msic_amd/lbdrn_hip/codec.py
@@ -135,7 +135,8 @@
     apply_ws = int(L.lbdrn_apply_workspace(ctypes.byref(g), ctypes.byref(net)))
     perms = epochs * N * 8 + int(L.lbdrn_randperm_workspace(N, min(32, max(epochs - 1, 1))))
     planes = 3 * C * N * 2
-    return train + apply_ws + perms + planes + (epochs + 4) * int(ops.param_count(net)) * 4 + (64 << 20)
+    eval_planes = int(L.lbdrn_eval_planes_bytes(ctypes.byref(g))) if ops.eval_planes_enabled() else 0
+    return train + apply_ws + perms + planes + eval_planes + (epochs + 4) * int(ops.param_count(net)) * 4 + (64 << 20)
 
 
 def default_in_flight(C, H, W, K, D, base_channel, num_layers, cfg=None, path=None):
@@ -220,6 +221,11 @@
     for s in _fit_stream_pool(dev, 2):
         if s.cuda_stream != main.cuda_stream:
             return s
+
+
+def _prepare_eval_planes(apply_ws, geom, net, img_d, msb_d, path, eval_epochs):
+    if eval_epochs and ops.eval_planes_serve(geom, net, path, fast_evaluation(), exact16_evaluation()):
+        apply_ws.prepare_planes(geom, img_d, msb_d)
 
 
 def fit_device(img_d, K, D, base_channel, num_layers, lr, batch_size, epochs, val_duration=1,
@@ -265,6 +271,7 @@
     apply_ws = ops.ApplyWorkspace(geom, net, dev)
     mse_log = torch.zeros((epochs, 2), dtype=torch.float32, device=dev)
     eval_epochs = [] if epochs == 1 else [e for e in range(1, epochs + 1) if e % min(val_duration, epochs) == 0]
+    _prepare_eval_planes(apply_ws, geom, net, img_d, msb_d, path, eval_epochs)
     main = torch.cuda.current_stream(dev)
     side = _eval_stream(dev, main) if len(eval_epochs) > 1 and overlap_evaluation(dev, alone) else None
     snaps = torch.empty((max(len(eval_epochs), 1), params.numel()), dtype=torch.float32, device=dev)
@@ -386,6 +393,7 @@
     steps_per_epoch = steps_of(n_fit, batch_size)
     eval_epochs = [] if epochs == 1 else [e for e in range(1, epochs + 1) if e % min(val_duration, epochs) == 0]
     for f in st:
+        _prepare_eval_planes(f["aws"], f["geom"], net, f["img"], f["msb"], path, eval_epochs)
         f["snaps"] = torch.empty((max(len(eval_epochs), 1), f["params"].numel()), dtype=torch.float32, device=dev)
         f["mses"] = torch.zeros((max(len(eval_epochs), 1),), dtype=torch.float32, device=dev)
     adam_steps = 0
diff --git a/lbdrn-msic_amd/lbdrn_hip/ops.py b/lbdrn-msic_amd/lbdrn_hip/ops.py
--- a/lbdrn-msic_amd/lbdrn_hip/ops.py
+++ b/lbdrn-msic_amd/lbdrn_hip/ops.py
@@ -1,4 +1,5 @@
 import ctypes
+import os
 
 import numpy as np
 import torch
@@ -143,10 +144,49 @@
     return grads, dx
 
 
+def eval_planes_enabled():
+    return os.environ.get("LBDRN_EVAL_PLANES", "1") != "0"
+
+
+def eval_planes_bytes(geom):
+    return int(lib().lbdrn_eval_planes_bytes(ctypes.byref(geom.c)))
+
+
+def eval_planes_serve(geom, net, path=PATH_AUTO, fast=False, x16=False):
+    if path == _lib.PATH_GENERIC:
+        return False
+    out = (ctypes.c_int32 * 8)()
+    word = path | (EVAL_FAST if fast else 0) | (EVAL_X16 if (fast and x16) else 0)
+    return lib().lbdrn_apply_instance(ctypes.byref(geom.c), ctypes.byref(net), word, out) == 0 and out[0] == 1 and out[3] in (1, 2)
+
+
 class ApplyWorkspace:
+
     def __init__(self, geom, net, device):
         self.nbytes = lib().lbdrn_apply_workspace(ctypes.byref(geom.c), ctypes.byref(net))
         self.buf = torch.empty(max(self.nbytes, 1), dtype=torch.uint8, device=device)
+        self.planes = None
+        self.planes_for = None
+
+    @staticmethod
+    def planes_key(img, msb, geom):
+        return (img.data_ptr(), img._version, msb.data_ptr(), msb._version, int(geom.c.K), int(geom.c.D), int(geom.c.msb_max))
+
+    def prepare_planes(self, geom, img, msb):
+        if not eval_planes_enabled():
+            return None
+        img, msb = _u16(img.contiguous()), _u16(msb.contiguous())
+        key = self.planes_key(img, msb, geom)
+        if self.planes_for != key:
+            nbytes = eval_planes_bytes(geom)
+            if not nbytes:
+                return None
+            if self.planes is None or self.planes.numel() != nbytes:
+                self.planes = torch.empty(nbytes, dtype=torch.uint8, device=self.buf.device)
+            self.planes_for = None
+            _call(lib().lbdrn_eval_planes_build, img, ctypes.byref(geom.c), _ptr(img), _ptr(msb), _ptr(self.planes), nbytes)
+            self.planes_for = key
+        return self.planes
 
 
 def decode_fused(geom, net, msb, params, want_y=False, path=PATH_AUTO, ws=None):
@@ -168,16 +208,23 @@
     msb = _u16(msb.contiguous())
     params = params.contiguous().float()
     sse = out if out is not None else torch.zeros(1, dtype=torch.float64, device=msb.device)
+    planes = ws.prepare_planes(geom, img, msb) if ws is not None and eval_planes_serve(geom, net, path, fast, x16) else None
     ws = ws or ApplyWorkspace(geom, net, msb.device)
     gc = geom.c
     if nodata is not None:
         gc = Geom.from_buffer_copy(geom.c)
         gc.reserved = int(nodata)
+    word = (path | (EVAL_BACKGROUND if background else 0) | (EVAL_FAST if fast else 0) | (EVAL_X16 if (fast and x16) else 0) |
+            (EVAL_VALID if nodata is not None else 0) | (EVAL_DECODED if decoded else 0))
+    if planes is not None:
+        with torch.cuda.device(msb.device):
+            check(lib().lbdrn_eval_sse_planes(ctypes.byref(gc), ctypes.byref(net), _ptr(img), _ptr(msb), _ptr(params), _ptr(sse),
+                                              _ptr(ws.buf), ws.nbytes, word,
+                                              ctypes.c_void_p(torch.cuda.current_stream(msb.device).cuda_stream),
+                                              _ptr(planes), planes.numel()))
+        return sse
     _call(lib().lbdrn_eval_sse, msb, ctypes.byref(gc), ctypes.byref(net), _ptr(img), _ptr(msb),
-                               _ptr(params), _ptr(sse), _ptr(ws.buf), ws.nbytes,
-                               path | (EVAL_BACKGROUND if background else 0) | (EVAL_FAST if fast else 0) |
-                               (EVAL_X16 if (fast and x16) else 0) | (EVAL_VALID if nodata is not None else 0) |
-                               (EVAL_DECODED if decoded else 0))
+                               _ptr(params), _ptr(sse), _ptr(ws.buf), ws.nbytes, word)
     return sse
 
 
```

Result: no change. 71.19 Mpixels/s (-0.6%).
